# pierluigiferrari/ssd_keras

Measured on AMD Instinct MI355X. Metric: images/sec SSD300 fwd+decode @batch32, higher is better.
Workload: dtype f32 (decode, threshold, TF-style f32 NMS, top-k); bf16 conv backbone; 1 GPU; SSD300 VGG-16 inference (mode='inference': forward + DecodeDetections), 21 classes, batch 32 per GPU, conf 0.01 / NMS 0.45 / top-200, random-init weights, synthetic 300x300x3 uint8-range images; per_gpu_batch=32, global_batch=32, conv_dtype=bf16, parallelism=replicas x1, launch=hip_graph (forward + DecodeDetections captured once, replayed per step), decode_stream=same stream; DecodeDetections reads the head outputs directly (no y_pred in HBM)

## Files before the change

### include/ssdhip.h

```cpp
#ifndef SSDHIP_H
#define SSDHIP_H

#include <stddef.h>

#ifdef __cplusplus
extern "C" {
#endif

#define SSDHIP_ABI_VERSION 1

enum {
    SSDHIP_OK = 0,
    SSDHIP_E_BADARG = -1,
    SSDHIP_E_WORKSPACE = -2,
    SSDHIP_E_LAUNCH = -3
};

enum { SSDHIP_F32 = 0, SSDHIP_F64 = 1 };
enum { SSDHIP_CENTROIDS = 0, SSDHIP_CORNERS = 1, SSDHIP_MINMAX = 2 };
enum { SSDHIP_BORDER_HALF = 0, SSDHIP_BORDER_INCLUDE = 1, SSDHIP_BORDER_EXCLUDE = 2 };
enum {
    SSDHIP_SEM_NUMPY = 0,
    SSDHIP_SEM_KERAS = 1,
    SSDHIP_SEM_DEBUG = 2
// ... 139 lines not shown
int ssdhip_conv1_1_x3_nhwc(const float* x, const float* weight, const float* bias, void* y, int B, int H, int W, int relu, void* stream);
int ssdhip_conv1_1_x3_pre_nhwc(const float* images, const float* weight, const float* bias, void* y, int B, int H, int W, int relu,
                               const float* mean_h, const float* divide_h, const int* swap_h, void* stream);

size_t ssdhip_conv2d_splitk_workspace_bytes(int B, int H, int W, int Cin, int Cout, int kernel, int stride, int pad, int dilation,
                                            int ksplit);
int ssdhip_conv2d_splitk_nhwc_bf16(const void* x, const void* weight, const void* bias, void* y, int B, int H, int W, int Cin, int Cout,
                                   int kernel, int stride, int pad, int dilation, int relu, int ksplit, void* ws, size_t ws_bytes,
                                   void* stream);

int ssdhip_conv2d_same_nhwc_bf16_variant(int variant, const void* x, const void* weight, const void* bias, void* y,
                                         int B, int H, int W, int Cin, int Cout, int kernel, int dilation, int relu, void* stream);

int ssdhip_assemble_predictions_strided_f32(int n_layers, const void* const* conf_h, const void* const* loc_h, const int* n_anchors_h,
                                            const int* n_boxes_h, const int* conf_stride_h, const int* loc_stride_h,
                                            const float* anchors_var, int B, int N, int C, float* y_pred, void* stream);
int ssdhip_decode_from_heads_f32(int n_layers, const void* const* conf_h, const void* const* loc_h, const int* n_anchors_h,
                                 const int* n_boxes_h, const int* conf_stride_h, const int* loc_stride_h, const float* anchors_var,
                                 int B, int N, int C, double conf_thresh, double iou_thresh, int top_k, int nms_cap, int class_agnostic,
                                 int semantics, int coords, int normalize_coords, double img_height, double img_width, int border_pixels,
                                 void* out, int out_dtype, int out_rows, int* out_count, int* out_anchor_idx, void* ws, size_t ws_bytes,
                                 void* stream);

int ssdhip_decode_from_heads(int n_layers, const void* const* conf_h, const void* const* loc_h,
                             const void* const* conf_bias_h, const void* const* loc_bias_h,
                             const int* n_anchors_h, const int* n_boxes_h, const int* conf_stride_h,
                             const int* loc_stride_h, const float* anchors_var, int B, int N, int C,
                             double conf_thresh, double iou_thresh, int top_k, int nms_cap, int class_agnostic,
                             int semantics, int coords, int normalize_coords, double img_height, double img_width,
                             int border_pixels, void* out, int out_dtype, int out_rows, int* out_count,
                             int* out_anchor_idx, void* ws, size_t ws_bytes, void* stream);

int ssdhip_conv2d_same_pool2_nhwc_bf16(const void* x, const void* weight, const void* bias, void* y, int B, int H, int W,
                                       int Cin, int Cout, int kernel, int dilation, int relu, void* stream);

int ssdhip_conv2d_same_group_nhwc_bf16(int n_problems, const void* const* x_h, const void* const* weight_h,
                                       const void* const* bias_h, void* const* y_h, const int* B_h, const int* H_h,
                                       const int* W_h, const int* Cin_h, const int* Cout_h, const int* kernel_h,
                                       const int* dilation_h, int relu, void* stream);

int ssdhip_conv3x3_c64_nhwc_bf16(const void* x, const void* weight, const void* bias, void* y, int B, int H, int W,
                                 int Cin, int Cout, int relu, int pool, int n_workgroups, void* stream);
int ssdhip_conv3x3_c64_pool_keep_nhwc_bf16(const void* x, const void* weight, const void* bias, void* y_full, void* y_pooled, int B, int H,
                                           int W, int Cin, int Cout, int relu, int n_workgroups, void* stream);

int ssdhip_conv3x3_halo_nhwc_bf16(const void* x, const void* weight, const void* bias, void* y, int B, int H, int W,
                                  int Cin, int Cout, int relu, int pool, void* stream);

int ssdhip_conv3x3_halo_plan(int B, int H, int W, int Cout, int pool, int* plan);

int ssdhip_conv3x3_halo_masked_nhwc_bf16(const void* x, const void* weight, const void* mask, void* y, float* bias_partial,
                                         int bias_rows, int B, int H, int W, int Cin, int Cout, void* stream);
int ssdhip_conv3x3_halo_masked_bias_rows(int B, int H, int W, int Cout);

int ssdhip_conv3x3_halo_pool_keep_nhwc_bf16(const void* x, const void* weight, const void* bias, void* y_full, void* y_pooled, int B, int H,
                                            int W, int Cin, int Cout, int relu, void* stream);

size_t ssdhip_conv_chain_packed_bytes(int k, int Cin, int Cout);
int ssdhip_conv_chain_pack_weight(const void* weight, void* packed, int k, int Cin, int Cout, void* stream);
int ssdhip_conv_chain_nhwc_bf16(const void* x, int B, int H, int W, int C0, int n_layers, const void* const* packed_h,
                                const void* const* bias_h, void* const* y_h, const int* k_h, const int* stride_h, const int* pad_h,
                                const int* cout_h, const int* relu_h, void* stream);
size_t ssdhip_conv_chain_x3_packed_bytes(int k, int Cin, int Cout);
int ssdhip_conv_chain_x3_pack_weight(const void* weight_x3, void* packed, int k, int Cin, int Cout, void* stream);
int ssdhip_conv_chain_x3_nhwc_f16(const void* x, int B, int H, int W, int C0, int n_layers, const void* const* packed_h,
                                  const float* const* bias_h, void* const* y_h, const int* k_h, const int* stride_h, const int* pad_h,
                                  const int* cout_h, const int* relu_h, const float* mul_h, void* stream);

size_t ssdhip_conv3x3_wgrad_workspace_bytes(int B, int H, int W, int Cin, int Cout);
int ssdhip_conv3x3_wgrad_bias_nhwc_bf16(const void* x, const void* dy, float* dw, const float* bias_partial, int bias_rows, float* db,
                                        int B, int H, int W, int Cin, int Cout, void* ws, size_t ws_bytes, void* stream);
int ssdhip_conv3x3_wgrad_nhwc_bf16(const void* x, const void* dy, float* dw, int B, int H, int W, int Cin, int Cout, void* ws,
                                   size_t ws_bytes, void* stream);

int ssdhip_conv3x3_halo_strided_nhwc_bf16(const void* x, const void* weight, const void* bias, void* y, int B, int H, int W,
                                          int Cin, int Cout, int stride, int pad, int relu, void* stream);

int ssdhip_conv3x3_halo_group_nhwc_bf16(int n_problems, const void* const* x_h, const void* const* weight_h, const void* const* bias_h,
                                        void* const* y_h, const int* B_h, const int* H_h, const int* W_h, const int* Cin_h,
                                        const int* Cout_h, int relu, int max_workgroups, void* stream);

int ssdhip_conv1_block_nhwc_bf16(const void* x3, const void* w1, const void* b1, const void* weight, const void* bias, void* y,
                                 int B, int H, int W, int Cout, int relu, int pool, int n_workgroups, void* stream);

int ssdhip_conv3x3_cin3_nhwc_bf16(const void* x, const void* weight, const void* bias, void* y, int B, int H, int W,
                                  int Cin, int Cout, int relu, void* stream);

size_t ssdhip_conv_bn_elu_pack_bytes(int Cin, int Cout, int kernel);
int ssdhip_conv_bn_elu_nhwc_bf16(const void* x, const void* w_packed, const float* scale, const float* shift, void* y, int B, int H, int W,
                                 int Cin, int Cout, int kernel, int pool, void* stream);

int ssdhip_bn_elu_train_blocks(long long positions, int C);
int ssdhip_bn_elu_train_fwd_nhwc_bf16(const void* y, const void* gamma, const void* beta, int param_bf16, void* running_mean,
                                      void* running_var, int running_bf16, double momentum, double eps, void* full, void* pooled,
                                      float* mean, float* invstd, float* tables, float* partial, int B, int H, int W, int C,
                                      int n_slots, void* stream);
int ssdhip_bn_elu_train_bwd_nhwc_bf16(const void* y, const float* mean, const float* invstd, const void* gamma, const void* beta,
                                      int param_bf16, const void* g_full, const void* g_pooled, void* dy, float* dgamma,
                                      float* dbeta, float* partial, int B, int H, int W, int C, int n_slots, void* stream);

int ssdhip_conv_same_bias_nhwc_bf16(const void* x, const void* w_packed, const void* bias, void* y, int B, int H, int W, int Cin, int Cout,
                                    int kernel, void* stream);
int ssdhip_ssd7_pack_filters(int n_layers, const void* const* weights, void* const* fwd, void* const* flipped, const int* Cin,
                             const int* Cout, const int* kernel, const long long* strides, void* stream);
int ssdhip_ssd7_conv_wgrad_plan(int B, int H, int W, int Cin, int Cout, int kernel, int* plan);
size_t ssdhip_ssd7_conv_wgrad_workspace_bytes(int B, int H, int W, int Cin, int Cout, int kernel);
int ssdhip_ssd7_conv_wgrad_nhwc_bf16(const void* x, const void* dy, void* dw, void* db, int B, int H, int W, int Cin, int Cout, int kernel,
                                     int out_bf16, const long long* dw_strides, void* workspace, size_t workspace_bytes, void* stream);

int ssdhip_image_program(const void* x, int in_dtype, void* y, int out_dtype, int n_images, long long pixels_per_image,
                         const int* ops_dev, const double* args_dev, void* stream);
int ssdhip_image_resize_cv_u8(const void* x, void* y, int B, int H, int W, int Ho, int Wo, int C, int kind, int area, const int* ix_dev,
                              const double* wx_dev, int nx, const int* iy_dev, const double* wy_dev, int ny, void* stream);
int ssdhip_image_resize_gather_cv_u8(const void* x, void* y, int B, int H, int W, int Ho, int Wo, int C, const int* plan_dev,
                                     const int* ix_dev, const double* wx_dev, int nx, const int* iy_dev, const double* wy_dev, int ny,
                                     const void* background_dev, void* stream);
int ssdhip_image_warp_affine_u8(const void* x, void* y, int B, int H, int W, int Ho, int Wo, int C, const int* geo_dev, const int* xtab_dev,
                                const int* ytab_dev, const void* background_dev, void* stream);
int ssdhip_image_resize_gather_ragged_u8(const void* x, const long long* table_dev, void* y, int B, int Ho, int Wo, const int* plan_dev,
                                         const int* ix_dev, const double* wx_dev, int nx, const int* iy_dev, const double* wy_dev, int ny,
                                         const void* background_dev, void* stream);
int ssdhip_image_program_ragged_u8(const void* x, const long long* table_dev, void* y, int B, long long max_pixels, const int* ops_dev,
                                   const double* args_dev, void* stream);
int ssdhip_image_hist_u8(const void* x, long long n_pixels, int C, int channel, unsigned int* hist_dev, void* stream);
int ssdhip_image_lut_u8(const void* x, void* y, long long n_values, int C, int channel_mask, const void* table_dev, void* stream);

int ssdhip_conv3x3_image_nhwc_bf16(const void* x, const void* weight, const void* bias, void* y, int B, int H, int W, int Cin, int Cout,
                                   int dilation, int relu, void* stream);
int ssdhip_conv2d_image_nhwc_bf16(const void* x, const void* weight, const void* bias, void* y, int B, int H, int W, int Cin, int Cout,
                                  int ksize, int stride, int padding, int dilation, int relu, void* stream);
int ssdhip_conv2d_image_x3_nhwc_f16(const void* x, const void* weight, const float* bias, void* y, int B, int H, int W, int C, int Cout,
                                    int ksize, int stride, int padding, int dilation, int relu, int out_f32, float oscale, void* stream);

typedef struct ssdhip_shadow_desc {
    const void* src;
    void* cl;
    void* tr;
    int O, I, KK, tr_ostride, tr_ooff, tile0;
    int src_channels_last;
    int reserved;
} ssdhip_shadow_desc;
int ssdhip_shadow_refresh(const ssdhip_shadow_desc* table_dev, int n_weights, int n_tiles, int n_vectors, int n_vector_blocks, void* stream);
int ssdhip_sgd_momentum_step(int n_tensors, void* const* params_h, const void* const* grads_h, void* const* bufs_h,
                             const long long* numel_h, double lr, double momentum, double weight_decay, void* stream);

#define SSDHIP_ADAM_MAX_GROUPS 64
typedef struct ssdhip_adam_group {
    double lr, decay, beta_1, beta_2;
    double b1t, b2t;
    float lr_t, one_minus_beta_1, one_minus_beta_2, beta_1_f, beta_2_f, epsilon, weight_decay;
    int reserved;
} ssdhip_adam_group;
typedef struct ssdhip_adam_state {
    long long iterations;
    int n_groups, reserved;
    ssdhip_adam_group groups[];
} ssdhip_adam_state;
size_t ssdhip_adam_state_bytes(int n_groups);
int ssdhip_adam_state_init(void* state, int n_groups, int group, double lr, double beta_1, double beta_2, double epsilon, double decay,
                           double weight_decay, long long iterations, void* stream);
int ssdhip_adam_step(int n_tensors, void* const* params_h, const void* const* grads_h, void* const* m_h, void* const* v_h,
                     void* const* vhat_h, const long long* numel_h, int group, void* state, int tick, void* stream);
int ssdhip_adam_step_bf16(int n_tensors, void* const* params_h, const void* const* grads_h, void* const* master_h, void* const* m_h,
                          void* const* v_h, void* const* vhat_h, const long long* numel_h, int group, void* state, int tick, void* stream);
int ssdhip_optim_set_lr(void* state, int group, double lr, void* stream);

typedef struct ssdhip_sgd_group {
    double lr, decay, momentum;
    float lr_t, momentum_f, weight_decay;
    int reserved;
} ssdhip_sgd_group;
typedef struct ssdhip_sgd_state {
    long long iterations;
    int n_groups, reserved;
    ssdhip_sgd_group groups[];
} ssdhip_sgd_state;
size_t ssdhip_sgd_state_bytes(int n_groups);
int ssdhip_sgd_state_init(void* state, int n_groups, int group, double lr, double momentum, double decay, double weight_decay,
                          long long iterations, void* stream);
int ssdhip_sgd_set_lr(void* state, int group, double lr, void* stream);
int ssdhip_sgd_step(int n_tensors, void* const* params_h, const void* const* grads_h, void* const* bufs_h, const long long* numel_h,
                    int group, void* state, int rule, int nesterov, int tick, void* stream);
int ssdhip_sgd_step_bf16(int n_tensors, void* const* params_h, const void* const* grads_h, void* const* master_h, void* const* bufs_h,
                         const long long* numel_h, int group, void* state, int rule, int nesterov, int tick, void* stream);

typedef struct ssdhip_augment_params {
    int img_height, img_width;
    double expand_prob, expand_min_scale, expand_max_scale;
    double crop_prob, crop_min_scale, crop_max_scale, crop_min_aspect_ratio, crop_max_aspect_ratio;
    int n_trials, n_bounds;
    double bound_cdf[8], bound_lower[8], bound_upper[8];
    double flip_prob;
    int n_modes, interpolation_modes[8], out_height, out_width;
    int max_rounds;
} ssdhip_augment_params;
int ssdhip_augment_plans(const int* geometry_dev, int B, int H, int W, int out_h, int out_w, int n_taps, int* plan_dev, int* ix_dev,
                         double* wx_dev, int* iy_dev, double* wy_dev, void* stream);
int ssdhip_ssd_augment_decide(const ssdhip_augment_params* params, int B, const unsigned int* mt_state, const double* labels,
                              const int* n_labels, int* geometry, double* labels_out, int* n_labels_out, unsigned int* mt_state_out,
                              void* stream);
typedef struct ssdhip_augment_photo {
    double prob[4], lower[4], upper[4];
    double swap_prob;
} ssdhip_augment_photo;
int ssdhip_ssd_augment_decide_stream(const ssdhip_augment_params* params, const ssdhip_augment_photo* photo, int B,
                                     const unsigned int* mt_state, const double* labels, const int* n_labels, int* programs_ops,
                                     double* programs_args, int* geometry, double* labels_out, int* n_labels_out,
                                     unsigned int* mt_state_out, void* stream);
int ssdhip_ssd_augment_decide_stream_ragged(const ssdhip_augment_params* params, const ssdhip_augment_photo* photo, int B,
                                            const long long* table_dev, const unsigned int* mt_state, const double* labels,
                                            const int* n_labels, int* programs_ops, double* programs_args, int* geometry,
                                            double* labels_out, int* n_labels_out, unsigned int* mt_state_out, void* stream);
int ssdhip_augment_plans_ragged(const int* geometry_dev, const long long* table_dev, int B, int out_h, int out_w, int n_taps, int* plan_dev,
// ... 7 lines not shown
```

### ssd_keras_amd/_native.py

```python
from __future__ import annotations

import ctypes
import os
import threading

import numpy as np

_LIB_PATH = os.environ.get("SSDHIP_LIB") or os.path.join(os.path.dirname(os.path.abspath(__file__)), "libssdhip.so")
_lib = None
_lock = threading.Lock()

F32, F64 = 0, 1
COORDS = {"centroids": 0, "corners": 1, "minmax": 2}
BORDER = {"half": 0, "include": 1, "exclude": 2}
SEM_NUMPY, SEM_KERAS, SEM_DEBUG = 0, 1, 2
ABI_VERSION = 1


class SsdHipError(RuntimeError):
    pass


def lib_path():
    return _LIB_PATH
# ... 24 lines not shown
    "ssdhip_decode_workspace_bytes": (_SZ, [_I] * 7),
    "ssdhip_decode_detections": (_I, [_P] + [_I] * 4 + [_D, _D] + [_I] * 6 + [_D, _D, _I, _P, _I, _I] + [_P] * 3 + [_SZ, _P]),
    "ssdhip_decode_stages": (_I, [_I, _P] + [_I] * 4 + [_D, _D] + [_I] * 6 + [_D, _D, _I, _P, _I, _I] + [_P] * 3 + [_SZ, _P]),
    "ssdhip_encode_workspace_bytes": (_SZ, [_I] * 4),
    "ssdhip_encode": (_I, [_P] * 4 + [_I] * 5 + [_D, _D, _I, _D, _D] + [_I] * 4 + [_P] * 4 + [_SZ, _P]),
    "ssdhip_loss_workspace_bytes": (_SZ, [_I] * 3),
    "ssdhip_loss_forward": (_I, [_P, _P] + [_I] * 5 + [_F] + [_P] * 4 + [_SZ, _P]),
    "ssdhip_loss_backward": (_I, [_P] * 5 + [_I] * 3 + [_F, _P, _P]),
    "ssdhip_convert_coordinates": (_I, [_P, _I, _P, _LL] + [_I] * 4 + [_P]),
    "ssdhip_iou_result_dtype": (_I, [_I] * 3),
    "ssdhip_box_overlap": (_I, [_I, _P, _I, _I, _P] + [_I] * 5 + [_P, _P]),
    "ssdhip_match_bipartite_greedy": (_I, [_P, _I, _I, _P, _P]),
    "ssdhip_match_multi_workspace_bytes": (_SZ, [_I, _I]),
    "ssdhip_match_multi": (_I, [_P, _I, _I, _D] + [_P] * 4 + [_SZ, _P]),
    "ssdhip_greedy_nms_workspace_bytes": (_SZ, [_I]),
    "ssdhip_greedy_nms": (_I, [_P] + [_I] * 4 + [_P, _I, _D, _I, _I] + [_P] * 3 + [_SZ, _P]),
    "ssdhip_box_filter": (_I, [_P] * 3 + [_I] * 6 + [_D] * 3 + [_I, _P, _P]),
    "ssdhip_match_predictions_workspace_bytes": (_SZ, [_I, _I]),
    "ssdhip_match_predictions": (_I, [_P, _P, _I] + [_P] * 3 + [_I, _I, _D, _I] + [_P] * 6 + [_SZ, _P]),
    "ssdhip_match_predictions_multi": (_I, [_P] * 3 + [_I] + [_P] * 3 + [_I, _I, _P, _I, _D, _I] + [_P] * 6 + [_SZ, _P]),
    "ssdhip_bias_act_nhwc_bf16": (_I, [_P] * 3 + [_LL, _I, _I, _P]),
    "ssdhip_bias_act_maxpool_nhwc_bf16": (_I, [_P] * 3 + [_I] * 10 + [_P]),
    "ssdhip_l2_normalize_nhwc_bf16": (_I, [_P] * 3 + [_LL, _I, _P]),
    "ssdhip_pool2_l2_normalize_nhwc_bf16": (_I, [_P] * 4 + [_I] * 4 + [_P]),
    "ssdhip_preprocess_nhwc_f32_to_bf16": (_I, [_P, _P, _LL, _I] + [_P] * 4),
    "ssdhip_assemble_predictions_bf16": (_I, [_I] + [_P] * 7 + [_I] * 3 + [_P, _P]),
    "ssdhip_l2_normalize_bwd_waves": (_I, [_LL, _I, _I]),
    "ssdhip_l2_normalize_fwd": (_I, [_P] * 4 + [_LL, _I, _I, _P]),
    "ssdhip_l2_normalize_bwd": (_I, [_P] * 6 + [_I, _LL, _I, _I, _P]),
    "ssdhip_relu_bwd_bias_blocks": (_I, [_LL, _I]),
    "ssdhip_channel_sums_nhwc_bf16": (_I, [_P, _P, _LL, _I, _I, _P]),
    "ssdhip_conv1x1_wgrad_workspace_bytes": (_SZ, [_LL, _I, _I]),
    "ssdhip_conv1x1_wgrad_bias_nhwc_bf16": (_I, [_P] * 4 + [_I, _P, _LL, _I, _I, _P, _SZ, _P]),
    "ssdhip_conv3x3_taps_wgrad_workspace_bytes": (_SZ, [_I] * 10),
    "ssdhip_conv3x3_taps_wgrad_bias_nhwc_bf16": (_I, [_P] * 4 + [_I, _P] + [_I] * 10 + [_P, _SZ, _P]),
    "ssdhip_row_sums_f32": (_I, [_P, _I, _I, _P, _P]),
    "ssdhip_embed_strided_nhwc_bf16": (_I, [_P, _P] + [_I] * 8 + [_P]),
    "ssdhip_assemble_predictions_backward_bf16": (_I, [_I] + [_P] * 6 + [_I] * 3 + [_P]),
    "ssdhip_assemble_backward_lds_bytes": (_SZ, [_I, _P, _P, _I]),
    "ssdhip_conv1_1_bwd_blocks": (_I, [_I] * 3),
    "ssdhip_conv1_1_bwd_nhwc_bf16": (_I, [_P] * 5 + [_I] * 4 + [_P]),
    "ssdhip_relu_bwd_bias_nhwc_bf16": (_I, [_P] * 4 + [_LL, _I, _I, _P]),
    "ssdhip_maxpool2_relu_bwd_bias_nhwc_bf16": (_I, [_P] * 4 + [_I] * 5 + [_P]),
    "ssdhip_maxpool_bwd_nhwc_bf16": (_I, [_P] * 3 + [_I] * 9 + [_P]),
    "ssdhip_assemble_predictions_strided_bf16": (_I, [_I] + [_P] * 9 + [_I] * 3 + [_P, _P]),
    "ssdhip_conv2d_same_nhwc_bf16": (_I, [_P] * 4 + [_I] * 8 + [_P]),
    "ssdhip_conv2d_nhwc_bf16": (_I, [_P] * 4 + [_I] * 10 + [_P]),
    "ssdhip_conv2d_nhwc_bf16_variant": (_I, [_I] + [_P] * 4 + [_I] * 10 + [_P]),
    "ssdhip_conv2d_x3_nhwc_f16": (_I, [_P] * 4 + [_I] * 12 + [_F, _P]),
    "ssdhip_conv3x3_halo_x3_nhwc_f16": (_I, [_P] * 4 + [_I] * 7 + [_F, _P]),
    "ssdhip_x3_split_nhwc": (_I, [_P, _P, _LL, _I, _P]),
    "ssdhip_x3_merge_nhwc": (_I, [_P, _P, _LL, _I, _P]),
    "ssdhip_x3_maxpool_nhwc": (_I, [_P, _P] + [_I] * 9 + [_P]),
    "ssdhip_x3_l2_normalize_nhwc": (_I, [_P] * 3 + [_LL, _I, _F, _P]),
    "ssdhip_conv1_1_x3_nhwc": (_I, [_P] * 4 + [_I] * 4 + [_P]),
    "ssdhip_conv1_1_x3_pre_nhwc": (_I, [_P] * 4 + [_I] * 4 + [_P] * 4),
    "ssdhip_conv2d_splitk_workspace_bytes": (_SZ, [_I] * 10),
    "ssdhip_conv2d_splitk_nhwc_bf16": (_I, [_P] * 4 + [_I] * 11 + [_P, _SZ, _P]),
    "ssdhip_conv2d_same_nhwc_bf16_variant": (_I, [_I] + [_P] * 4 + [_I] * 8 + [_P]),
    "ssdhip_assemble_predictions_strided_f32": (_I, [_I] + [_P] * 7 + [_I] * 3 + [_P, _P]),
    "ssdhip_decode_from_heads_f32": (_I, [_I] + [_P] * 7 + [_I] * 3 + [_D, _D] + [_I] * 6 + [_D, _D, _I, _P, _I, _I] + [_P] * 3 + [_SZ, _P]),
    "ssdhip_decode_from_heads": (_I, [_I] + [_P] * 9 + [_I] * 3 + [_D, _D] + [_I] * 6 + [_D, _D, _I, _P, _I, _I] + [_P] * 3 + [_SZ, _P]),
    "ssdhip_conv2d_same_pool2_nhwc_bf16": (_I, [_P] * 4 + [_I] * 8 + [_P]),
    "ssdhip_conv2d_same_group_nhwc_bf16": (_I, [_I] + [_P] * 11 + [_I, _P]),
    "ssdhip_conv3x3_c64_nhwc_bf16": (_I, [_P] * 4 + [_I] * 8 + [_P]),
    "ssdhip_conv3x3_c64_pool_keep_nhwc_bf16": (_I, [_P] * 5 + [_I] * 7 + [_P]),
    "ssdhip_conv3x3_halo_nhwc_bf16": (_I, [_P] * 4 + [_I] * 7 + [_P]),
    "ssdhip_conv3x3_halo_plan": (_I, [_I] * 5 + [_INTP]),
    "ssdhip_conv3x3_halo_masked_nhwc_bf16": (_I, [_P] * 5 + [_I] * 6 + [_P]),
    "ssdhip_conv3x3_halo_masked_bias_rows": (_I, [_I] * 4),
    "ssdhip_conv3x3_halo_pool_keep_nhwc_bf16": (_I, [_P] * 5 + [_I] * 6 + [_P]),
    "ssdhip_conv_chain_packed_bytes": (_SZ, [_I] * 3),
    "ssdhip_conv_chain_pack_weight": (_I, [_P, _P] + [_I] * 3 + [_P]),
    "ssdhip_conv_chain_nhwc_bf16": (_I, [_P] + [_I] * 5 + [_P] * 9),
    "ssdhip_conv_chain_x3_packed_bytes": (_SZ, [_I] * 3),
    "ssdhip_conv_chain_x3_pack_weight": (_I, [_P, _P] + [_I] * 3 + [_P]),
    "ssdhip_conv_chain_x3_nhwc_f16": (_I, [_P] + [_I] * 5 + [_P] * 10),
    "ssdhip_conv3x3_wgrad_workspace_bytes": (_SZ, [_I] * 5),
    "ssdhip_conv3x3_wgrad_bias_nhwc_bf16": (_I, [_P] * 4 + [_I, _P] + [_I] * 5 + [_P, _SZ, _P]),
    "ssdhip_conv3x3_wgrad_nhwc_bf16": (_I, [_P] * 3 + [_I] * 5 + [_P, _SZ, _P]),
    "ssdhip_conv3x3_halo_strided_nhwc_bf16": (_I, [_P] * 4 + [_I] * 8 + [_P]),
    "ssdhip_conv3x3_halo_group_nhwc_bf16": (_I, [_I] + [_P] * 9 + [_I, _I, _P]),
    "ssdhip_conv1_block_nhwc_bf16": (_I, [_P] * 6 + [_I] * 7 + [_P]),
    "ssdhip_conv3x3_cin3_nhwc_bf16": (_I, [_P] * 4 + [_I] * 6 + [_P]),
    "ssdhip_conv_bn_elu_pack_bytes": (_SZ, [_I] * 3),
    "ssdhip_conv_bn_elu_nhwc_bf16": (_I, [_P] * 5 + [_I] * 7 + [_P]),
    "ssdhip_bn_elu_train_blocks": (_I, [_LL, _I]),
    "ssdhip_bn_elu_train_fwd_nhwc_bf16": (_I, [_P] * 3 + [_I, _P, _P, _I, _D, _D] + [_P] * 6 + [_I] * 5 + [_P]),
    "ssdhip_bn_elu_train_bwd_nhwc_bf16": (_I, [_P] * 5 + [_I] + [_P] * 6 + [_I] * 5 + [_P]),
    "ssdhip_conv_same_bias_nhwc_bf16": (_I, [_P] * 4 + [_I] * 6 + [_P]),
    "ssdhip_ssd7_pack_filters": (_I, [_I] + [_P] * 3 + [_INTP] * 3 + [_LLP, _P]),
    "ssdhip_ssd7_conv_wgrad_plan": (_I, [_I] * 6 + [_INTP]),
    "ssdhip_ssd7_conv_wgrad_workspace_bytes": (_SZ, [_I] * 6),
    "ssdhip_ssd7_conv_wgrad_nhwc_bf16": (_I, [_P] * 4 + [_I] * 7 + [_LLP, _P, _SZ, _P]),
    "ssdhip_image_program": (_I, [_P, _I, _P, _I, _I, _LL] + [_P] * 3),
    "ssdhip_image_resize_cv_u8": (_I, [_P, _P] + [_I] * 8 + [_P, _P, _I, _P, _P, _I, _P]),
    "ssdhip_image_resize_gather_cv_u8": (_I, [_P, _P] + [_I] * 6 + [_P] * 3 + [_I, _P, _P, _I, _P, _P]),
    "ssdhip_image_warp_affine_u8": (_I, [_P, _P] + [_I] * 6 + [_P] * 5),
    "ssdhip_image_resize_gather_ragged_u8": (_I, [_P, _P, _P] + [_I] * 3 + [_P] * 3 + [_I, _P, _P, _I, _P, _P]),
    "ssdhip_image_program_ragged_u8": (_I, [_P, _P, _P, _I, _LL] + [_P] * 3),
    "ssdhip_image_hist_u8": (_I, [_P, _LL, _I, _I, _P, _P]),
    "ssdhip_image_lut_u8": (_I, [_P, _P, _LL, _I, _I, _P, _P]),
    "ssdhip_conv3x3_image_nhwc_bf16": (_I, [_P] * 4 + [_I] * 7 + [_P]),
    "ssdhip_conv2d_image_nhwc_bf16": (_I, [_P] * 4 + [_I] * 10 + [_P]),
    "ssdhip_conv2d_image_x3_nhwc_f16": (_I, [_P] * 4 + [_I] * 11 + [_F, _P]),
    "ssdhip_shadow_refresh": (_I, [_P] + [_I] * 4 + [_P]),
    "ssdhip_sgd_momentum_step": (_I, [_I] + [_P] * 4 + [_D] * 3 + [_P]),
    "ssdhip_adam_state_bytes": (_SZ, [_I]),
    "ssdhip_adam_state_init": (_I, [_P, _I, _I] + [_D] * 6 + [_LL, _P]),
    "ssdhip_adam_step": (_I, [_I] + [_P] * 6 + [_I, _P, _I, _P]),
    "ssdhip_adam_step_bf16": (_I, [_I] + [_P] * 7 + [_I, _P, _I, _P]),
    "ssdhip_optim_set_lr": (_I, [_P, _I, _D, _P]),
    "ssdhip_sgd_state_bytes": (_SZ, [_I]),
    "ssdhip_sgd_state_init": (_I, [_P, _I, _I] + [_D] * 4 + [_LL, _P]),
    "ssdhip_sgd_set_lr": (_I, [_P, _I, _D, _P]),
    "ssdhip_sgd_step": (_I, [_I] + [_P] * 4 + [_I, _P, _I, _I, _I, _P]),
    "ssdhip_sgd_step_bf16": (_I, [_I] + [_P] * 5 + [_I, _P, _I, _I, _I, _P]),
    "ssdhip_augment_plans": (_I, [_P] + [_I] * 6 + [_P] * 6),
    "ssdhip_ssd_augment_decide": (_I, [_PARAMS, _I] + [_P] * 8),
    "ssdhip_ssd_augment_decide_stream": (_I, [_PARAMS, _PHOTO, _I] + [_P] * 10),
    "ssdhip_ssd_augment_decide_stream_ragged": (_I, [_PARAMS, _PHOTO, _I] + [_P] * 11),
    "ssdhip_augment_plans_ragged": (_I, [_P, _P] + [_I] * 4 + [_P] * 6),
}


def load():
    global _lib
    if _lib is not None:
        return _lib
    with _lock:
        if _lib is not None:
            return _lib
        if not os.path.exists(_LIB_PATH):
            raise SsdHipError("libssdhip.so not found at %s: build it with `python -m ssd_keras_amd.build` "
                              "(hipcc, gfx950).  ssd_keras_amd has no CPU fallback." % _LIB_PATH)
        lib = ctypes.CDLL(_LIB_PATH)
        for name, (restype, argtypes) in SIGNATURES.items():
            if not hasattr(lib, name):
                raise SsdHipError("%s lacks %s: rebuild it with `python -m ssd_keras_amd.build`" % (_LIB_PATH, name))
            fn = getattr(lib, name)
            fn.restype, fn.argtypes = restype, argtypes
        if lib.ssdhip_abi_version() != ABI_VERSION:
            raise SsdHipError("libssdhip.so ABI %d != expected %d" % (lib.ssdhip_abi_version(), ABI_VERSION))
        _lib = lib
    return _lib


def check(rc, what):
    if rc != 0:
        raise SsdHipError("%s failed: %s (rc=%d)" % (what, load().ssdhip_strerror(rc).decode(), rc))


def _torch():
    import torch
    return torch


def require_cuda(t, name):
    if not t.is_cuda:
        raise SsdHipError("%s must live on a GPU (got device %s): ssd_keras_amd has no CPU path" % (name, t.device))
    if not t.is_contiguous():
        raise SsdHipError("%s must be contiguous" % name)


def current_stream_ptr(device):
    torch = _torch()
    return ctypes.c_void_p(torch.cuda.current_stream(device).cuda_stream)


def launch(name, device, *args):
    torch = _torch()
    with torch.cuda.device(device):
        rc = getattr(load(), name)(*args, current_stream_ptr(device))
    check(rc, name)


class _Workspaces:

    def __init__(self):
        self._bufs = {}

    def get(self, device, purpose, nbytes, zeroed=False):
        torch = _torch()
        key = (str(device), purpose, int(torch.cuda.current_stream(device).cuda_stream))
        buf = self._bufs.get(key)
        if buf is None or buf.numel() < nbytes:
            buf = (torch.zeros if zeroed else torch.empty)(int(nbytes), dtype=torch.uint8, device=device)
# ... 526 lines not shown
    launch("ssdhip_maxpool_bwd_nhwc_bf16", x.device, _ptr(x), _ptr(gy), _ptr(gx), b, h, w, c, int(kernel), int(stride), int(pad), ho, wo)
    return gx


def conv2d_same(x, weight, bias, dilation=1, relu=True, variant=None):
    torch = _torch()
    x, (b, h, w, cin) = _nhwc_bf16(x, "x")
    cout, cin_w, kh, kw = weight.shape
    if weight.dtype != torch.bfloat16 or cin_w != cin or kh != kw:
        raise SsdHipError("weight must be bfloat16 (Cout, %d, k, k)" % cin)
    wt = weight if weight.permute(0, 2, 3, 1).is_contiguous() else weight.permute(0, 2, 3, 1).contiguous().permute(0, 3, 1, 2)
    y = torch.empty((b, h, w, cout), dtype=torch.bfloat16, device=x.device).permute(0, 3, 1, 2)
    args = (_ptr(x), _ptr(wt), _ptr(bias), _ptr(y), b, h, w, cin, cout, int(kh), int(dilation), int(bool(relu)))
    if variant is None:
        launch("ssdhip_conv2d_same_nhwc_bf16", x.device, *args)
    else:
        launch("ssdhip_conv2d_same_nhwc_bf16_variant", x.device, int(variant), *args)
    return y


def conv3x3_halo_plan(b, h, w, pool, cout=128):
    plan = (ctypes.c_int * 4)()
    check(load().ssdhip_conv3x3_halo_plan(int(b), int(h), int(w), int(cout), int(bool(pool)), plan), "ssdhip_conv3x3_halo_plan")
    return tuple(plan)


def conv3x3_halo(x, weight, bias, relu=True, pool=False):
    torch = _torch()
    x, (b, h, w, cin) = _nhwc_bf16(x, "x")
    cout, cin_w, kh, kw = weight.shape
    if weight.dtype != torch.bfloat16 or cin_w != cin or kh != 3 or kw != 3:
        raise SsdHipError("weight must be bfloat16 (Cout, %d, 3, 3)" % cin)
    wt = weight if weight.permute(0, 2, 3, 1).is_contiguous() else weight.permute(0, 2, 3, 1).contiguous().permute(0, 3, 1, 2)
    ho, wo = ((h + 1) // 2, (w + 1) // 2) if pool else (h, w)
    y = torch.empty((b, ho, wo, cout), dtype=torch.bfloat16, device=x.device).permute(0, 3, 1, 2)
    launch("ssdhip_conv3x3_halo_nhwc_bf16", x.device, _ptr(x), _ptr(wt), _ptr(bias), _ptr(y), b, h, w, cin, cout, int(bool(relu)),
           int(bool(pool)))
    return y


def conv3x3_halo_masked(x, weight, mask, sums=False):
    torch = _torch()
    lib = load()
    cout, cin_w, kh, kw = weight.shape
    if (not x.is_cuda or x.dtype != torch.bfloat16 or weight.dtype != torch.bfloat16 or mask.dtype != torch.bfloat16 or kh != 3 or kw != 3
            or cin_w % 128 or cout % 128 or x.shape[1] != cin_w):
        return None
    x, (b, h, w, cin) = _nhwc_bf16(x, "x")
    mask, mshape = _nhwc_bf16(mask, "mask")
    if mshape != (b, h, w, cout):
        raise SsdHipError("mask must have the output's shape %s, got %s" % ((b, h, w, cout), mshape))
    wt = weight if weight.permute(0, 2, 3, 1).is_contiguous() else weight.permute(0, 2, 3, 1).contiguous().permute(0, 3, 1, 2)
    y = torch.empty((b, h, w, cout), dtype=torch.bfloat16, device=x.device).permute(0, 3, 1, 2)
    partial, rows = None, 0
    with torch.cuda.device(x.device):
        if sums:
            rows = lib.ssdhip_conv3x3_halo_masked_bias_rows(b, h, w, cout)
            if rows <= 0:
                return None
            partial = torch.empty((rows, cout), dtype=torch.float32, device=x.device)
        rc = lib.ssdhip_conv3x3_halo_masked_nhwc_bf16(_ptr(x), _ptr(wt), _ptr(mask), _ptr(y), _ptr(partial), rows, b, h, w, cin, cout,
                                                      current_stream_ptr(x.device))
    if rc == -1:
        return None
    check(rc, "ssdhip_conv3x3_halo_masked_nhwc_bf16")
    return (y, partial) if sums else y


def conv3x3_image_supported(x, weight, dilation=1):
    b, cin, h, w = x.shape
    cout, cin_w, kh, kw = weight.shape
    return kh == 3 and kw == 3 and cin_w == cin and h * w <= 384 and cin % 64 == 0 and cout % 64 == 0 and 1 <= int(dilation) <= 16


def conv3x3_image(x, weight, bias, dilation=1, relu=True):
    torch = _torch()
    x, (b, h, w, cin) = _nhwc_bf16(x, "x")
    cout, cin_w, kh, kw = weight.shape
    if weight.dtype != torch.bfloat16 or cin_w != cin or kh != 3 or kw != 3:
        raise SsdHipError("weight must be bfloat16 (Cout, %d, 3, 3)" % cin)
    wt = weight if weight.permute(0, 2, 3, 1).is_contiguous() else weight.permute(0, 2, 3, 1).contiguous().permute(0, 3, 1, 2)
    y = torch.empty((b, h, w, cout), dtype=torch.bfloat16, device=x.device).permute(0, 3, 1, 2)
    launch("ssdhip_conv3x3_image_nhwc_bf16", x.device, _ptr(x), _ptr(wt), _ptr(bias), _ptr(y), b, h, w, cin, cout, int(dilation),
           int(bool(relu)))
    return y


def conv2d_image_supported(x, weight, stride=1, padding=0, dilation=1):
    b, cin, h, w = x.shape
    cout, cin_w, kh, kw = weight.shape
    k, s, p, d = int(kh), int(stride), int(padding), int(dilation)
    if kh != kw or k not in (1, 3) or cin_w != cin or cin % 64 or cout % 64 or h * w > 384:
        return False
    if not (1 <= s <= 4 and 1 <= d <= 16 and 0 <= p <= d * (k // 2)) or h + 2 * p < d * (k - 1) + 1 or w + 2 * p < d * (k - 1) + 1:
        return False
    ho, wo = (h + 2 * p - d * (k - 1) - 1) // s + 1, (w + 2 * p - d * (k - 1) - 1) // s + 1
    return 1 <= ho * wo <= 384


def conv2d_image(x, weight, bias, stride=1, padding=0, dilation=1, relu=True):
    torch = _torch()
    x, (b, h, w, cin) = _nhwc_bf16(x, "x")
    cout, cin_w, kh, kw = weight.shape
    if weight.dtype != torch.bfloat16 or cin_w != cin or kh != kw or kh not in (1, 3):
        raise SsdHipError("weight must be bfloat16 (Cout, %d, k, k) with k in (1, 3)" % cin)
    k, s, p, d = int(kh), int(stride), int(padding), int(dilation)
    wt = weight if weight.permute(0, 2, 3, 1).is_contiguous() else weight.permute(0, 2, 3, 1).contiguous().permute(0, 3, 1, 2)
    ho, wo = (h + 2 * p - d * (k - 1) - 1) // s + 1, (w + 2 * p - d * (k - 1) - 1) // s + 1
    if ho < 1 or wo < 1:
        raise SsdHipError("the filter does not fit the padded map")
    y = torch.empty((b, ho, wo, cout), dtype=torch.bfloat16, device=x.device).permute(0, 3, 1, 2)
    launch("ssdhip_conv2d_image_nhwc_bf16", x.device, _ptr(x), _ptr(wt), _ptr(bias), _ptr(y), b, h, w, cin, cout, k, s, p, d,
           int(bool(relu)))
    return y


def conv_chain_pack(weight, out=None):
    torch = _torch()
    lib = load()
    cout, cin, kh, kw = weight.shape
    if weight.dtype != torch.bfloat16 or kh != kw:
        raise SsdHipError("weight must be bfloat16 (Cout, Cin, k, k)")
    n = int(lib.ssdhip_conv_chain_packed_bytes(kh, cin, cout))
    if n == 0:
        return None
    wt = weight if weight.permute(0, 2, 3, 1).is_contiguous() else weight.permute(0, 2, 3, 1).contiguous().permute(0, 3, 1, 2)
    if out is not None and (out.numel() != n or out.dtype != torch.uint8 or out.device != weight.device):
        raise SsdHipError("conv_chain_pack: `out` does not match this filter's packed size")
    packed = out if out is not None else torch.empty((n,), dtype=torch.uint8, device=weight.device)
    launch("ssdhip_conv_chain_pack_weight", weight.device, _ptr(wt), _ptr(packed), kh, cin, cout)
    return packed


def conv_chain(x, layers):
    torch = _torch()
    lib = load()
    x, (b, h, w, c0) = _nhwc_bf16(x, "x")
    n = len(layers)
    outs, ys = [], []
    hh, ww = h, w
    for l in layers:
        hh = (hh + 2 * l["pad"] - l["k"]) // l["stride"] + 1
        ww = (ww + 2 * l["pad"] - l["k"]) // l["stride"] + 1
        if hh < 1 or ww < 1:
            return None
        if l.get("keep", False):
            y = torch.empty((b, hh, ww, l["cout"]), dtype=torch.bfloat16, device=x.device).permute(0, 3, 1, 2)
            outs.append(y)
            ys.append(y)
        else:
            ys.append(None)
    parr = lambda ts: (ctypes.c_void_p * n)(*[(t.data_ptr() if t is not None else None) for t in ts])
    iarr = lambda key: (ctypes.c_int * n)(*[int(l[key]) for l in layers])
    with torch.cuda.device(x.device):
        rc = lib.ssdhip_conv_chain_nhwc_bf16(_ptr(x), b, h, w, c0, n, parr([l["packed"] for l in layers]), parr([l.get("bias") for l in layers]),
                                             parr(ys), iarr("k"), iarr("stride"), iarr("pad"), iarr("cout"), iarr("relu"),
                                             current_stream_ptr(x.device))
    if rc == -1:
        return None
    check(rc, "ssdhip_conv_chain_nhwc_bf16")
    return outs


def conv_chain_x3_pack(packed_weight, out=None):
    torch = _torch()
    lib = load()
# ... 621 lines not shown
                or t.dtype not in (torch.float32, torch.bfloat16)):
            raise SsdHipError("bn_elu_train: %s must be a contiguous (%d,) float32 or bfloat16 tensor on %s" % (name, c, device))
        dtypes.add(t.dtype)
    if len(dtypes) > 1:
        raise SsdHipError("bn_elu_train: %s must share one dtype" % " and ".join(named))
    return int(dtypes.pop() == torch.bfloat16)


def bn_elu_train_blocks(positions, c):
    return int(load().ssdhip_bn_elu_train_blocks(int(positions), int(c)))


def bn_elu_train_forward(y, gamma, beta, running_mean, running_var, momentum, eps, pool, keep_full):
    torch = _torch()
    b, h, w, c = _bn_train_map(y, "y")
    nb = bn_elu_train_blocks(b * h * w, c)
    if nb == 0:
        raise SsdHipError("bn_elu_train: no kernel for C = %d with B H W = %d (C in 32, 48, 64; at least two positions)" % (c, b * h * w))
    if pool and (h < 2 or w < 2):
        raise SsdHipError("bn_elu_train: a %d x %d map has no 2 x 2 window to pool" % (h, w))
    param_bf16 = _bn_train_vectors(c, y.device, gamma=gamma, beta=beta)
    if (running_mean is None) != (running_var is None):
        raise SsdHipError("bn_elu_train: running_mean and running_var come together")
    running_bf16 = 0 if running_mean is None else _bn_train_vectors(c, y.device, running_mean=running_mean, running_var=running_var)
    dev = y.device
    full = torch.empty((b, h, w, c), dtype=torch.bfloat16, device=dev).permute(0, 3, 1, 2) if (keep_full or not pool) else None
    pooled = torch.empty((b, h // 2, w // 2, c), dtype=torch.bfloat16, device=dev).permute(0, 3, 1, 2) if pool else None
    stats = torch.empty((4, c), dtype=torch.float32, device=dev)
    partial = torch.empty((nb, 3, c), dtype=torch.float32, device=dev)
    launch("ssdhip_bn_elu_train_fwd_nhwc_bf16", dev, _ptr(y), _ptr(gamma), _ptr(beta), param_bf16, _ptr(running_mean), _ptr(running_var),
           running_bf16, float(momentum), float(eps), _ptr(full), _ptr(pooled), _ptr(stats[0]), _ptr(stats[1]), _ptr(stats[2]),
           _ptr(partial), b, h, w, c, nb)
    return full, pooled, stats[0], stats[1]


def bn_elu_train_backward(y, mean, invstd, gamma, beta, g_full, g_pooled):
    torch = _torch()
    b, h, w, c = _bn_train_map(y, "y")
    nb = bn_elu_train_blocks(b * h * w, c)
    if nb == 0:
        raise SsdHipError("bn_elu_train: no kernel for C = %d with B H W = %d (C in 32, 48, 64; at least two positions)" % (c, b * h * w))
    if g_full is None and g_pooled is None:
        raise SsdHipError("bn_elu_train: the backward needs the gradient of the full map, of the pooled map or both")
    if g_full is not None and _bn_train_map(g_full, "g_full") != (b, h, w, c):
        raise SsdHipError("bn_elu_train: g_full must have y's shape")
    if g_pooled is not None and (h < 2 or w < 2 or _bn_train_map(g_pooled, "g_pooled") != (b, h // 2, w // 2, c)):
        raise SsdHipError("bn_elu_train: g_pooled must be the gradient of y's 2 x 2 'valid' pooled map")
    param_bf16 = _bn_train_vectors(c, y.device, gamma=gamma, beta=beta)
    if _bn_train_vectors(c, y.device, mean=mean, invstd=invstd) != 0:
        raise SsdHipError("bn_elu_train: mean and invstd are float32")
    dev = y.device
    dy = torch.empty((b, h, w, c), dtype=torch.bfloat16, device=dev).permute(0, 3, 1, 2)
    grads = torch.empty((2, c), dtype=torch.float32, device=dev)
    partial = torch.empty((nb, 2, c), dtype=torch.float32, device=dev)
    launch("ssdhip_bn_elu_train_bwd_nhwc_bf16", dev, _ptr(y), _ptr(mean), _ptr(invstd), _ptr(gamma), _ptr(beta), param_bf16, _ptr(g_full),
           _ptr(g_pooled), _ptr(dy), _ptr(grads[0]), _ptr(grads[1]), _ptr(partial), b, h, w, c, nb)
    return dy, grads[0], grads[1]


def conv1_block(x, w1, b1, weight, bias, relu=True, pool=False):
    torch = _torch()
    if not x.is_cuda or x.dtype != torch.bfloat16 or x.dim() != 4 or x.shape[1] != 3:
        raise SsdHipError("x must be a (B, 3, H, W) bfloat16 CUDA tensor")
    if not x.permute(0, 2, 3, 1).is_contiguous():
        x = x.permute(0, 2, 3, 1).contiguous().permute(0, 3, 1, 2)
    b, _, h, w = x.shape
    if tuple(w1.shape) != (64, 3, 3, 3) or weight.shape[1:] != (64, 3, 3) or w1.dtype != torch.bfloat16 or weight.dtype != torch.bfloat16:
        raise SsdHipError("conv1_block needs bfloat16 (64, 3, 3, 3) and (Cout, 64, 3, 3) weights")
    cl = lambda t: t if t.permute(0, 2, 3, 1).is_contiguous() else t.permute(0, 2, 3, 1).contiguous().permute(0, 3, 1, 2)
    w1c, w2c = cl(w1), cl(weight)
    cout = weight.shape[0]
    ho, wo = ((h + 1) // 2, (w + 1) // 2) if pool else (h, w)
    y = torch.empty((b, ho, wo, cout), dtype=torch.bfloat16, device=x.device).permute(0, 3, 1, 2)
    dev = x.device
    n_cu = _CU_COUNT.get(dev.index)
    if n_cu is None:
        n_cu = torch.cuda.get_device_properties(dev).multi_processor_count
        _CU_COUNT[dev.index] = n_cu
    launch("ssdhip_conv1_block_nhwc_bf16", dev, _ptr(x), _ptr(w1c), _ptr(b1), _ptr(w2c), _ptr(bias), _ptr(y), b, h, w, cout,
           int(bool(relu)), int(bool(pool)), int(n_cu))
    return y


CONVERSIONS = {"minmax2centroids": 0, "centroids2minmax": 1, "corners2centroids": 2, "centroids2corners": 3,
               "minmax2corners": 4, "corners2minmax": 4}


def _float_device(a, name):
    torch = _torch()
    if isinstance(a, np.ndarray):
        if a.dtype not in (np.float32, np.float64):
            a = a.astype(np.float64)
        return to_device(a)
    if not torch.is_tensor(a):
        return to_device(np.asarray(a, dtype=np.float64))
    if a.dtype not in (torch.float32, torch.float64):
        a = a.to(torch.float64)
    return to_device(a)


def _dt(t):
    torch = _torch()
    return F32 if t.dtype == torch.float32 else F64


def convert_coordinates(t, start_index, conversion, border_pixels):
    torch = _torch()
    require_cuda(t, "tensor")
    L = int(t.shape[-1])
    rows = t.numel() // L if L else 0
    out = torch.empty(t.shape, dtype=torch.float64, device=t.device)
    if t.numel() == 0:
        return out
    launch("ssdhip_convert_coordinates", t.device, _ptr(t), _dt(t), _ptr(out), rows, L, int(start_index), CONVERSIONS[conversion],
           BORDER[border_pixels])
    return out


def box_overlap(op, b1, b2, coords, mode, border_pixels):
    torch = _torch()
    lib = load()
    require_cuda(b1, "boxes1")
    require_cuda(b2, "boxes2")
    m, n = int(b1.shape[0]), int(b2.shape[0])
    rdt = torch.float32 if lib.ssdhip_iou_result_dtype(_dt(b1), _dt(b2), COORDS[coords]) == F32 else torch.float64
    outer = mode == "outer_product"
    out = torch.empty((m, n) if outer else (max(m, n) if min(m, n) > 0 else 0,), dtype=rdt, device=b1.device)
    if out.numel() == 0:
        return out
    launch("ssdhip_box_overlap", b1.device, int(op), _ptr(b1), _dt(b1), m, _ptr(b2), _dt(b2), n, COORDS[coords], 0 if outer else 1,
           BORDER[border_pixels], _ptr(out))
    return out


def match_bipartite_greedy(w):
    torch = _torch()
    require_cuda(w, "weight_matrix")
    m, n = int(w.shape[0]), int(w.shape[1])
    out = torch.zeros((m,), dtype=torch.int32, device=w.device)
    if m == 0:
        return out
    launch("ssdhip_match_bipartite_greedy", w.device, _ptr(w), m, n, _ptr(out))
    return out


def match_multi(w, threshold):
    torch = _torch()
    lib = load()
    require_cuda(w, "weight_matrix")
    m, n = int(w.shape[0]), int(w.shape[1])
    gt = torch.empty((max(n, 1),), dtype=torch.int32, device=w.device)
    col = torch.empty((max(n, 1),), dtype=torch.int32, device=w.device)
    cnt = torch.zeros((1,), dtype=torch.int32, device=w.device)
    ws = workspaces.get(w.device, "match_multi", lib.ssdhip_match_multi_workspace_bytes(m, n))
    launch("ssdhip_match_multi", w.device, _ptr(w), m, n, float(threshold), _ptr(gt), _ptr(col), _ptr(cnt), _ptr(ws), ws.numel())
    k = int(cnt.item())
    return gt[:k], col[:k]


def greedy_nms_rows(rows, seg_offsets, score_col, box_col, iou_threshold, coords, border_pixels):
    torch = _torch()
    lib = load()
    require_cuda(rows, "rows")
    n_total, L = int(rows.shape[0]), int(rows.shape[1])
    S = len(seg_offsets) - 1
    dev = rows.device
# ... 349 lines not shown
```

### ssd_keras_amd/csrc/ssdhip_bf16.h

```cpp
#pragma once
#include <hip/hip_runtime.h>
#include <stdint.h>

namespace ssdhip {

typedef unsigned int u32;

typedef unsigned short bf16_t;
typedef __bf16 bf16x2 __attribute__((ext_vector_type(2)));
typedef __bf16 bf16x8 __attribute__((ext_vector_type(8)));
typedef _Float16 f16x8 __attribute__((ext_vector_type(8)));
typedef float f32x2 __attribute__((ext_vector_type(2)));
typedef float f32x16 __attribute__((ext_vector_type(16)));
typedef short s16x2 __attribute__((ext_vector_type(2)));
typedef int i32x4 __attribute__((ext_vector_type(4)));
typedef unsigned int u32x2 __attribute__((ext_vector_type(2)));
typedef unsigned int u32x4 __attribute__((ext_vector_type(4)));

__device__ __forceinline__ float bf16_float(u32 h) { return __uint_as_float(h << 16); }
template <typename T = u32>
__device__ __forceinline__ T bf16_bits(float f) {
    const u32 u = __float_as_uint(f);
    if ((u & 0x7fffffffu) > 0x7f800000u) return (T)((u >> 16) | 0x40u);
    return (T)((u + 0x7fffu + ((u >> 16) & 1u)) >> 16);
}

__device__ __forceinline__ u32 pack2_bf16(float a, float b) {
    const f32x2 v = {a, b};
    return __builtin_bit_cast(u32, __builtin_convertvector(v, bf16x2));
}

__device__ __forceinline__ float relu_nan(float v) { return v <= 0.f ? 0.f : v; }

__device__ __forceinline__ u32 pkmax_i16(u32 a, u32 b) {
    return __builtin_bit_cast(u32, __builtin_elementwise_max(__builtin_bit_cast(s16x2, a), __builtin_bit_cast(s16x2, b)));
}

__device__ __forceinline__ u32 split2_f16(float a, float b, u32& lo_out) {
    const _Float16 ha = (_Float16)a, hb = (_Float16)b;
    const _Float16 la = (_Float16)(a - (float)ha), lb = (_Float16)(b - (float)hb);
    lo_out = (u32)__builtin_bit_cast(unsigned short, la) | ((u32)__builtin_bit_cast(unsigned short, lb) << 16);
    return (u32)__builtin_bit_cast(unsigned short, ha) | ((u32)__builtin_bit_cast(unsigned short, hb) << 16);
}

}
```

### ssd_keras_amd/csrc/ssdhip_conv64.hip

```cpp
#include <hip/hip_runtime.h>
#include <stdint.h>
#include <stdlib.h>

#include <type_traits>

#include "ssdhip.h"
#include "ssdhip_math.h"
#include "ssdhip_bf16.h"
#include "ssdhip_tile.h"

#ifndef SSDHIP_C64_ABLATE
#define SSDHIP_C64_ABLATE 0
#endif

namespace ssdhip {

#ifdef SSDHIP_PROFILE
__device__ unsigned long long g_prof64[32];
#define C64_PROF_DECL long long _pt = clock64(); long long _pa[8] = {0, 0, 0, 0, 0, 0, 0, 0}; int _pn = 0;
#define C64_PROF_MARK(i) { const long long _t = clock64(); _pa[i] += _t - _pt; _pt = _t; }
#define C64_PROF_TILE ++_pn;
#define C64_PROF_FLUSH(base) if (lane == 0) { for (int _i = 0; _i < 8; ++_i) atomicAdd(&g_prof64[(base) + _i], (unsigned long long)_pa[_i]); atomicAdd(&g_prof64[(base) + 8], (unsigned long long)_pn); }
#else
#define C64_PROF_DECL
#define C64_PROF_MARK(i)
#define C64_PROF_TILE
#define C64_PROF_FLUSH(base)
#endif

#ifndef SSDHIP_C64_NLOAD
#define SSDHIP_C64_NLOAD 1
#endif
constexpr int C64_NLOAD = SSDHIP_C64_NLOAD;
constexpr int C64_THREADS = (4 + C64_NLOAD) * 64;
constexpr int C64_NPROD = 3;
constexpr int C64_FRONT_THREADS = (4 + C64_NPROD) * 64;
constexpr int C64_WBYTES = 9 * 64 * 128;
constexpr int C64_STAGE = 0;
constexpr int c64_halo_bytes(int cs) { return ((9 * (2 * (64 >> cs) + 2) * ((1 << cs) + 2) + 63) / 64) * 1024; }
constexpr int C64_PATCH1 = 1600;
constexpr int C64_PATCH = ((C64_NPROD * C64_PATCH1 + 1023) / 1024) * 1024;
constexpr int C64_WREG_BYTES = 1024;
constexpr int c64_lds_bytes(int cs, int nb, bool front = false, bool wreg = false) {
    return (wreg ? C64_WREG_BYTES : C64_WBYTES) + nb * c64_halo_bytes(cs) + C64_STAGE + (front ? C64_PATCH : 0);
}

struct C64Params {
    const bf16_t* x;
    const bf16_t* w;
    const bf16_t* bias;
    bf16_t* y;
    int B, H, W, Cout, relu;
    int HT, WT, n_slices, tiles;
    int Ho, Wo;
    int x_bytes, w_bytes;
    const bf16_t* x3;
    const bf16_t* w1;
    const bf16_t* b1;
    int prio;
    int xcd_pairs;
    bf16_t* y2;
};

#if defined(__HIP_DEVICE_COMPILE__)
__device__ __forceinline__ float c64_max_with_lane_xor1(float v) {
    float r;
    asm("s_nop 1\n\tv_max_f32_dpp %0, %1, %1 quad_perm:[1,0,3,2] row_mask:0xf bank_mask:0xf" : "=v"(r) : "v"(v));
    return r;
}
__device__ __forceinline__ void c64_store_runs(const u32 (&lo)[4], const u32 (&hi)[4], __amdgpu_buffer_rsrc_t ry, u32 voff, u32 soff) {
#pragma unroll
    for (int pr = 0; pr < 2; ++pr) {
        const auto sl = __builtin_amdgcn_permlane32_swap(lo[2 * pr], lo[2 * pr + 1], false, false);
        const auto sh = __builtin_amdgcn_permlane32_swap(hi[2 * pr], hi[2 * pr + 1], false, false);
        if (!(SSDHIP_C64_ABLATE & 1)) __builtin_amdgcn_raw_buffer_store_b128(u32x4{sl[0], sh[0], sl[1], sh[1]}, ry, voff + pr * 32, soff, 0);
    }
}
__device__ __forceinline__ u32 c64_load_u16(u32 voff, i32x4 rsrc, u32 soff) {
    u32 v;
    asm volatile("buffer_load_ushort %0, %1, %2, %3 offen" : "=v"(v) : "v"(voff), "s"(rsrc), "s"(soff) : "memory");
    return v;
}

__device__ __forceinline__ u32 c64_load_u32(u32 voff, i32x4 rsrc, u32 soff) {
    u32 v;
    asm volatile("buffer_load_dword %0, %1, %2, %3 offen" : "=v"(v) : "v"(voff), "s"(rsrc), "s"(soff) : "memory");
    return v;
}

template <int CS, bool POOL, int NB, bool FRONT, bool WREG, bool KEEP = false>
__device__ __forceinline__ void conv64_body(const C64Params& p, unsigned char* lds) {
    static_assert(!KEEP || (POOL && !FRONT), "KEEP is a variant of the pooled, un-fused kernel");
    constexpr int CC = 1 << CS, RP = 64 >> CS;
    constexpr int HC = CC + 2, HR = 2 * RP + 2;
    constexpr int HPX = HR * HC;
    constexpr int SLOTS = 9 * HPX;
    constexpr int NP = (SLOTS + 63) / 64;
    constexpr int HB = NP * 1024;
    static_assert(HB == c64_halo_bytes(CS) && c64_lds_bytes(CS, NB, FRONT, WREG) <= 160 * 1024, "LDS budget");
    constexpr int WB = WREG ? C64_WREG_BYTES : C64_WBYTES;
    constexpr int W_OFF = 0, H_OFF = WB, STAGE_OFF = WB + NB * HB, PATCH_OFF = STAGE_OFF + C64_STAGE;
    constexpr unsigned OOB = 0x80000000u;

    const int G = (int)gridDim.x;
    int slice = (int)blockIdx.x % p.n_slices, first = (int)blockIdx.x / p.n_slices;
    const int stride = G / p.n_slices;
    if (p.xcd_pairs) {
        const int xcd = (int)blockIdx.x & 7, j = (int)blockIdx.x >> 3;
        slice = j % p.n_slices;
        first = xcd + 8 * (j / p.n_slices);
    }
    if (first >= p.tiles) return;
    const int co0 = slice * 64;

    const int tid = threadIdx.x, lane = tid & 63;
    const int wave = __builtin_amdgcn_readfirstlane(tid >> 6);
    const int wc = wave >> 1, wp = wave & 1;
    const int r31 = lane & 31, khalf = lane >> 5;
    const u32 lds0 = (u32)(uintptr_t)(__attribute__((address_space(3))) unsigned char*)lds;
    const int xneg = (p.W + 1) * 128;
    const i32x4 rx = tile_rsrc(reinterpret_cast<const unsigned char*>(p.x) - xneg, p.x_bytes + 2 * xneg);
    const i32x4 rw = tile_rsrc(p.w, p.w_bytes);

    if (!WREG && wave < 4) {
        const int pos = lane & 7;
#pragma unroll
        for (int t = 0; t < 9; ++t)
#pragma unroll
            for (int i = 0; i < 2; ++i) {
                const int piece = i * 4 + wave;
                const int row = piece * 8 + (lane >> 3);
                const int j = pos ^ ((row >> 1) & 7);
                tile_dma16_soff((u32)((co0 + row) * 1152 + t * 128 + j * 16), rw, lds0 + W_OFF + t * 8192 + piece * 1024, 0u);
            }
    }

    auto tile_origin = [&](int tile, int& b, int& h0, int& w0) {
        const int wt = tile % p.WT, r = tile / p.WT;
        b = r / p.HT;
        h0 = (r - b * p.HT) * (2 * RP);
        w0 = wt * CC;
    };

    if constexpr (FRONT) {
      if (wave >= 4) {
        const int prod = wave - 4;
        constexpr int PR = HR + 2, PC = HC + 2, PROW = PC * 3, PATCH = PR * PROW;
        constexpr int NRAW = (PATCH + 63) / 64, NBLK = (HPX + 31) / 32, MYB = NBLK / C64_NPROD;
        static_assert(NB == 2 && (PR + 1) * PROW * 2 <= C64_PATCH1 && NRAW * 64 * 2 <= C64_PATCH1 && NBLK % C64_NPROD == 0,
                      "two halo buffers; a patch copy holds the patch, a spare row and every raw slot");
        unsigned char* patch = lds + PATCH_OFF + prod * C64_PATCH1;
        for (int i = lane; i < C64_PATCH1 / 4; i += 64) reinterpret_cast<u32*>(patch)[i] = 0u;
        bf16x8 aw[2][2];
#pragma unroll
        for (int cb = 0; cb < 2; ++cb)
#pragma unroll
            for (int st = 0; st < 2; ++st) {
                union { bf16x8 v; unsigned short u[8]; } t;
#pragma unroll
                for (int j = 0; j < 8; ++j) {
                    const int k = (2 * st + khalf) * 8 + j;
                    t.u[j] = k < 27 ? p.w1[(cb * 32 + r31) * 27 + k] : (unsigned short)0;
                }
                aw[cb][st] = t.v;
            }
        float b1v[2][16];
#pragma unroll
        for (int cb = 0; cb < 2; ++cb)
#pragma unroll
            for (int g = 0; g < 4; ++g)
#pragma unroll
                for (int e = 0; e < 4; ++e)
                    b1v[cb][4 * g + e] = p.b1 ? __uint_as_float((u32)p.b1[cb * 32 + 8 * g + 4 * khalf + e] << 16) : 0.f;
        u32 pbase[MYB], hdst[MYB], hcoord[MYB];
#pragma unroll
        for (int blk = 0; blk < MYB; ++blk) {
            const int hp = (C64_NPROD * blk + prod) * 32 + r31, hpc = hp < HPX ? hp : HPX - 1;
            const int hr = hpc / HC, hc = hpc - hr * HC;
            pbase[blk] = (u32)((hr * PROW + hc * 3) * 2);
            hdst[blk] = (u32)(hpc * 144 + 8 * khalf);
            hcoord[blk] = (u32)((hr << 8) | hc | (hp < HPX ? 0 : 0x10000));
        }
        const i32x4 r3 = tile_rsrc(p.x3, p.B * p.H * p.W * 6);
        auto run = [&](auto widec) {
        constexpr bool WIDE = decltype(widec)::value;
        constexpr int ROWB = PROW * 2, NDW = PATCH / 2, DPR = PROW / 2, NRAWW = (NDW + 63) / 64;
        constexpr int NR = WIDE ? NRAWW : NRAW;
        static_assert(PROW % 2 == 0 && NRAWW * 64 * 4 <= C64_PATCH1 && (HR + 1) * ROWB + (HC - 1) * 6 + 32 <= C64_PATCH1,
                      "dword patch rows; every raw slot and every fragment read stay inside the producer's patch copy");
        [[maybe_unused]] u32 kofs[2][8];
        [[maybe_unused]] u32 fadr[MYB][4], fsel[MYB][5];
        if constexpr (WIDE) {
#pragma unroll
            for (int blk = 0; blk < MYB; ++blk) {
                const u32 sb = pbase[blk] & 2u, a0 = pbase[blk] - sb;
                const u32 fun0 = 0x03020100u + sb * 0x01010101u, fun2 = fun0 + 0x02020202u;
                const u32 one = sb | ((sb + 1u) << 8);
                if (khalf == 0) {
                    fadr[blk][0] = a0; fadr[blk][1] = a0 + 4; fadr[blk][2] = a0 + ROWB + 12; fadr[blk][3] = a0 + 2 * ROWB;
                    fsel[blk][0] = fun0; fsel[blk][1] = fun0; fsel[blk][2] = fun2; fsel[blk][3] = fun0; fsel[blk][4] = fun0;
                } else {
                    fadr[blk][0] = a0 + 16; fadr[blk][1] = a0 + ROWB; fadr[blk][2] = a0 + 2 * ROWB + 12; fadr[blk][3] = a0 + 2 * ROWB + 16;
                    fsel[blk][0] = one | ((one + 0x0404u) << 16);
                    fsel[blk][1] = fun2;
                    fsel[blk][2] = fun0;
                    fsel[blk][3] = one | 0x0c0c0000u;
                    fsel[blk][4] = 0x0c0c0c0cu;
                }
            }
        } else {
#pragma unroll
            for (int st = 0; st < 2; ++st)
#pragma unroll
                for (int j = 0; j < 8; ++j) {
                    const int k = (2 * st + khalf) * 8 + j;
                    kofs[st][j] = (u32)(((k / 9) * PROW + (k % 9)) * 2);
                }
        }
        u32 rrel[NR], rco[NR];
#pragma unroll
        for (int i = 0; i < NR; ++i) {
            const int n = 64 * i + lane;
            if constexpr (WIDE) {
                const int nn = n < NDW ? n : 0;
                const int pr = nn / DPR, c4 = nn - pr * DPR;
                rrel[i] = n < NDW ? (u32)((pr * p.W) * 6 + c4 * 4) : OOB;
                rco[i] = (u32)((pr << 16) | (((2 * c4) / 3) << 8) | ((2 * c4 + 1) / 3));
            } else {
                const int nn = n < PATCH ? n : 0;
                const int pr = nn / PROW, rem = nn - pr * PROW, pc = rem / 3;
                rrel[i] = n < PATCH ? (u32)(((pr * p.W) * 3 + rem) * 2) : OOB;
                rco[i] = (u32)((pr << 16) | (pc << 8) | pc);
            }
        }
        auto load = [&](u32 voff, u32 soff) { return WIDE ? c64_load_u32(voff, r3, soff) : c64_load_u16(voff, r3, soff); };
        auto request = [&](int tile, u32 (&raw)[NR]) {
            int b, h0, w0;
            tile_origin(tile, b, h0, w0);
            const int ph = h0 - 2, pw = w0 - 2;
            const bool inside = ph >= 0 && pw >= 0 && ph + PR <= p.H && pw + PC <= p.W;
            if (inside) {
                const u32 soff = (u32)((((b * p.H + ph) * p.W + pw) * 3) * 2);
#pragma unroll
                for (int i = 0; i < NR; ++i) raw[i] = load(rrel[i], soff);
            } else {
                const int base = ((b * p.H + ph) * p.W + pw) * 6;
#pragma unroll
                for (int i = 0; i < NR; ++i) {
                    const int pr = (int)(rco[i] >> 16), pcs = (int)(rco[i] >> 8) & 0xff, pce = (int)rco[i] & 0xff;
                    const bool ok = rrel[i] != OOB && (unsigned)(ph + pr) < (unsigned)p.H && (unsigned)(pw + pcs) < (unsigned)p.W &&
                                    (unsigned)(pw + pce) < (unsigned)p.W;
                    raw[i] = load(ok ? (u32)(base + (int)rrel[i]) : OOB, 0u);
                }
            }
        };
        C64_PROF_DECL
        auto landed = [&](u32 (&raw)[NR], bool newer) {
            if (newer) asm volatile("s_waitcnt vmcnt(%0)" :: "n"(NR) : "memory");
            else asm volatile("s_waitcnt vmcnt(0)" ::: "memory");
#pragma unroll
            for (int i = 0; i < NR; ++i) asm volatile("" : "+v"(raw[i]));
        };
        auto produce = [&](int tile, const u32 (&raw)[NR], int buf) {
            int b, h0, w0;
            tile_origin(tile, b, h0, w0);
            unsigned char* hb = lds + H_OFF + buf * HB;
            bf16x8 bfr[MYB][2];
            if constexpr (WIDE) {
#pragma unroll
                for (int i = 0; i < NR; ++i) reinterpret_cast<u32*>(patch)[64 * i + lane] = raw[i];
#pragma unroll
                for (int blk = 0; blk < MYB; ++blk) {
                    const u32* q0 = reinterpret_cast<const u32*>(patch + fadr[blk][0]);
                    const u32* q1 = reinterpret_cast<const u32*>(patch + fadr[blk][1]);
                    const u32* q2 = reinterpret_cast<const u32*>(patch + fadr[blk][2]);
                    const u32* q3 = reinterpret_cast<const u32*>(patch + fadr[blk][3]);
                    const u32 s0 = q0[0], s1 = q1[0], s2 = q1[1], s3 = q1[2], s4 = q1[3];
                    const u32 t0 = q2[0], t1 = q2[1], t2 = q3[0], t3 = q3[1], t4 = q3[2], t5 = q3[3];
                    const u32x4 f0 = {__builtin_amdgcn_perm(s1, s0, fsel[blk][0]), __builtin_amdgcn_perm(s2, s1, fsel[blk][1]),
                                          __builtin_amdgcn_perm(s3, s2, fsel[blk][1]), __builtin_amdgcn_perm(s4, s3, fsel[blk][1])};
                    const u32x4 f1 = {__builtin_amdgcn_perm(t1, t0, fsel[blk][2]), __builtin_amdgcn_perm(t3, t2, fsel[blk][3]),
                                          __builtin_amdgcn_perm(t4, t3, fsel[blk][4]), __builtin_amdgcn_perm(t5, t4, fsel[blk][4])};
                    bfr[blk][0] = __builtin_bit_cast(bf16x8, f0);
                    bfr[blk][1] = __builtin_bit_cast(bf16x8, f1);
                }
            } else {
#pragma unroll
                for (int i = 0; i < NR; ++i) reinterpret_cast<unsigned short*>(patch)[64 * i + lane] = (unsigned short)raw[i];
#pragma unroll
                for (int blk = 0; blk < MYB; ++blk)
#pragma unroll
                    for (int st = 0; st < 2; ++st) {
                        union { bf16x8 v; unsigned short u[8]; } t;
#pragma unroll
                        for (int j = 0; j < 8; ++j) t.u[j] = *reinterpret_cast<const unsigned short*>(patch + pbase[blk] + kofs[st][j]);
                        bfr[blk][st] = t.v;
                    }
            }
            if (p.prio & 2) __builtin_amdgcn_s_setprio(3);
            f32x16 a1[MYB][2];
#pragma unroll
            for (int blk = 0; blk < MYB; ++blk)
#pragma unroll
                for (int cb = 0; cb < 2; ++cb) {
#pragma unroll
                    for (int v = 0; v < 16; ++v) a1[blk][cb][v] = 0.f;
                    a1[blk][cb] = __builtin_amdgcn_mfma_f32_32x32x16_bf16(aw[cb][0], bfr[blk][0], a1[blk][cb], 0, 0, 0);
                }
#pragma unroll
            for (int blk = 0; blk < MYB; ++blk)
#pragma unroll
                for (int cb = 0; cb < 2; ++cb) a1[blk][cb] = __builtin_amdgcn_mfma_f32_32x32x16_bf16(aw[cb][1], bfr[blk][1], a1[blk][cb], 0, 0, 0);
            if (p.prio & 2) __builtin_amdgcn_s_setprio(0);
            C64_PROF_MARK(2)
            auto finish = [&](auto edge) {
                constexpr bool EDGE = decltype(edge)::value;
#pragma unroll
                for (int blk = 0; blk < MYB; ++blk) {
                    const int hr = (int)(hcoord[blk] >> 8) & 0xff, hc = (int)hcoord[blk] & 0xff;
                    const bool live = (blk + 1 < MYB) || !(hcoord[blk] & 0x10000);
                    const bool in_img = !EDGE || ((unsigned)(h0 - 1 + hr) < (unsigned)p.H && (unsigned)(w0 - 1 + hc) < (unsigned)p.W);
                    const u32 keep = in_img ? 0xffffffffu : 0u;
#pragma unroll
                    for (int cb = 0; cb < 2; ++cb)
#pragma unroll
                        for (int g = 0; g < 4; ++g) {
                            float o[4];
#pragma unroll
                            for (int e = 0; e < 4; ++e) o[e] = a1[blk][cb][4 * g + e] + b1v[cb][4 * g + e];
                            u32 lo = pkmax_i16(pack2_bf16(o[0], o[1]), 0u), hi = pkmax_i16(pack2_bf16(o[2], o[3]), 0u);
                            if constexpr (EDGE) { lo &= keep; hi &= keep; }
                            if (live) *reinterpret_cast<uint2*>(hb + hdst[blk] + (cb * 32 + 8 * g) * 2) = make_uint2(lo, hi);
                        }
                }
            };
            if (h0 >= 1 && w0 >= 1 && h0 - 1 + HR <= p.H && w0 - 1 + HC <= p.W) finish(std::false_type{});
            else finish(std::true_type{});
            C64_PROF_MARK(3)
        };
        u32 raw_a[NR], raw_b[NR];
        request(first, raw_a);
        landed(raw_a, false);
        produce(first, raw_a, 0);
        if (first + stride < p.tiles) request(first + stride, raw_a);
        asm volatile("s_waitcnt lgkmcnt(0)" ::: "memory");
        __builtin_amdgcn_s_barrier();
        int buf = 0;
        auto step = [&](int tile, u32 (&cur)[NR], u32 (&nxt)[NR]) {
            const bool req = !(SSDHIP_C64_ABLATE & 8) && tile + 2 * stride < p.tiles;
            if (req) request(tile + 2 * stride, nxt);
            C64_PROF_MARK(0)
            if (!(SSDHIP_C64_ABLATE & 8) && tile + stride < p.tiles) {
                landed(cur, req);
                C64_PROF_MARK(1)
                produce(tile + stride, cur, buf ^ 1);
            }
            asm volatile("s_waitcnt lgkmcnt(0)" ::: "memory");
            C64_PROF_MARK(4)
            __builtin_amdgcn_s_barrier();
            C64_PROF_MARK(5)
            C64_PROF_TILE
            buf ^= 1;
        };
        for (int tile = first; tile < p.tiles; tile += 2 * stride) {
            step(tile, raw_a, raw_b);
            if (tile + stride >= p.tiles) break;
            step(tile + stride, raw_b, raw_a);
        }
        if (wave == 4) { C64_PROF_FLUSH(16) }
        };
        if (!(p.W & 1) && !((uintptr_t)p.x3 & 3)) run(std::true_type{});
        else run(std::false_type{});
        return;
      }
    }

    if (!FRONT && wave >= 4) {
        const int lw = wave - 4;
        constexpr int NPW = NP / C64_NLOAD;
        static_assert(NP % C64_NLOAD == 0, "every loader wave issues the same number of pieces (compile-time wait counts)");
        int hrc[NPW];
        u32 rel[NPW];
#pragma unroll
        for (int k = 0; k < NPW; ++k) {
            const int n = 64 * (k * C64_NLOAD + lw) + lane;
            const int px = n / 9, c = n - 9 * px;
            const int hr = px / HC, hc = px - hr * HC;
            const bool data = c < 8 && px < HPX;
            hrc[k] = data ? ((hr << 16) | (hc << 4) | c) : -1;
            rel[k] = data ? (u32)((hr * p.W + hc) * 128 + c * 16) : OOB;
        }
        auto issue_halo = [&](int tile, int buf) {
            int b, h0, w0;
            tile_origin(tile, b, h0, w0);
            const u32 dst = lds0 + H_OFF + buf * HB + lw * 1024;
            if (h0 >= 1 && w0 >= 1 && h0 + 2 * RP + 1 <= p.H && w0 + CC + 1 <= p.W) {
                const u32 soff = (u32)(((b * p.H + h0 - 1) * p.W + (w0 - 1)) * 128 + xneg);
#pragma unroll
                for (int k = 0; k < NPW; ++k) tile_dma16_soff(rel[k], rx, dst + k * C64_NLOAD * 1024, soff);
            } else {
#pragma unroll
                for (int k = 0; k < NPW; ++k) {
                    const int h = h0 - 1 + (hrc[k] >> 16), w = w0 - 1 + ((hrc[k] >> 4) & 0xfff);
                    const bool ok = hrc[k] >= 0 && (unsigned)h < (unsigned)p.H && (unsigned)w < (unsigned)p.W;
                    const u32 voff = ok ? (u32)(((b * p.H + h) * p.W + w) * 128 + (hrc[k] & 15) * 16 + xneg) : OOB;
                    tile_dma16_soff(voff, rx, dst + k * C64_NLOAD * 1024, 0u);
                }
            }
        };
        static_assert(FRONT || (NB == 3 && 2 * NPW <= 63), "wait accounting: two halos of NPW loads in flight must fit vmcnt");
        issue_halo(first, 0);
        if (first + stride < p.tiles) issue_halo(first + stride, 1);
        if (first + 2 * stride < p.tiles) issue_halo(first + 2 * stride, 2);
        if (first + 2 * stride < p.tiles) asm volatile("s_waitcnt vmcnt(%0)" :: "n"(2 * NPW) : "memory");
        else if (first + stride < p.tiles) asm volatile("s_waitcnt vmcnt(%0)" :: "n"(NPW) : "memory");
        else asm volatile("s_waitcnt vmcnt(0)" ::: "memory");
        __builtin_amdgcn_s_barrier();
        int buf = 0;
        C64_PROF_DECL
        for (int tile = first; tile < p.tiles; tile += stride) {
            if (tile + 2 * stride < p.tiles) asm volatile("s_waitcnt vmcnt(%0)" :: "n"(NPW) : "memory");
            else asm volatile("s_waitcnt vmcnt(0)" ::: "memory");
            C64_PROF_MARK(0)
            __builtin_amdgcn_s_barrier();
            C64_PROF_MARK(1)
            if (tile + 3 * stride < p.tiles) issue_halo(tile + 3 * stride, buf);
            C64_PROF_MARK(2)
            C64_PROF_TILE
            buf = buf + 1 == NB ? 0 : buf + 1;
        }
        if (wave == 4) { C64_PROF_FLUSH(16) }
        return;
    }

    if (p.prio & 1) __builtin_amdgcn_s_setprio(2);
    const int q = wp * 32 + r31;
    const int rp = q >> CS, col = q & (CC - 1);
    u32 bbase[2];
#pragma unroll
    for (int pi = 0; pi < 2; ++pi) bbase[pi] = (u32)(H_OFF + ((2 * rp + pi) * HC + col) * 144 + khalf * 16);
    u32 ylane[2];
    [[maybe_unused]] u32 yfull[2] = {0u, 0u};
    if constexpr (KEEP) {
#pragma unroll
        for (int pi = 0; pi < 2; ++pi) yfull[pi] = (u32)((((2 * rp + pi) * p.W + col) * p.Cout) * 2 + khalf * 16);
    }
    if constexpr (POOL) {
        ylane[0] = ylane[1] = (u32)(((rp * p.Wo + (col >> 1)) * p.Cout) * 2 + khalf * 16);
    } else {
#pragma unroll
        for (int pi = 0; pi < 2; ++pi) ylane[pi] = (u32)((((2 * rp + pi) * p.W + col) * p.Cout) * 2 + khalf * 16);
    }
    u32 abase[4];
    {
// ... 73 lines not shown
        int b, h0, w0;
        tile_origin(tile, b, h0, w0);
        const u32 floor16 = p.relu ? 0u : 0x80008000u;
        if constexpr ((SSDHIP_C64_ABLATE & 2) != 0) {
            asm volatile("" :: "v"(acc[0]), "v"(acc[1]));
        } else
        if constexpr (POOL) {
            if constexpr (KEEP) {
                const size_t img2 = (size_t)p.H * p.W * p.Cout * 2;
                const __amdgpu_buffer_rsrc_t ry2 = __builtin_amdgcn_make_buffer_rsrc(reinterpret_cast<unsigned char*>(p.y2) + (size_t)b * img2, 0, (int)img2, 0x00020000);
                const u32 sbase2 = (u32)(((h0 * p.W + w0) * p.Cout + co0 + wc * 32) * 2);
#pragma unroll
                for (int pi = 0; pi < 2; ++pi) {
                    const bool ok = ((h0 + 2 * rp + pi) < p.H) & ((w0 + col) < p.W);
                    const u32 voff2 = yfull[pi] | (ok ? 0u : OOB);
                    u32 lo[4], hi[4];
#pragma unroll
                    for (int g = 0; g < 4; ++g) {
                        lo[g] = pkmax_i16(pack2_bf16(acc[pi][4 * g] + bv[4 * g], acc[pi][4 * g + 1] + bv[4 * g + 1]), floor16);
                        hi[g] = pkmax_i16(pack2_bf16(acc[pi][4 * g + 2] + bv[4 * g + 2], acc[pi][4 * g + 3] + bv[4 * g + 3]), floor16);
                    }
                    c64_store_runs(lo, hi, ry2, voff2, sbase2);
                }
            }
            const size_t img = (size_t)p.Ho * p.Wo * p.Cout * 2;
            const __amdgpu_buffer_rsrc_t ry = __builtin_amdgcn_make_buffer_rsrc(reinterpret_cast<unsigned char*>(p.y) + (size_t)b * img, 0, (int)img, 0x00020000);
            const u32 sbase = (u32)((((h0 >> 1) * p.Wo + (w0 >> 1)) * p.Cout + co0 + wc * 32) * 2);
            const int hq = h0 + 2 * rp, wq = w0 + col;
            const bool okp = (!(r31 & 1)) & (((h0 >> 1) + rp) < p.Ho) & ((wq >> 1) < p.Wo);
            const u32 voff = ylane[0] | (okp ? 0u : OOB);
            auto pooled = [&](auto edge) {
                constexpr bool EDGE = decltype(edge)::value;
                const bool has_below = !EDGE || hq + 1 < p.H, has_right = !EDGE || wq + 1 < p.W;
                u32 lo[4], hi[4];
#pragma unroll
                for (int g = 0; g < 4; ++g) {
                    float o[4];
#pragma unroll
                    for (int e = 0; e < 4; ++e) {
                        float v = acc[0][4 * g + e];
                        if constexpr (EDGE) {
                            const float below = acc[1][4 * g + e];
                            if (has_below) v = below > v ? below : v;
                            const float right = __int_as_float(__builtin_amdgcn_update_dpp(0, __float_as_int(v), 0xB1, 0xf, 0xf, false));
                            if (has_right) v = right > v ? right : v;
                        } else {
                            const float below = acc[1][4 * g + e];
                            v = below > v ? below : v;
                            v = c64_max_with_lane_xor1(v);
                        }
                        o[e] = v + bv[4 * g + e];
                    }
                    lo[g] = pkmax_i16(pack2_bf16(o[0], o[1]), floor16);
                    hi[g] = pkmax_i16(pack2_bf16(o[2], o[3]), floor16);
                }
                c64_store_runs(lo, hi, ry, voff, sbase);
            };
            if (h0 + 2 * RP <= p.H && w0 + CC <= p.W) pooled(std::false_type{});
            else pooled(std::true_type{});
        } else {
            const size_t img = (size_t)p.H * p.W * p.Cout * 2;
            const __amdgpu_buffer_rsrc_t ry = __builtin_amdgcn_make_buffer_rsrc(reinterpret_cast<unsigned char*>(p.y) + (size_t)b * img, 0, (int)img, 0x00020000);
            const u32 sbase = (u32)(((h0 * p.W + w0) * p.Cout + co0 + wc * 32) * 2);
#pragma unroll
            for (int pi = 0; pi < 2; ++pi) {
                const bool ok = ((h0 + 2 * rp + pi) < p.H) & ((w0 + col) < p.W);
                const u32 voff = ylane[pi] | (ok ? 0u : OOB);
                u32 lo[4], hi[4];
#pragma unroll
                for (int g = 0; g < 4; ++g) {
                    lo[g] = pkmax_i16(pack2_bf16(acc[pi][4 * g] + bv[4 * g], acc[pi][4 * g + 1] + bv[4 * g + 1]), floor16);
                    hi[g] = pkmax_i16(pack2_bf16(acc[pi][4 * g + 2] + bv[4 * g + 2], acc[pi][4 * g + 3] + bv[4 * g + 3]), floor16);
                }
                c64_store_runs(lo, hi, ry, voff, sbase);
            }
        }
        C64_PROF_MARK(2)
        C64_PROF_TILE
    }
    if (wave == 0) { C64_PROF_FLUSH(0) }
}
#endif

template <int CS, bool POOL, int NB, bool FRONT = false, bool WREG = false, bool KEEP = false>
__global__ __launch_bounds__(FRONT ? C64_FRONT_THREADS : C64_THREADS, 1) void conv64_kernel(C64Params p) {
#if defined(__HIP_DEVICE_COMPILE__)
    __shared__ __attribute__((aligned(1024))) unsigned char lds[c64_lds_bytes(CS, NB, FRONT, WREG)];
    conv64_body<CS, POOL, NB, FRONT, WREG, KEEP>(p, lds);
#endif
}

}

using namespace ssdhip;

static int c64_launch(const void* x, const void* weight, const void* bias, void* y, void* y2, int B, int H, int W, int Cin, int Cout, int relu,
                      int pool, int n_workgroups, void* stream_) {
    hipStream_t stream = static_cast<hipStream_t>(stream_);
    if (!x || !weight || !y || B <= 0 || H <= 0 || W <= 0 || Cin != 64 || Cout <= 0 || (Cout % 64)) return SSDHIP_E_BADARG;
    if (((uintptr_t)x | (uintptr_t)weight | (uintptr_t)y | (uintptr_t)y2) & 15 || ((uintptr_t)bias & 1)) return SSDHIP_E_BADARG;
    if (y2 && !pool) return SSDHIP_E_BADARG;
    const long long xb = (long long)B * H * W * 128, wb = (long long)Cout * 1152;
    if (xb >= 0x7ffff000LL || wb >= 0x7ffff000LL || (long long)B * H * W * Cout > 0x7fffffff0LL) return SSDHIP_E_BADARG;
    C64Params p;
    p.x = static_cast<const bf16_t*>(x); p.w = static_cast<const bf16_t*>(weight); p.bias = static_cast<const bf16_t*>(bias);
    p.y = static_cast<bf16_t*>(y);
    p.B = B; p.H = H; p.W = W; p.Cout = Cout; p.relu = relu ? 1 : 0;
    p.Ho = (H + 1) / 2; p.Wo = (W + 1) / 2;
    p.x_bytes = (int)xb; p.w_bytes = (int)wb;
    p.x3 = nullptr; p.w1 = nullptr; p.b1 = nullptr;
    p.y2 = static_cast<bf16_t*>(y2);
    { const char* e = getenv("SSDHIP_C64_PRIO"); p.prio = e ? atoi(e) : 1; }
    p.n_slices = Cout / 64;
    int cs_best = 4;
    long long best = -1;
    for (int cs = 4; cs >= 3; --cs) {
        const long long wt = (W + (1 << cs) - 1) >> cs, ht = (p.Ho + (64 >> cs) - 1) / (64 >> cs);
        if (best < 0 || wt * ht < best) { best = wt * ht; cs_best = cs; p.WT = (int)wt; p.HT = (int)ht; }
    }
    const long long tiles = (long long)B * p.HT * p.WT;
    if (tiles > 0x3fffffffLL) return SSDHIP_E_BADARG;
    p.tiles = (int)tiles;
    int G = n_workgroups > 0 ? n_workgroups : 256;
    if (G > 4096) G = 4096;
    G = (G / p.n_slices) * p.n_slices;
    if (G < p.n_slices) G = p.n_slices;
    { const char* e = getenv("SSDHIP_C64_XCD"); p.xcd_pairs = (p.n_slices > 1 && G % (8 * p.n_slices) == 0 && !(e && atoi(e) == 0)) ? 1 : 0; }
    static const bool wreg = []() { const char* e = getenv("SSDHIP_C64_WREG"); return e ? atoi(e) != 0 : true; }();
#define C64_LAUNCH(CS_, POOL_) do { if (wreg) hipLaunchKernelGGL((conv64_kernel<CS_, POOL_, 3, false, true>), dim3(G), dim3(C64_THREADS), 0, stream, p); \
                                    else hipLaunchKernelGGL((conv64_kernel<CS_, POOL_, 3>), dim3(G), dim3(C64_THREADS), 0, stream, p); } while (0)
    if (pool && y2) {
        if (cs_best == 3) hipLaunchKernelGGL((conv64_kernel<3, true, 3, false, true, true>), dim3(G), dim3(C64_THREADS), 0, stream, p);
        else hipLaunchKernelGGL((conv64_kernel<4, true, 3, false, true, true>), dim3(G), dim3(C64_THREADS), 0, stream, p);
    } else if (pool) {
        if (cs_best == 3) C64_LAUNCH(3, true); else C64_LAUNCH(4, true);
    } else {
        if (cs_best == 3) C64_LAUNCH(3, false); else C64_LAUNCH(4, false);
    }
#undef C64_LAUNCH
    return hipGetLastError() == hipSuccess ? SSDHIP_OK : SSDHIP_E_LAUNCH;
}

extern "C" int ssdhip_conv3x3_c64_nhwc_bf16(const void* x, const void* weight, const void* bias, void* y, int B, int H, int W,
                                            int Cin, int Cout, int relu, int pool, int n_workgroups, void* stream) {
    return c64_launch(x, weight, bias, y, nullptr, B, H, W, Cin, Cout, relu, pool, n_workgroups, stream);
}

extern "C" int ssdhip_conv3x3_c64_pool_keep_nhwc_bf16(const void* x, const void* weight, const void* bias, void* y_full, void* y_pooled, int B,
                                                      int H, int W, int Cin, int Cout, int relu, int n_workgroups, void* stream) {
    if (!y_full) return SSDHIP_E_BADARG;
    return c64_launch(x, weight, bias, y_pooled, y_full, B, H, W, Cin, Cout, relu, 1, n_workgroups, stream);
}

extern "C" int ssdhip_conv1_block_nhwc_bf16(const void* x3, const void* w1, const void* b1, const void* weight, const void* bias, void* y,
                                            int B, int H, int W, int Cout, int relu, int pool, int n_workgroups, void* stream_) {
    hipStream_t stream = static_cast<hipStream_t>(stream_);
    if (!x3 || !w1 || !weight || !y || B <= 0 || H <= 0 || W <= 0 || Cout <= 0 || (Cout % 64)) return SSDHIP_E_BADARG;
    if (((uintptr_t)weight | (uintptr_t)y) & 15 || (((uintptr_t)x3 | (uintptr_t)w1 | (uintptr_t)b1 | (uintptr_t)bias) & 1)) return SSDHIP_E_BADARG;
    const long long wb = (long long)Cout * 1152;
    if ((long long)B * H * W * 6 >= 0x7ffff000LL || wb >= 0x7ffff000LL || (long long)B * H * W * Cout > 0x7fffffff0LL) return SSDHIP_E_BADARG;
    C64Params p;
    p.x = nullptr; p.w = static_cast<const bf16_t*>(weight); p.bias = static_cast<const bf16_t*>(bias);
    p.y = static_cast<bf16_t*>(y);
    p.x3 = static_cast<const bf16_t*>(x3); p.w1 = static_cast<const bf16_t*>(w1); p.b1 = static_cast<const bf16_t*>(b1);
    p.y2 = nullptr;
    { const char* e = getenv("SSDHIP_C64_PRIO"); p.prio = e ? atoi(e) : 3; }
    p.B = B; p.H = H; p.W = W; p.Cout = Cout; p.relu = relu ? 1 : 0;
    p.Ho = (H + 1) / 2; p.Wo = (W + 1) / 2;
    p.x_bytes = 0; p.w_bytes = (int)wb;
    p.n_slices = Cout / 64;
    int cs_best = 4;
    long long best = -1;
    for (int cs = 4; cs >= 3; --cs) {
        const long long wt = (W + (1 << cs) - 1) >> cs, ht = (p.Ho + (64 >> cs) - 1) / (64 >> cs);
        if (best < 0 || wt * ht < best) { best = wt * ht; cs_best = cs; p.WT = (int)wt; p.HT = (int)ht; }
    }
    const long long tiles = (long long)B * p.HT * p.WT;
    if (tiles > 0x3fffffffLL) return SSDHIP_E_BADARG;
    p.tiles = (int)tiles;
    int G = n_workgroups > 0 ? n_workgroups : 256;
    if (G > 4096) G = 4096;
    G = (G / p.n_slices) * p.n_slices;
    if (G < p.n_slices) G = p.n_slices;
    { const char* e = getenv("SSDHIP_C64_XCD"); p.xcd_pairs = (p.n_slices > 1 && G % (8 * p.n_slices) == 0 && !(e && atoi(e) == 0)) ? 1 : 0; }
    static const bool wreg = []() { const char* e = getenv("SSDHIP_C64_WREG"); return e ? atoi(e) != 0 : true; }();
#define C64F_LAUNCH(CS_, POOL_) do { if (wreg) hipLaunchKernelGGL((conv64_kernel<CS_, POOL_, 2, true, true>), dim3(G), dim3(C64_FRONT_THREADS), 0, stream, p); \
                                     else hipLaunchKernelGGL((conv64_kernel<CS_, POOL_, 2, true>), dim3(G), dim3(C64_FRONT_THREADS), 0, stream, p); } while (0)
    if (pool) {
        if (cs_best == 3) C64F_LAUNCH(3, true); else C64F_LAUNCH(4, true);
    } else {
        if (cs_best == 3) C64F_LAUNCH(3, false); else C64F_LAUNCH(4, false);
    }
#undef C64F_LAUNCH
    return hipGetLastError() == hipSuccess ? SSDHIP_OK : SSDHIP_E_LAUNCH;
}

#ifdef SSDHIP_PROFILE
extern "C" int ssdhip_profile_read_c64(unsigned long long* host_out, int reset) {
    if (hipMemcpyFromSymbol(host_out, HIP_SYMBOL(g_prof64), sizeof(g_prof64)) != hipSuccess) return -1;
    if (reset) { unsigned long long z[32] = {0}; if (hipMemcpyToSymbol(HIP_SYMBOL(g_prof64), z, sizeof(z)) != hipSuccess) return -1; }
    return 0;
}
#endif
```

### ssd_keras_amd/csrc/ssdhip_convimg.hip

```cpp
#include <hip/hip_runtime.h>
#include <stdint.h>
#include <stdlib.h>

#include "ssdhip.h"
#include "ssdhip_math.h"
#include "ssdhip_bf16.h"
#include "ssdhip_tile.h"

namespace ssdhip {

constexpr int CI_THREADS = 512;
constexpr int CI_PX = 384;
constexpr int CI_ROW = 144;
constexpr int CI_SLAB = (CI_PX + 1) * CI_ROW;
[[maybe_unused]] constexpr int CI_ZERO = CI_PX * CI_ROW;
constexpr int CI_WST = 128 * 128;
constexpr int CI_NW = 3;
constexpr int CI_W0 = 2 * CI_SLAB;
constexpr int CI_DUMP = CI_W0 + CI_NW * CI_WST;
constexpr int CI_BIAS = CI_DUMP + 1024;
constexpr int CI_LDS = CI_BIAS + 512;
static_assert(CI_LDS <= 160 * 1024, "LDS budget");
static_assert(CI_SLAB % 16 == 0, "slab buffers are 16-byte aligned");

#ifdef SSDHIP_PROFILE
__device__ unsigned long long g_profi[8];
#define CI_PROF_DECL long long _pt = clock64(); long long _pa[4] = {0, 0, 0, 0};
#define CI_PROF_MARK(i) { const long long _t = clock64(); _pa[i] += _t - _pt; _pt = _t; }
#define CI_PROF_FLUSH if (tid == 0) { for (int _i = 0; _i < 4; ++_i) atomicAdd(&g_profi[_i], (unsigned long long)_pa[_i]); atomicAdd(&g_profi[4], 1ull); }
#else
#define CI_PROF_DECL
#define CI_PROF_MARK(i)
#define CI_PROF_FLUSH
#endif

struct ConvImgParams {
    const bf16_t* x;
    const bf16_t* w;
    const bf16_t* bias;
    bf16_t* y;
    int B, H, W, Cin, Cout, dil, relu;
    int n_cot;
    int xcd_map;
    int n_pxt;
    int Ho, Wo, stride, pad;
    int xC, xslices, out_f32;
    const float* bias32;
    float oscale;
};


template <int BM, int KS, int NPB, bool X3 = false>
__global__ __launch_bounds__(CI_THREADS, 1) void conv_image_kernel(ConvImgParams p) {
#if defined(__HIP_DEVICE_COMPILE__)
    __shared__ __attribute__((aligned(1024))) unsigned char lds[CI_LDS];
    constexpr unsigned OOB = 0x80000000u;
    const int tid = threadIdx.x, lane = tid & 63;
    const int wave = __builtin_amdgcn_readfirstlane(tid >> 6);
    constexpr int NCB = BM / 64;
    constexpr int WCH = BM / 2;
    constexpr int NFP = BM / 64;
    constexpr int NT = KS * KS;

    const int wm = wave & 1, wn = wave >> 1;
    const int r31 = lane & 31, khalf = lane >> 5;
    const u32 lds0 = (u32)(uintptr_t)(__attribute__((address_space(3))) unsigned char*)lds;
    const int HW = p.H * p.W, HWo = p.Ho * p.Wo;

    int b, ct;
    const int tpi = p.n_cot * p.n_pxt;
    if (p.xcd_map) {
        const int xcd = (int)blockIdx.x & 7, j = (int)blockIdx.x >> 3;
        ct = j % tpi;
        b = xcd + 8 * (j / tpi);
    } else {
        b = (int)blockIdx.x / tpi;
        ct = (int)blockIdx.x - b * tpi;
    }
    if (b >= p.B) return;
    const int pt = ct / p.n_cot;
    ct -= pt * p.n_cot;
    const int px0 = pt * (128 * NPB);
    const int npx = (KS == 1 && p.n_pxt > 1) ? min(HW - px0, 128 * NPB) : HW;
    const int co0 = ct * BM;
    const int n_slices = p.Cin >> 6, n_steps = n_slices * NT;
    constexpr int SR = (KS == 1 && NPB == 1) ? 3 : 7;

    CI_PROF_DECL
    if (tid < 2 * (CI_ROW / 4)) reinterpret_cast<u32*>(lds + (tid / (CI_ROW / 4)) * CI_SLAB + CI_ZERO)[tid % (CI_ROW / 4)] = 0u;
    if (tid >= 128 && tid < 128 + BM) {
        if constexpr (X3) reinterpret_cast<float*>(lds + CI_BIAS)[tid - 128] = p.bias32 ? p.bias32[co0 + tid - 128] : 0.f;
        else reinterpret_cast<float*>(lds + CI_BIAS)[tid - 128] = p.bias ? __uint_as_float((u32)p.bias[co0 + tid - 128] << 16) : 0.f;
    }
    const int XC = X3 ? p.xC : p.Cin;
    const i32x4 rx = tile_rsrc(p.x + ((size_t)b * HW + px0) * XC, (u32)((size_t)npx * XC * 2));
    const i32x4 rw = tile_rsrc(p.w + (size_t)co0 * NT * p.Cin, (u32)((size_t)BM * NT * p.Cin * 2));

    u32 wrel[NFP];
#pragma unroll
    for (int i = 0; i < NFP; ++i) {
        const int row = (NFP * wave + i) * 8 + (lane >> 3);
        const int j = (lane & 7) ^ ((row >> 1) & 7);
        wrel[i] = (u32)((row * NT * p.Cin) * 2 + j * 16);
    }
    auto issue_slab = [&](const int slice, const int t, const int buf) {
        const int piece = t * 8 + wave, n = piece * 64 + lane;
        const int px = n / 9, c = n - 9 * px;
        const bool ok = (slice < n_slices) & (px < npx) & (c < 8);
        const bool any = (slice < n_slices) & (piece * 64 < 9 * npx);
        const int xs = (X3 && slice >= p.xslices) ? slice - p.xslices : slice;
        tile_dma16(ok ? (u32)((px * XC + xs * 64) * 2 + c * 16) : OOB, rx,
                   wave_uniform(any ? lds0 + buf * CI_SLAB + piece * 1024 : lds0 + CI_DUMP));
    };
    auto issue_filter_piece = [&](const int i, const int wstep, const int stage) {
        const bool wok = wstep < n_steps;
        const int ws = wstep / NT, wt = wstep - NT * ws;
        const u32 wo = (u32)((wt * p.Cin + ws * 64) * 2);
        tile_dma16(wok ? wrel[i] + wo : OOB, rw,
                   wave_uniform(wok ? lds0 + CI_W0 + stage * CI_WST + (NFP * wave + i) * 1024 : lds0 + CI_DUMP));
    };
    auto issue_filters = [&](const int wstep, const int stage) {
#pragma unroll
        for (int i = 0; i < NFP; ++i) issue_filter_piece(i, wstep, stage);
    };

    u32 abase[4];
    {
        const int row = wm * WCH + r31;
#pragma unroll
        for (int kk = 0; kk < 4; ++kk) abase[kk] = (u32)(CI_W0 + row * 128 + (((2 * kk + khalf) ^ ((row >> 1) & 7)) << 4));
    }
    u32 baddr[NT][NPB];
#pragma unroll
    for (int pi = 0; pi < NPB; ++pi) {
        const int q = px0 + wn * (32 * NPB) + pi * 32 + r31;
// ... 48 lines not shown
                __builtin_amdgcn_sched_barrier(0);
                if (kk < 3) { read_a(stage_off, kk + 1, (kk + 1) & 1); read_b(t, kk + 1, (kk + 1) & 1); }
                else if (t < NT - 1) read_b(t + 1, 0, 0);
                __builtin_amdgcn_sched_barrier(0);
#pragma unroll
                for (int pi = 0; pi < NPB; ++pi) {
                    if constexpr (X3) acc[0][pi] = __builtin_amdgcn_mfma_f32_32x32x16_f16(__builtin_bit_cast(f16x8, fa[kk & 1][0]), __builtin_bit_cast(f16x8, fb[kk & 1][pi]), acc[0][pi], 0, 0, 0);
                    else acc[0][pi] = __builtin_amdgcn_mfma_f32_32x32x16_bf16(fa[kk & 1][0], fb[kk & 1][pi], acc[0][pi], 0, 0, 0);
                }
                __builtin_amdgcn_sched_barrier(0);
                if constexpr (KS == 3) {
                    if (kk < NFP) issue_filter_piece(kk, s * NT + t + 2, stage_p2);
                    if (kk == NFP) issue_slab(s + 1, t, (s + 1) & 1);
                } else if constexpr (SR == 7) {
                    if (kk < 3) { issue_slab(s + 1, 2 * kk, (s + 1) & 1); issue_slab(s + 1, 2 * kk + 1, (s + 1) & 1); }
                    else {
                        issue_slab(s + 1, 6, (s + 1) & 1);
#pragma unroll
                        for (int i = 0; i < NFP; ++i) issue_filter_piece(i, s + 2, stage_p2);
                    }
                } else {
                    if (kk < 3) issue_slab(s + 1, kk, (s + 1) & 1);
                    else {
#pragma unroll
                        for (int i = 0; i < NFP; ++i) issue_filter_piece(i, s + 2, stage_p2);
                    }
                }
                __builtin_amdgcn_sched_barrier(0);
                if constexpr (NCB == 2) {
#pragma unroll
                    for (int pi = 0; pi < NPB; ++pi) {
                        if constexpr (X3) acc[1][pi] = __builtin_amdgcn_mfma_f32_32x32x16_f16(__builtin_bit_cast(f16x8, fa[kk & 1][1]), __builtin_bit_cast(f16x8, fb[kk & 1][pi]), acc[1][pi], 0, 0, 0);
                        else acc[1][pi] = __builtin_amdgcn_mfma_f32_32x32x16_bf16(fa[kk & 1][1], fb[kk & 1][pi], acc[1][pi], 0, 0, 0);
                    }
                }
            }
            if constexpr (KS == 1) stg = stg == CI_NW - 1 ? 0 : stg + 1;
        }
        const u32 flip = (s & 1) ? (u32)(-CI_SLAB) : (u32)CI_SLAB;
#pragma unroll
        for (int t = 0; t < NT; ++t)
#pragma unroll
            for (int pi = 0; pi < NPB; ++pi) baddr[t][pi] += flip;
    }

    CI_PROF_MARK(2)
    asm volatile("s_waitcnt vmcnt(0)" ::: "memory");
    if constexpr (X3) {
#pragma unroll
        for (int ci = 0; ci < NCB; ++ci)
#pragma unroll
            for (int pi = 0; pi < NPB; ++pi) {
                const int q = px0 + wn * (32 * NPB) + pi * 32 + r31;
#pragma unroll
                for (int g = 0; g < 4; ++g) {
                    const int chl = wm * WCH + ci * 32 + 8 * g + 4 * khalf;
                    const float4 b4 = *reinterpret_cast<const float4*>(lds + CI_BIAS + chl * 4);
                    const float bv[4] = {b4.x, b4.y, b4.z, b4.w};
                    float v[4];
#pragma unroll
                    for (int e = 0; e < 4; ++e) {
                        float t = acc[ci][pi][4 * g + e] * p.oscale + bv[e];
                        if (p.relu) t = t > 0.f ? t : (t != t ? t : 0.f);
                        v[e] = t;
                    }
                    if (q >= HWo) continue;
                    const size_t pix = (size_t)b * HWo + q;
                    if (p.out_f32) {
                        *reinterpret_cast<float4*>(reinterpret_cast<float*>(p.y) + pix * p.Cout + co0 + chl) = make_float4(v[0], v[1], v[2], v[3]);
                    } else {
                        u32 l0, l1;
                        const u32 h0 = split2_f16(v[0], v[1], l0), h1 = split2_f16(v[2], v[3], l1);
                        bf16_t* row = p.y + pix * (2 * p.Cout) + co0 + chl;
                        *reinterpret_cast<uint2*>(row) = make_uint2(h0, h1);
                        *reinterpret_cast<uint2*>(row + p.Cout) = make_uint2(l0, l1);
                    }
                }
            }
        CI_PROF_MARK(3)
        CI_PROF_FLUSH
        return;
    }
    const u32 floor16 = p.relu ? 0u : 0x80008000u;
    const size_t img = (size_t)HWo * p.Cout * 2;
    const __amdgpu_buffer_rsrc_t ry = __builtin_amdgcn_make_buffer_rsrc(reinterpret_cast<unsigned char*>(p.y) + (size_t)b * img, 0, (int)img, 0x00020000);
#pragma unroll
    for (int ci = 0; ci < NCB; ++ci) {
        float bv[16];
#pragma unroll
        for (int g = 0; g < 4; ++g) {
            const float4 t4 = *reinterpret_cast<const float4*>(lds + CI_BIAS + (wm * WCH + ci * 32 + 8 * g + 4 * khalf) * 4);
            bv[4 * g] = t4.x; bv[4 * g + 1] = t4.y; bv[4 * g + 2] = t4.z; bv[4 * g + 3] = t4.w;
        }
#pragma unroll
        for (int pi = 0; pi < NPB; ++pi) {
            const int q = px0 + wn * (32 * NPB) + pi * 32 + r31;
            const u32 voff = (u32)((q * p.Cout + co0 + wm * WCH + ci * 32) * 2 + khalf * 16) | (q < HWo ? 0u : OOB);
            u32 lo[4], hi[4];
#pragma unroll
            for (int g = 0; g < 4; ++g) {
                lo[g] = pkmax_i16(pack2_bf16(acc[ci][pi][4 * g] + bv[4 * g], acc[ci][pi][4 * g + 1] + bv[4 * g + 1]), floor16);
                hi[g] = pkmax_i16(pack2_bf16(acc[ci][pi][4 * g + 2] + bv[4 * g + 2], acc[ci][pi][4 * g + 3] + bv[4 * g + 3]), floor16);
            }
#pragma unroll
            for (int pr = 0; pr < 2; ++pr) {
                const auto sl = __builtin_amdgcn_permlane32_swap(lo[2 * pr], lo[2 * pr + 1], false, false);
                const auto sh = __builtin_amdgcn_permlane32_swap(hi[2 * pr], hi[2 * pr + 1], false, false);
                __builtin_amdgcn_raw_buffer_store_b128(u32x4{sl[0], sh[0], sl[1], sh[1]}, ry, voff + pr * 32, 0, 0);
            }
        }
    }
    CI_PROF_MARK(3)
    CI_PROF_FLUSH
#endif
}

}

using namespace ssdhip;

static void ci_pick_tiles(int B, int HW, int Kc, int Cout, int ksize, int stride, int padding, int HWo, int& bm, int& n_pxt) {
    bm = ((Cout % 128) == 0 && (long long)B * (Cout / 128) >= 192) ? 128 : 64;
    if (const char* e = getenv("SSDHIP_CONVIMG_BM")) { const int v = atoi(e); if (v == 64 || (v == 128 && (Cout % 128) == 0)) bm = v; }
    n_pxt = 1;
    const char* e = getenv("SSDHIP_CONVIMG_PXT");
    if (ksize != 1 || stride != 1 || padding != 0 || HWo <= 128 || (e && atoi(e) == 0) || getenv("SSDHIP_CONVIMG_BM")) return;
    int n_cu = 256;
    { int dev = 0, n = 0; if (hipGetDevice(&dev) == hipSuccess && hipDeviceGetAttribute(&n, hipDeviceAttributeMultiprocessorCount, dev) == hipSuccess && n > 0) n_cu = n; }
    auto cost = [&](long long tiles, long long px, long long co) { return ((tiles + n_cu - 1) / n_cu) * (px + co) * Kc * 2; };
    long long best = cost((long long)B * (Cout / bm), HW, bm);
    const int npt = (HWo + 127) / 128;
    for (int co = 128; co >= 64; co -= 64) {
        if (Cout % co) continue;
        const long long c = cost((long long)B * (Cout / co) * npt, 128, co);
        if (c < best) { best = c; bm = co; n_pxt = npt; }
    }
}

extern "C" int ssdhip_conv2d_image_nhwc_bf16(const void* x, const void* weight, const void* bias, void* y, int B, int H, int W, int Cin,
                                             int Cout, int ksize, int stride, int padding, int dilation, int relu, void* stream_) {
    hipStream_t stream = static_cast<hipStream_t>(stream_);
    if (!x || !weight || !y || B <= 0 || H <= 0 || W <= 0 || Cin <= 0 || Cout <= 0) return SSDHIP_E_BADARG;
    if ((ksize != 1 && ksize != 3) || stride < 1 || stride > 4 || dilation < 1 || dilation > 16 || padding < 0 ||
        padding > dilation * (ksize / 2))
        return SSDHIP_E_BADARG;
    if ((Cin % 64) || (Cout % 64) || (long long)H * W > CI_PX) return SSDHIP_E_BADARG;
    const int Ho = (H + 2 * padding - dilation * (ksize - 1) - 1) / stride + 1, Wo = (W + 2 * padding - dilation * (ksize - 1) - 1) / stride + 1;
    if (H + 2 * padding < dilation * (ksize - 1) + 1 || W + 2 * padding < dilation * (ksize - 1) + 1 || Ho < 1 || Wo < 1 ||
        (long long)Ho * Wo > CI_PX)
        return SSDHIP_E_BADARG;
    if (((uintptr_t)x | (uintptr_t)weight | (uintptr_t)y) & 15 || ((uintptr_t)bias & 1)) return SSDHIP_E_BADARG;
    if ((long long)H * W * (Cin > Cout ? Cin : Cout) * 2 >= 0x7ffff000LL || 128LL * 9 * Cin * 2 >= 0x7ffff000LL) return SSDHIP_E_BADARG;
    ConvImgParams p;
    p.x = static_cast<const bf16_t*>(x); p.w = static_cast<const bf16_t*>(weight); p.bias = static_cast<const bf16_t*>(bias);
    p.y = static_cast<bf16_t*>(y);
    p.B = B; p.H = H; p.W = W; p.Cin = Cin; p.Cout = Cout; p.dil = dilation; p.relu = relu ? 1 : 0;
    p.Ho = Ho; p.Wo = Wo; p.stride = stride; p.pad = padding;
    p.xC = Cin; p.xslices = Cin / 64; p.out_f32 = 0; p.bias32 = nullptr; p.oscale = 1.f;
    int bm;
    ci_pick_tiles(B, H * W, Cin, Cout, ksize, stride, padding, Ho * Wo, bm, p.n_pxt);
    p.n_cot = Cout / bm;
    const dim3 grid((unsigned)(B * p.n_cot * p.n_pxt)), block(CI_THREADS);
    p.xcd_map = (B % 8 == 0) ? 1 : 0;
    const bool small = (Ho * Wo <= 128 && (ksize == 3 || H * W <= 128)) || p.n_pxt > 1;
#define CI_LAUNCH(BM_, KS_, NPB_) hipLaunchKernelGGL((conv_image_kernel<BM_, KS_, NPB_>), grid, block, 0, stream, p)
    if (ksize == 3) {
        if (bm == 128) { if (small) CI_LAUNCH(128, 3, 1); else CI_LAUNCH(128, 3, 3); }
        else { if (small) CI_LAUNCH(64, 3, 1); else CI_LAUNCH(64, 3, 3); }
    } else {
        if (bm == 128) { if (small) CI_LAUNCH(128, 1, 1); else CI_LAUNCH(128, 1, 3); }
        else { if (small) CI_LAUNCH(64, 1, 1); else CI_LAUNCH(64, 1, 3); }
    }
#undef CI_LAUNCH
    return hipGetLastError() == hipSuccess ? SSDHIP_OK : SSDHIP_E_LAUNCH;
}

extern "C" int ssdhip_conv2d_image_x3_nhwc_f16(const void* x, const void* weight, const float* bias, void* y, int B, int H, int W, int C,
                                               int Cout, int ksize, int stride, int padding, int dilation, int relu, int out_f32,
                                               float oscale, void* stream_) {
    hipStream_t stream = static_cast<hipStream_t>(stream_);
    if (!x || !weight || !y || B <= 0 || H <= 0 || W <= 0 || C <= 0 || Cout <= 0) return SSDHIP_E_BADARG;
    if ((ksize != 1 && ksize != 3) || stride < 1 || stride > 4 || dilation < 1 || dilation > 16 || padding < 0 ||
        padding > dilation * (ksize / 2))
        return SSDHIP_E_BADARG;
    if ((C % 64) || (Cout % 64) || (long long)H * W > CI_PX) return SSDHIP_E_BADARG;
    const int Ho = (H + 2 * padding - dilation * (ksize - 1) - 1) / stride + 1, Wo = (W + 2 * padding - dilation * (ksize - 1) - 1) / stride + 1;
    if (H + 2 * padding < dilation * (ksize - 1) + 1 || W + 2 * padding < dilation * (ksize - 1) + 1 || Ho < 1 || Wo < 1 ||
        (long long)Ho * Wo > CI_PX)
        return SSDHIP_E_BADARG;
    if (((uintptr_t)x | (uintptr_t)weight | (uintptr_t)y) & 15 || ((uintptr_t)bias & 3)) return SSDHIP_E_BADARG;
    if ((long long)H * W * 3 * (C > Cout ? C : Cout) * 4 >= 0x7ffff000LL || 128LL * 9 * 3 * C * 2 >= 0x7ffff000LL) return SSDHIP_E_BADARG;
    ConvImgParams p;
    p.x = static_cast<const bf16_t*>(x); p.w = static_cast<const bf16_t*>(weight); p.bias = nullptr;
    p.y = static_cast<bf16_t*>(y);
    p.B = B; p.H = H; p.W = W; p.Cin = 3 * C; p.Cout = Cout; p.dil = dilation; p.relu = relu ? 1 : 0;
    p.Ho = Ho; p.Wo = Wo; p.stride = stride; p.pad = padding;
    p.xC = 2 * C; p.xslices = C / 64; p.out_f32 = out_f32 ? 1 : 0; p.bias32 = bias; p.oscale = oscale;
    int bm;
    ci_pick_tiles(B, H * W, 3 * C, Cout, ksize, stride, padding, Ho * Wo, bm, p.n_pxt);
    p.n_cot = Cout / bm;
    const dim3 grid((unsigned)(B * p.n_cot * p.n_pxt)), block(CI_THREADS);
    p.xcd_map = (B % 8 == 0) ? 1 : 0;
    const bool small = (Ho * Wo <= 128 && (ksize == 3 || H * W <= 128)) || p.n_pxt > 1;
#define CI_LAUNCH3(BM_, KS_, NPB_) hipLaunchKernelGGL((conv_image_kernel<BM_, KS_, NPB_, true>), grid, block, 0, stream, p)
    if (ksize == 3) {
        if (bm == 128) { if (small) CI_LAUNCH3(128, 3, 1); else CI_LAUNCH3(128, 3, 3); }
        else { if (small) CI_LAUNCH3(64, 3, 1); else CI_LAUNCH3(64, 3, 3); }
    } else {
        if (bm == 128) { if (small) CI_LAUNCH3(128, 1, 1); else CI_LAUNCH3(128, 1, 3); }
        else { if (small) CI_LAUNCH3(64, 1, 1); else CI_LAUNCH3(64, 1, 3); }
    }
#undef CI_LAUNCH3
    return hipGetLastError() == hipSuccess ? SSDHIP_OK : SSDHIP_E_LAUNCH;
}

extern "C" int ssdhip_conv3x3_image_nhwc_bf16(const void* x, const void* weight, const void* bias, void* y, int B, int H, int W, int Cin,
                                              int Cout, int dilation, int relu, void* stream_) {
    return ssdhip_conv2d_image_nhwc_bf16(x, weight, bias, y, B, H, W, Cin, Cout, 3, 1, dilation, dilation, relu, stream_);
}

#ifdef SSDHIP_PROFILE
extern "C" int ssdhip_profile_read_convimg(unsigned long long* host_out, int reset) {
    if (hipMemcpyFromSymbol(host_out, HIP_SYMBOL(g_profi), sizeof(g_profi)) != hipSuccess) return -1;
    if (reset) { unsigned long long z[8] = {0}; if (hipMemcpyToSymbol(HIP_SYMBOL(g_profi), z, sizeof(z)) != hipSuccess) return -1; }
    return 0;
}
#endif
```

### ssd_keras_amd/csrc/ssdhip_layers.hip

```cpp
#include <hip/hip_runtime.h>
#include <stdint.h>

#include "ssdhip.h"
#include "ssdhip_math.h"
#include "ssdhip_bf16.h"
#include "ssdhip_heads.h"

namespace ssdhip {

__device__ __forceinline__ u32 bias_act2(u32 x, u32 b, bool relu) {
    u32 lo = bf16_bits(bf16_float(x & 0xffffu) + bf16_float(b & 0xffffu));
    u32 hi = bf16_bits(bf16_float(x >> 16) + bf16_float(b >> 16));
    if (relu) {
        if ((lo & 0x8000u) && (lo & 0x7fffu) <= 0x7f80u) lo = 0;
        if ((hi & 0x8000u) && (hi & 0x7fffu) <= 0x7f80u) hi = 0;
    }
    return lo | (hi << 16);
}
__device__ __forceinline__ uint4 bias_act8(uint4 x, uint4 b, bool relu) {
    return make_uint4(bias_act2(x.x, b.x, relu), bias_act2(x.y, b.y, relu), bias_act2(x.z, b.z, relu), bias_act2(x.w, b.w, relu));
}
__device__ __forceinline__ u32 bfmax1(u32 a, u32 b) {
    const float fa = bf16_float(a), fb = bf16_float(b);
    return (fa > fb || fa != fa) ? a : b;
}
__device__ __forceinline__ u32 bfmax2(u32 a, u32 b) { return bfmax1(a & 0xffffu, b & 0xffffu) | (bfmax1(a >> 16, b >> 16) << 16); }
__device__ __forceinline__ uint4 bfmax8(uint4 a, uint4 b) { return make_uint4(bfmax2(a.x, b.x), bfmax2(a.y, b.y), bfmax2(a.z, b.z), bfmax2(a.w, b.w)); }

__global__ __launch_bounds__(256) void bias_act_kernel(const uint4* __restrict__ x, const uint4* __restrict__ bias,
                                                       uint4* __restrict__ y, u32 nvec, u32 cvec, int relu) {
    const u32 stride = gridDim.x * 256u;
    for (u32 i0 = blockIdx.x * 256u + threadIdx.x; i0 < nvec; i0 += 4u * stride) {
        uint4 v[4];
#pragma unroll
        for (int u = 0; u < 4; ++u) { const u32 i = i0 + u * stride; if (i < nvec) v[u] = x[i]; }
#pragma unroll
        for (int u = 0; u < 4; ++u) {
            const u32 i = i0 + u * stride;
            if (i < nvec) y[i] = bias_act8(v[u], bias ? bias[i % cvec] : make_uint4(0, 0, 0, 0), relu != 0);
        }
    }
}

__global__ __launch_bounds__(256) void bias_act_maxpool_kernel(const uint4* __restrict__ x, const uint4* __restrict__ bias,
                                                               uint4* __restrict__ y, int B, int H, int W, u32 cvec, int k, int s,
                                                               int p, int Ho, int Wo, int relu) {
    const u32 total = (u32)B * Ho * Wo * cvec;
    for (u32 i = blockIdx.x * 256u + threadIdx.x; i < total; i += gridDim.x * 256u) {
        const u32 cg = i % cvec;
        u32 t = i / cvec;
        const int wo = t % Wo; t /= Wo;
        const int ho = t % Ho;
        const int b = t / Ho;
        const int h0 = max(ho * s - p, 0), h1 = min(ho * s - p + k, H);
        const int w0 = max(wo * s - p, 0), w1 = min(wo * s - p + k, W);
        const uint4 bv = bias ? bias[cg] : make_uint4(0, 0, 0, 0);
        uint4 best = make_uint4(0xff80ff80u, 0xff80ff80u, 0xff80ff80u, 0xff80ff80u);
        if (k == 3 && s == 1) {
            uint4 v[9];
            bool in[9];
#pragma unroll
            for (int dh = 0; dh < 3; ++dh)
#pragma unroll
                for (int dw = 0; dw < 3; ++dw) {
                    const int hi = ho - p + dh, wi = wo - p + dw;
                    in[dh * 3 + dw] = hi >= 0 && hi < H && wi >= 0 && wi < W;
                    const int hc = min(max(hi, 0), H - 1), wc = min(max(wi, 0), W - 1);
                    v[dh * 3 + dw] = x[((size_t)(b * H + hc) * W + wc) * cvec + cg];
                }
#pragma unroll
            for (int q = 0; q < 9; ++q)
                if (in[q]) best = bfmax8(bias_act8(v[q], bv, relu != 0), best);
            y[i] = best;
            continue;
        }
        for (int hi = h0; hi < h1; ++hi)
            for (int wi = w0; wi < w1; ++wi)
                best = bfmax8(bias_act8(x[((size_t)(b * H + hi) * W + wi) * cvec + cg], bv, relu != 0), best);
        y[i] = best;
    }
}

constexpr int POOL3_THREADS = 1024;
typedef unsigned short l_u16x2 __attribute__((ext_vector_type(2)));
__device__ __forceinline__ u32 l_ordered2(u32 v) {
    const u32 mag = v & 0x7fff7fffu;
    const l_u16x2 over = __builtin_elementwise_sub_sat(__builtin_bit_cast(l_u16x2, mag), __builtin_bit_cast(l_u16x2, 0x7f807f80u));
    const l_u16x2 one = __builtin_elementwise_min(over, __builtin_bit_cast(l_u16x2, 0x00010001u));
    v &= ~(__builtin_bit_cast(u32, one) << 15);
    const u32 neg = __builtin_bit_cast(u32, __builtin_bit_cast(s16x2, v) >> 15);
    return v ^ (neg & 0x7fff7fffu);
}
__device__ __forceinline__ u32 l_unordered2(u32 t) {
    const u32 neg = __builtin_bit_cast(u32, __builtin_bit_cast(s16x2, t) >> 15);
    return t ^ (neg & 0x7fff7fffu);
}
__global__ __launch_bounds__(POOL3_THREADS) void pool3x3s1_slab_kernel(const uint4* __restrict__ x, uint4* __restrict__ y, int H, int W,
                                                                       u32 cvec, u32 slabs) {
    extern __shared__ uint4 pool3_tile[];
    const u32 b = blockIdx.x / slabs, slab = blockIdx.x - b * slabs;
    const u32 n = (u32)(H * W) * 8u;
    const size_t base = (size_t)b * (size_t)(H * W) * cvec + slab * 8u;
    for (u32 i = threadIdx.x; i < n; i += POOL3_THREADS) {
        const uint4 v = x[base + (size_t)(i >> 3) * cvec + (i & 7u)];
        pool3_tile[i] = make_uint4(l_ordered2(v.x), l_ordered2(v.y), l_ordered2(v.z), l_ordered2(v.w));
    }
    __syncthreads();
    for (u32 i = threadIdx.x; i < n; i += POOL3_THREADS) {
        const int px = (int)(i >> 3), c = (int)(i & 7u);
        const int h = px / W, w = px - h * W;
        uint4 best = make_uint4(0x80008000u, 0x80008000u, 0x80008000u, 0x80008000u);
#pragma unroll
        for (int dh = -1; dh <= 1; ++dh)
#pragma unroll
            for (int dw = -1; dw <= 1; ++dw) {
                const int hi = h + dh, wi = w + dw;
                const bool in = (hi >= 0) & (hi < H) & (wi >= 0) & (wi < W);
                const uint4 v = pool3_tile[(in ? hi * W + wi : px) * 8 + c];
                best = make_uint4(pkmax_i16(v.x, best.x), pkmax_i16(v.y, best.y), pkmax_i16(v.z, best.z), pkmax_i16(v.w, best.w));
            }
        y[base + (size_t)px * cvec + (u32)c] = make_uint4(l_unordered2(best.x), l_unordered2(best.y), l_unordered2(best.z), l_unordered2(best.w));
    }
}

__global__ __launch_bounds__(256) void l2norm_kernel(const uint4* __restrict__ x, const float* __restrict__ gamma,
                                                     uint4* __restrict__ y, u32 n_pixels, u32 cvec) {
    const u32 lane = threadIdx.x & 63u;
    const u32 wave = (blockIdx.x * 256u + threadIdx.x) >> 6;
    const u32 nwaves = (gridDim.x * 256u) >> 6;
    for (u32 px = wave; px < n_pixels; px += nwaves) {
        const uint4* row = x + (size_t)px * cvec;
        float ss = 0.f;
        for (u32 j = lane; j < cvec; j += 64u) {
            const uint4 v = row[j];
            const u32 w[4] = {v.x, v.y, v.z, v.w};
#pragma unroll
            for (int q = 0; q < 4; ++q) { const float a = bf16_float(w[q] & 0xffffu), c = bf16_float(w[q] >> 16); ss += a * a; ss += c * c; }
        }
        for (int off = 32; off > 0; off >>= 1) ss += __shfl_xor(ss, off);
        const float inv = rsqrtf(fmaxf(ss, 1e-12f));
        for (u32 j = lane; j < cvec; j += 64u) {
            const uint4 v = row[j];
            const u32 w[4] = {v.x, v.y, v.z, v.w};
            u32 o[4];
#pragma unroll
            for (int q = 0; q < 4; ++q) {
                const float g0 = gamma[j * 8 + q * 2], g1 = gamma[j * 8 + q * 2 + 1];
                o[q] = bf16_bits((bf16_float(w[q] & 0xffffu) * inv) * g0) | (bf16_bits((bf16_float(w[q] >> 16) * inv) * g1) << 16);
            }
            y[(size_t)px * cvec + j] = make_uint4(o[0], o[1], o[2], o[3]);
        }
    }
}

__global__ __launch_bounds__(256) void pool2_l2norm_kernel(const uint4* __restrict__ x, const float* __restrict__ gamma, uint4* __restrict__ y_pool,
                                                           uint4* __restrict__ y_norm, int B, int H, int W, int Ho, int Wo) {
    const u32 lane = threadIdx.x & 63u;
    const u32 wave = (blockIdx.x * 256u + threadIdx.x) >> 6;
    const u32 nwaves = (gridDim.x * 256u) >> 6;
    float g[8];
#pragma unroll
    for (int e = 0; e < 8; ++e) g[e] = gamma[lane * 8 + e];
    const u32 total = (u32)B * Ho * Wo;
    for (u32 o = wave; o < total; o += nwaves) {
        const int wo = o % Wo;
        const int ho = (o / Wo) % Ho;
        const int b = o / (Wo * Ho);
        uint4 v[4];
        bool in[4];
#pragma unroll
        for (int q = 0; q < 4; ++q) {
            const int h = 2 * ho + (q >> 1), w = 2 * wo + (q & 1);
            in[q] = h < H && w < W;
            v[q] = in[q] ? x[((size_t)(b * H + h) * W + w) * 64 + lane] : make_uint4(0, 0, 0, 0);
        }
        uint4 best = make_uint4(0xff80ff80u, 0xff80ff80u, 0xff80ff80u, 0xff80ff80u);
#pragma unroll
        for (int q = 0; q < 4; ++q)
            if (in[q]) best = bfmax8(v[q], best);
        y_pool[(size_t)o * 64 + lane] = best;
        float ss[4];
#pragma unroll
        for (int q = 0; q < 4; ++q) {
            const u32 w4[4] = {v[q].x, v[q].y, v[q].z, v[q].w};
            float acc = 0.f;
#pragma unroll
            for (int t = 0; t < 4; ++t) { const float a = bf16_float(w4[t] & 0xffffu), c = bf16_float(w4[t] >> 16); acc += a * a; acc += c * c; }
            ss[q] = acc;
        }
        for (int off = 32; off > 0; off >>= 1) {
#pragma unroll
            for (int q = 0; q < 4; ++q) ss[q] += __shfl_xor(ss[q], off);
        }
#pragma unroll
        for (int q = 0; q < 4; ++q) {
            if (!in[q]) continue;
            const float inv = rsqrtf(fmaxf(ss[q], 1e-12f));
            const u32 w4[4] = {v[q].x, v[q].y, v[q].z, v[q].w};
            u32 r[4];
#pragma unroll
            for (int t = 0; t < 4; ++t)
                r[t] = bf16_bits((bf16_float(w4[t] & 0xffffu) * inv) * g[2 * t]) | (bf16_bits((bf16_float(w4[t] >> 16) * inv) * g[2 * t + 1]) << 16);
            const int h = 2 * ho + (q >> 1), w = 2 * wo + (q & 1);
            y_norm[((size_t)(b * H + h) * W + w) * 64 + lane] = make_uint4(r[0], r[1], r[2], r[3]);
// ... 580 lines not shown
```

### ssd_keras_amd/models/_common.py

```python
from __future__ import annotations

import numpy as np
import torch
from torch import nn
import torch.nn.functional as F

from .. import _native as nat
from ..anchor_math import n_boxes_for
from ..keras_layers.keras_layer_AnchorBoxes import AnchorBoxes
from ..keras_layers.keras_layer_DecodeDetections import DecodeDetections
from ..keras_layers.keras_layer_DecodeDetectionsFast import DecodeDetectionsFast
from ..keras_layers.keras_layer_L2Normalization import L2Normalization
from . import _conv_select as sel
from . import _shadow
from ._graphed import GraphedInference
from ._heads import PredictorHeads
from ._train_fns import (_AssembleTrainFn, _ConvBiasActFn, _ConvBiasActPoolFn, _MaxPoolFn, _PackedHeadFn, _ReluLink,
                         _conv_input_weight_grads)



def conv_out(n, k, s=1, p=0, d=1):
    return (n + 2 * p - d * (k - 1) - 1) // s + 1


def pool_out(n, k, s, p=0, ceil_mode=False):
    if ceil_mode:
        o = -(-(n + 2 * p - k) // s) + 1
        if (o - 1) * s >= n + p:
            o -= 1
        return o
    return (n + 2 * p - k) // s + 1


def he_normal_(module):
    for m in module.modules():
        if isinstance(m, nn.Conv2d):
            nn.init.kaiming_normal_(m.weight, mode='fan_in', nonlinearity='relu')
            if m.bias is not None:
                nn.init.zeros_(m.bias)


def resolve_anchor_config(n_predictor_layers, min_scale, max_scale, scales, aspect_ratios_global,
                          aspect_ratios_per_layer, two_boxes_for_ar1, steps, offsets, variances):
    if aspect_ratios_global is None and aspect_ratios_per_layer is None:
        raise ValueError("`aspect_ratios_global` and `aspect_ratios_per_layer` cannot both be None. At least one needs to be specified.")
    if aspect_ratios_per_layer:
        if len(aspect_ratios_per_layer) != n_predictor_layers:
            raise ValueError("It must be either aspect_ratios_per_layer is None or len(aspect_ratios_per_layer) == {}, but "
                             "len(aspect_ratios_per_layer) == {}.".format(n_predictor_layers, len(aspect_ratios_per_layer)))
    if (min_scale is None or max_scale is None) and scales is None:
        raise ValueError("Either `min_scale` and `max_scale` or `scales` need to be specified.")
    if scales:
        if len(scales) != n_predictor_layers + 1:
            raise ValueError("It must be either scales is None or len(scales) == {}, but len(scales) == {}.".format(
                n_predictor_layers + 1, len(scales)))
    else:
        scales = np.linspace(min_scale, max_scale, n_predictor_layers + 1)
    if len(variances) != 4:
        raise ValueError("4 variance values must be pased, but {} values were received.".format(len(variances)))
    if np.any(np.array(variances) <= 0):
        raise ValueError("All variances must be >0, but the variances given are {}".format(variances))
    if (steps is not None) and (len(steps) != n_predictor_layers):
        raise ValueError("You must provide at least one step value per predictor layer.")
    if (offsets is not None) and (len(offsets) != n_predictor_layers):
        raise ValueError("You must provide at least one offset value per predictor layer.")
    ars = aspect_ratios_per_layer if aspect_ratios_per_layer else [aspect_ratios_global] * n_predictor_layers
    n_boxes = [n_boxes_for(ar, two_boxes_for_ar1) for ar in ars]
    steps = steps if steps is not None else [None] * n_predictor_layers
    offsets = offsets if offsets is not None else [None] * n_predictor_layers
    return list(scales), ars, n_boxes, steps, offsets


class SSDModel(PredictorHeads, nn.Module):

    def __init__(self, image_size, n_classes, mode, l2_regularization, subtract_mean, divide_by_stddev, swap_channels,
                 confidence_thresh, iou_threshold, top_k, nms_max_output_size, coords, normalize_coords):
        super().__init__()
        if mode not in ('training', 'inference', 'inference_fast'):
            raise ValueError("`mode` must be one of 'training', 'inference' or 'inference_fast', but received '{}'.".format(mode))
        self.img_height, self.img_width, self.img_channels = image_size
        self.n_classes = n_classes + 1
        self.mode = mode
        self.l2_regularization = l2_regularization
        self.subtract_mean = subtract_mean
        self.divide_by_stddev = divide_by_stddev
        self.swap_channels = swap_channels
        self.fused_inference = True
        self.fused_training = True
        self.decoder = None
        if mode != 'training':
            layer = DecodeDetections if mode == 'inference' else DecodeDetectionsFast
            self.decoder = layer(confidence_thresh=confidence_thresh, iou_threshold=iou_threshold, top_k=top_k,
                                 nms_max_output_size=nms_max_output_size, coords=coords,
                                 normalize_coords=normalize_coords, img_height=self.img_height,
                                 img_width=self.img_width, name='decoded_predictions')
        self._anchor_cache = {}
        self._packed_heads = {}

    def _fused(self, x, conv=None):
        return (self.fused_inference and x.is_cuda and x.dtype == torch.bfloat16 and not torch.is_grad_enabled()
                and (conv is None or (conv.weight.dtype == torch.bfloat16 and conv.out_channels % 8 == 0)))

    @staticmethod
    def _conv_nobias(conv, x):
        return F.conv2d(x, conv.weight, None, conv.stride, conv.padding, conv.dilation, conv.groups)

    _conv_choice = {}

    def _pick(self, key, candidates):
        mode = sel.switch("CONV")
        if mode in candidates:
            return mode
        prefer = sel.switch("PREFER")
        if prefer and prefer in candidates:
            return prefer
        if mode == "igemm" and "igemm" not in candidates:
            return "miopen"
        hit = SSDModel._conv_choice.get(key)
        if hit is None:
            if mode != "auto_miopen" and len(candidates) > 1 and "miopen" in candidates:
                candidates = {k: v for k, v in candidates.items() if k != "miopen"}
                if len(candidates) == 1:
                    hit = next(iter(candidates))
                    SSDModel._conv_choice[key] = hit
                    return hit
            best, hit, times = None, None, {}
            for name in sorted(candidates, key=lambda n: n == "miopen"):
                fn = candidates[name]
                fn()
                torch.cuda.synchronize()
                a, b = torch.cuda.Event(enable_timing=True), torch.cuda.Event(enable_timing=True)
                if best is not None:
                    a.record()
                    fn()
                    b.record()
                    b.synchronize()
                    if a.elapsed_time(b) > 3.0 * best / 4.0:
                        continue
                t = None
                for _ in range(3):
                    a.record()
                    for _ in range(6):
                        fn()
                    b.record()
                    b.synchronize()
                    t = a.elapsed_time(b) if t is None else min(t, a.elapsed_time(b))
                times[name] = t
                if best is None or t < best:
                    best, hit = t, name
            if key and key[0] == "act" and hit in ("igemm", "miopen"):
                near = [(times[name], name) for name in ("halo", "image", "igemm6", "igemm5")
                        if name in times and times[name] <= 1.08 * best]
                if near:
# ... 22 lines not shown
            if len(cands) == 1:
                return cands["miopen"]()
            name = sel.untimed_choice(g, relu) or self._pick(sel.act_key(g, relu), cands)
            return cands[name]()
        if self._fused_train(x, conv):
            run, _name = self._train_thunk(conv, x, relu)
            if run is not None:
                wb, bb, wt = self._bf16_shadow(conv, with_transposed=True)
                return _ConvBiasActFn.apply(x, conv.weight, conv.bias, run, conv.stride, conv.padding, conv.dilation, relu, wb, bb, wt,
                                            link_in, link_out)
        y = conv(x)
        return F.relu(y) if relu else y

    def _fused_train(self, x, conv):
        return (self.fused_training and x.is_cuda and torch.is_grad_enabled() and conv.bias is not None and conv.groups == 1
                and (x.dtype == torch.bfloat16 or (torch.is_autocast_enabled() and torch.get_autocast_dtype("cuda") == torch.bfloat16)))


    def _bf16_shadow(self, conv, with_transposed=False):
        if conv.weight.dtype == torch.bfloat16:
            return (conv.weight.detach(), conv.bias.detach(), None) if with_transposed else (conv.weight.detach(), conv.bias.detach())
        st = _shadow.fresh(self, conv.weight.device)
        i = st.index.get(id(conv))
        if i is None:
            return (None, None, None) if with_transposed else (None, None)
        if with_transposed:
            packed = st.tr_arg[i][0] != conv.out_channels
            return st.cl[i], st.bias[i], (None if packed else st.tr[i])
        return st.cl[i], st.bias[i]

    def _packed_head_shadow(self, l):
        ch = self.conf_heads[l]
        if ch.weight.dtype == torch.bfloat16:
            return None
        return _shadow.fresh(self, ch.weight.device).packs.get(l)

    def _train_thunk(self, conv, x, relu):
        g = sel.geometry_of(conv, x)
        if sel.first_layer(g):
            return (lambda xb, wb, bb: nat.conv3x3_cin3(xb, wb, bb, relu=relu)), "cin3"
        cands = sel.candidates(g, relu, sel.TRAINING)
        if not cands:
            return None, None
        key = sel.act_key(g, relu)
        forced = sel.switch("CONV")
        if len(cands) == 1:
            name = "igemm"
        elif forced in cands:
            name = forced
        elif SSDModel._conv_choice.get(key) in cands:
            name = SSDModel._conv_choice[key]
        else:
            with torch.no_grad():
                xb = x.detach().to(torch.bfloat16).contiguous(memory_format=torch.channels_last)
                wb = conv.weight.detach().to(torch.bfloat16).contiguous(memory_format=torch.channels_last)
                bb = conv.bias.detach().to(torch.bfloat16)
                name = self._pick(key, {n: (lambda fn=fn: fn(xb, wb, bb)) for n, fn in cands.items()})
            if name not in cands:
                name = "igemm"
        return cands[name], name

    @staticmethod
    def relu_link():
        return _ReluLink() if torch.is_grad_enabled() else None


    def conv_act_pool(self, conv, x, kernel, stride, pad=0, ceil_mode=False, link_in=None):
        if self._fused(x, conv):
            cands = {"miopen": lambda: nat.bias_act_maxpool(self._conv_nobias(conv, x), conv.bias, kernel, stride, pad, ceil_mode,
                                                            relu=True)}
            for name, fn in sel.pooled_candidates(sel.geometry_of(conv, x), kernel, stride, pad, ceil_mode).items():
                cands[name] = lambda fn=fn: fn(x, conv.weight, conv.bias)
            name = (self._pick(("pool", tuple(x.shape), conv.out_channels, conv.kernel_size[0], conv.dilation[0], kernel, stride, pad),
                               cands) if len(cands) > 1 else "miopen")
            return cands[name]()
        if (kernel == 2 and stride == 2 and pad == 0 and ceil_mode and self._fused_train(x, conv) and conv.out_channels % 8 == 0
                and 256 % (conv.out_channels // 8) == 0 and not sel.on("NO_FUSED_POOL_BWD")):
            run, _name = self._train_thunk(conv, x, True)
            if run is not None:
                wb, bb, wt = self._bf16_shadow(conv, with_transposed=True)
                return _ConvBiasActPoolFn.apply(x, conv.weight, conv.bias, run, conv.stride, conv.padding, conv.dilation, wb, bb, wt, link_in)
        return self.max_pool(self.conv_act(conv, x, relu=True, link_in=link_in), kernel, stride, pad, ceil_mode=ceil_mode)

    def conv1_block_pool(self, c1, c2, x):
        same3 = lambda c: (c.kernel_size == (3, 3) and c.stride == (1, 1) and c.padding == (1, 1) and c.dilation == (1, 1)
                           and c.groups == 1 and c.bias is not None)
        if (not sel.on("NO_CONV1_BLOCK") and sel.switch("CONV") in ("auto", "auto_miopen")
                and self._fused(x, c1) and self._fused(x, c2) and same3(c1) and same3(c2)
                and c1.in_channels == 3 and c1.out_channels == 64
                and c2.in_channels == 64 and c2.out_channels % 64 == 0):
            cands = {"separate": lambda: self.conv_act_pool(c2, self.conv_act(c1, x), 2, 2, ceil_mode=True),
                     "conv1_block": lambda: nat.conv1_block(x, c1.weight, c1.bias, c2.weight, c2.bias, relu=True, pool=True)}
            key = ("conv1_block", tuple(x.shape), c2.out_channels)
            if SSDModel._conv_choice.get(key) is None:
                cands["separate"]()
            name = self._pick(key, cands)
            return cands[name if name in cands else "separate"]()
        return self.conv_act_pool(c2, self.conv_act(c1, x), 2, 2, ceil_mode=True)

    def max_pool(self, x, kernel, stride, pad=0, ceil_mode=False):
        if self._fused(x) and x.shape[1] % 8 == 0:
            return nat.bias_act_maxpool(x, None, kernel, stride, pad, ceil_mode, relu=False)
        if (self.fused_training and x.is_cuda and x.dtype == torch.bfloat16 and torch.is_grad_enabled() and x.shape[1] % 8 == 0
                and x.requires_grad and not sel.on("NO_OWN_POOL")):
            return _MaxPoolFn.apply(x, kernel, stride, pad, ceil_mode)
        return F.max_pool2d(x, kernel, stride, pad, ceil_mode=ceil_mode)

    def preprocess(self, images):
        x = images
        if x.dim() != 4:
            raise ValueError("expected images of shape (batch, height, width, channels)")
        nhwc = x.shape[-1] == self.img_channels and x.shape[1] != self.img_channels
        if (nhwc and self.fused_inference and x.is_cuda and x.dtype == torch.float32 and x.is_contiguous()
                and not torch.is_grad_enabled() and self.img_channels <= 4
                and next(self.parameters()).dtype == torch.bfloat16):
            return nat.preprocess(x, self.subtract_mean, self.divide_by_stddev,
                                  list(self.swap_channels) if self.swap_channels else None)
        if (nhwc and self.fused_training and x.is_cuda and x.dtype == torch.float32 and x.is_contiguous() and torch.is_grad_enabled()
                and not x.requires_grad and self.img_channels <= 4 and torch.is_autocast_enabled()
                and torch.get_autocast_dtype("cuda") == torch.bfloat16 and not sel.on("NO_TRAIN_PREPROCESS")):
            return nat.preprocess(x, self.subtract_mean, self.divide_by_stddev,
                                  list(self.swap_channels) if self.swap_channels else None)
        if nhwc:
            x = x.permute(0, 3, 1, 2)
        x = x.float()
        if self.subtract_mean is not None:
            x = x - self._device_const("mean", x.device, lambda: torch.as_tensor(self.subtract_mean, dtype=torch.float32).view(1, -1, 1, 1))
        if self.divide_by_stddev is not None:
            x = x / self._device_const("std", x.device, lambda: torch.as_tensor(self.divide_by_stddev, dtype=torch.float32).view(1, -1, 1, 1))
        if self.swap_channels:
            x = x.index_select(1, self._device_const("swap", x.device, lambda: torch.as_tensor(list(self.swap_channels), dtype=torch.long)))
        return x.contiguous(memory_format=torch.channels_last)

    def _device_const(self, name, device, build):
        key = ("const", name, str(device))
        t = self._anchor_cache.get(key)
        if t is None:
            t = build().to(device)
            self._anchor_cache[key] = t
        return t

    def anchors_and_variances(self, feature_sizes, device):
        key = (tuple(feature_sizes), str(device))
        t = self._anchor_cache.get(key)
        if t is None:
            t = torch.cat([pb.constant(h, w, device).reshape(-1, 8) for pb, (h, w) in zip(self.priorboxes, feature_sizes)], dim=0)
            self._anchor_cache[key] = t
        return t

    def predictor_sizes(self):
        raise NotImplementedError

    def precise(self, enable=True, check_finite=True):
        if not enable:
            self.__dict__["_precise"] = None
            return self
        from .precise import PreciseForward
        self.__dict__["_precise"] = PreciseForward(self, check_finite=check_finite)
        return self

    def raw_predictions(self, images, decode=False):
        pf = self.__dict__.get("_precise")
        if (pf is not None and images.is_cuda and not torch.is_grad_enabled() and next(self.parameters()).dtype == torch.float32):
            return pf(images, decode=bool(decode and self.decoder is not None))
        self.__dict__["_shadow_fresh"] = False
        self.__dict__["_in_forward"] = True
        try:
            return self._raw_predictions(images, decode)
        finally:
            self.__dict__["_in_forward"] = False

    def _raw_predictions(self, images, decode):
        x = self.preprocess(images)
        dtype = next(self.parameters()).dtype
        xin = x.to(dtype) if not torch.is_autocast_enabled() else x
        split = self._split_heads(xin)
        if split is not None:
            feats, confs = split
            sizes = [(f.shape[2], f.shape[3]) for f in feats]
            anchors = self.anchors_and_variances(sizes, x.device)
            head_args = (confs, [None] * len(confs), [ch.bias for ch in self.conf_heads], [lh.bias for lh in self.loc_heads],
                         [pb.n_boxes for pb in self.priorboxes], anchors, self.n_classes)
            if decode and self.decoder is not None and self.n_classes <= 81:
                return self.decoder.forward_from_heads(*head_args)
            pred = nat.assemble_predictions(*head_args)
            return self.decoder(pred) if (decode and self.decoder is not None) else pred
        feats = self.features(xin)
        b = x.shape[0]
        sizes = [(f.shape[2], f.shape[3]) for f in feats]
        if all(self._fused_head_ok(f, ch) for f, ch in zip(feats, self.conf_heads)):
            packable = all(self._packed_head_ok(ch, lh, f) for f, ch, lh in zip(feats, self.conf_heads, self.loc_heads))
            how = "per_layer"
            if packable and len(feats) <= 8:
                hc = {"per_layer": lambda: self._heads_per_layer(feats), "grouped": lambda: self._heads_grouped(feats)}
                if self._halo_heads_ok(feats):
                    hc["halo_grouped"] = lambda: self._heads_halo_grouped(feats)
                elif self._halo_heads_mixed_ok(feats):
                    hc["halo_mixed"] = lambda: self._heads_halo_mixed(feats)
                how = self._pick(("heads", tuple(tuple(f.shape) for f in feats), self.n_classes), hc)
            confs, locs = (self._heads_halo_grouped(feats) if how == "halo_grouped" else
                           self._heads_halo_mixed(feats) if how == "halo_mixed" else
                           self._heads_grouped(feats) if how == "grouped" else self._heads_per_layer(feats))
            anchors = self.anchors_and_variances(sizes, x.device)
            head_args = (confs, locs, [ch.bias for ch in self.conf_heads], [lh.bias for lh in self.loc_heads],
                         [pb.n_boxes for pb in self.priorboxes], anchors, self.n_classes)
            if decode and self.decoder is not None and self.n_classes <= 81:
                return self.decoder.forward_from_heads(*head_args)
            pred = nat.assemble_predictions(*head_args)
            return self.decoder(pred) if (decode and self.decoder is not None) else pred
        if (torch.is_grad_enabled() and not decode and not sel.on("NO_TRAIN_ASSEMBLY") and len(feats) <= 8
                and all(self._packed_train_head_ok(f, ch, lh) for f, ch, lh in zip(feats, self.conf_heads, self.loc_heads))
                and self._train_assembly_fits(len(feats))):
            ys = []
            for l, (f, ch, lh) in enumerate(zip(feats, self.conf_heads, self.loc_heads)):
                pw, pb, pwt, _nc, _nl = self._packed_head_shadow(l)
                ys.append(_PackedHeadFn.apply(f, ch.weight, ch.bias, lh.weight, lh.bias, pw, pb, pwt))
            anchors = self.anchors_and_variances(sizes, x.device)
            return _AssembleTrainFn.apply(anchors, self.n_classes, [pb_.n_boxes for pb_ in self.priorboxes], *ys)
        confs, locs = [], []
        for f, ch, lh in zip(feats, self.conf_heads, self.loc_heads):
            if self._packed_train_head_ok(f, ch, lh):
                pw, pb, pwt, _nc, _nl = self._packed_head_shadow(len(confs))
                y = _PackedHeadFn.apply(f, ch.weight, ch.bias, lh.weight, lh.bias, pw, pb, pwt).permute(0, 2, 3, 1)
                confs.append(y[..., :ch.out_channels].reshape(b, -1, self.n_classes))
                locs.append(y[..., ch.out_channels:ch.out_channels + lh.out_channels].reshape(b, -1, 4))
                continue
            confs.append(ch(f).permute(0, 2, 3, 1).reshape(b, -1, self.n_classes))
            locs.append(lh(f).permute(0, 2, 3, 1).reshape(b, -1, 4))
        conf = torch.softmax(torch.cat(confs, dim=1).float(), dim=-1)
        loc = torch.cat(locs, dim=1).float()
        anchors = self.anchors_and_variances(sizes, conf.device)
        pred = torch.cat([conf, loc, anchors.unsqueeze(0).expand(b, -1, -1)], dim=2)
        return self.decoder(pred) if (decode and self.decoder is not None) else pred

    def _derived_weights_key(self):
        gammas = tuple((m.gamma.data_ptr(), m.gamma._version) for m in self.modules()
                       if isinstance(m, L2Normalization) and m.gamma is not None)
        return self._head_weights_key() + gammas

    def _refresh_derived_weights(self):
        self._refresh_packed_heads()
        for m in self.modules():
            if isinstance(m, L2Normalization):
                m.refresh_cached_gamma()

    def _fused_head_ok(self, f, conv):
        return (self.fused_inference and f.is_cuda and f.dtype == torch.bfloat16 and not torch.is_grad_enabled()
                and conv.weight.dtype == torch.bfloat16)

    def forward(self, images):
        return self.raw_predictions(images, decode=self.decoder is not None)

    def head_outputs(self, images):
        if torch.is_grad_enabled():
            raise RuntimeError("head_outputs is an inference-path probe: call it under torch.no_grad()")
        self.__dict__["_shadow_fresh"] = False
        self.__dict__["_in_forward"] = True
        had = self.__dict__.get("_head_overlap")
        if not had:
            self.__dict__["_head_overlap"] = "4"
        try:
            x = self.preprocess(images)
            split = self._split_heads(x.to(next(self.parameters()).dtype))
            if split is None:
                raise RuntimeError("head_outputs: this model / input does not take the fused inference path")
            return list(split[1])
        finally:
            self.__dict__["_head_overlap"] = had
            self.__dict__["_in_forward"] = False

    def graphed(self, images, warmup=3, heads_only=False):
        return GraphedInference(self, images, warmup, fn=self.head_outputs if heads_only else None)

    predict = forward

    def l2_regularization_loss(self):
        if not self.l2_regularization:
            return torch.zeros((), device=next(self.parameters()).device)
        return self.l2_regularization * sum((m.weight.float() ** 2).sum() for m in self.modules() if isinstance(m, nn.Conv2d))


def make_priorboxes(img_height, img_width, scales, aspect_ratios, two_boxes_for_ar1, steps, offsets, clip_boxes,
                    variances, coords, normalize_coords, names):
    return nn.ModuleList([
        AnchorBoxes(img_height, img_width, this_scale=scales[i], next_scale=scales[i + 1], aspect_ratios=aspect_ratios[i],
                    two_boxes_for_ar1=two_boxes_for_ar1, this_steps=steps[i], this_offsets=offsets[i],
                    clip_boxes=clip_boxes, variances=variances, coords=coords, normalize_coords=normalize_coords,
                    name=names[i])
        for i in range(len(names))])
```

### ssd_keras_amd/models/_conv_select.py

```python
import os
from collections import namedtuple

from .. import _native as nat

SWITCHES = {
    "CONV": "auto", "PREFER": None, "GEMM_1X1": "0", "IMAGE2": "1",
    "NO_HALO": "0", "NO_IMAGE": "0", "NO_SPLITK": "0", "NO_CONV1_BLOCK": "0", "NO_CHAIN": "0", "NO_POOL_NORM": "0",
    "NO_HALO_MIXED": "0", "HEAD_OVERLAP": None, "GRAPH_HEAD_OVERLAP": "4", "HEAD_SPLIT": "3", "HEAD_WGS": None, "SIDE_PRIORITY": "0",
    "NO_OWN_DGRAD": "0", "NO_OWN_WGRAD": "0", "NO_TAPS_BWD": "0", "NO_MASKED_DGRAD": "0", "NO_MASKED_SUMS": "0", "NO_C64_DGRAD": "0",
    "NO_CONV1_1_BWD": "0", "NO_POOL_KEEP": "0", "NO_HALO_POOL_KEEP": "0", "NO_FUSED_POOL_BWD": "0", "NO_OWN_POOL": "0",
    "NO_TRAIN_PREPROCESS": "0", "NO_TRAIN_ASSEMBLY": "0", "NO_OWN_HEADS": "0",
}


def switch(name):
    return os.environ.get("SSDHIP_" + name, SWITCHES[name])


def on(name):
    return switch(name) == "1"


def autotuned():
    return switch("CONV") in ("auto", "auto_miopen") and not switch("PREFER")


Geometry = namedtuple("Geometry", "batch h w cin cout k stride padding dilation groups bias")
_Shape = namedtuple("_Shape", "shape")


def _square(kh, kw, stride, padding, dilation):
    return (kh == kw and isinstance(padding, tuple) and stride[0] == stride[1] and padding[0] == padding[1] and dilation[0] == dilation[1])


def geometry_of(conv, x=None):
    if not _square(*conv.kernel_size, conv.stride, conv.padding, conv.dilation) or conv.padding_mode != 'zeros':
        return None
    b, _, h, w = x.shape if x is not None else (0, 0, 0, 0)
    return Geometry(b, h, w, conv.in_channels, conv.out_channels, conv.kernel_size[0], conv.stride[0],
                    conv.padding[0], conv.dilation[0], conv.groups, int(conv.bias is not None))


def geometry_of_grads(wb, xb, stride, padding, dilation):
    if not _square(wb.shape[2], wb.shape[3], stride, tuple(padding), dilation):
        return None
    return Geometry(xb.shape[0], xb.shape[2], xb.shape[3], wb.shape[1], wb.shape[0], wb.shape[2], stride[0], padding[0], dilation[0], 1, 1)


def out_side(n, g):
    return (n + 2 * g.padding - g.dilation * (g.k - 1) - 1) // g.stride + 1


def first_layer(g):
    return g is not None and g[3:] == (3, 64, 3, 1, 1, 1, 1, 1)


def igemm(g):
    return (g is not None and g.k in (1, 3) and g.stride == 1 and g.groups == 1 and g.padding == g.dilation * (g.k // 2)
            and g.cin % 64 == 0 and g.cout % 64 == 0 and bool(g.bias))


def igemm_general(g):
    return (g is not None and g.k in (1, 3) and 1 <= g.stride <= 4 and g.groups == 1 and 0 <= g.padding <= g.dilation * (g.k // 2)
            and g.cin % 64 == 0 and g.cout % 64 == 0 and bool(g.bias))


def few_tiles(m_pixels, cout):
    return -(-m_pixels // 128) * -(-cout // 128) <= 100


def splitk_measured_regime(g):
    return g.batch >= 16 and g.h * g.w <= 32 * 32


def halo(g):
    return g.k == 3 and g.dilation == 1 and g.cin % 128 == 0 and g.cout % 128 == 0 and not on("NO_HALO")


def halo_strided(g):
    return (halo(g) and g.stride in (1, 2) and g.padding in (0, 1) and g.w <= 94 and g.h + 2 * g.padding >= 3 and g.w + 2 * g.padding >= 3)


def c64(g):
    return g.cin == 64 and g.k == 3 and g.dilation == 1


def _half_a_chip(g):
    return g.batch * (g.cout // 64) >= 128


def image(g):
    return (g.k == 3 and g.h * g.w <= 384 and g.cin % 64 == 0 and g.cout % 64 == 0 and 1 <= g.dilation <= 16 and _half_a_chip(g)
            and not on("NO_IMAGE"))


def image2(g):
    if switch("IMAGE2") == "0" or on("NO_IMAGE") or g.groups != 1:
        return False
    return _half_a_chip(g) and nat.conv2d_image_supported(_Shape((g.batch, g.cin, g.h, g.w)), _Shape((g.cout, g.cin, g.k, g.k)), g.stride,
                                                          g.padding, g.dilation)


def own_dgrad(g):
    return g is not None and g.groups == 1 and (dgrad_same(g) or dgrad_embedded(g))


def dgrad_same(g):
    return g.stride == 1 and g.k in (1, 3) and g.padding == g.dilation * (g.k // 2) and g.cin % 64 == 0 and g.cout % 64 == 0


def dgrad_embedded(g):
    return (not dgrad_same(g) and g.k == 3 and g.dilation == 1 and g.padding in (0, 1) and g.cin % 64 == 0 and g.cout % 64 == 0)


def dgrad_geometry(g):
    return g._replace(cin=g.cout, cout=g.cin, stride=1, padding=g.dilation * (g.k // 2))


INFERENCE, POOLED, TRAINING, DGRAD = "inference", "pooled", "training", "dgrad"
_EVERYWHERE = (INFERENCE, POOLED, TRAINING, DGRAD)
_UNPOOLED = (INFERENCE, TRAINING, DGRAD)
DGRAD_PRIORITY = ("image", "halo", "c64", "igemm")
UNTIMED_PRIORITY = ("image", "splitk")


def _forms(g, relu, context):
    if igemm(g):
        d, p = g.dilation, g.padding
        pixels = g.batch * g.h * g.w
        return (
            ("igemm", _EVERYWHERE, True, False, lambda x, w, b: nat.conv2d_same(x, w, b, dilation=d, relu=relu)),
            ("igemm6", (INFERENCE, POOLED, TRAINING), True, False, lambda x, w, b: nat.conv2d_same(x, w, b, dilation=d, relu=relu, variant=6)),
            ("igemm5", (INFERENCE,), pixels <= 128 * 128, False, lambda x, w, b: nat.conv2d_same(x, w, b, dilation=d, relu=relu, variant=5)),
            ("splitk", (INFERENCE,), few_tiles(pixels, g.cout), splitk_measured_regime(g) and not on("NO_SPLITK"),
             lambda x, w, b: nat.conv2d(x, w, b, stride=1, padding=p, dilation=d, relu=relu, variant=8)),
            ("c64", _UNPOOLED, c64(g) and not (context == DGRAD and on("NO_C64_DGRAD")), False,
             lambda x, w, b: nat.conv3x3_c64(x, w, b, relu=relu, pool=False)),
            ("halo", _EVERYWHERE, halo(g), False, lambda x, w, b: nat.conv2d_same(x, w, b, dilation=1, relu=relu, variant=7)),
            ("image", _EVERYWHERE, image(g), False, lambda x, w, b: nat.conv3x3_image(x, w, b, dilation=d, relu=relu)),
            ("image", _UNPOOLED, g.k == 1 and image2(g), True, lambda x, w, b: nat.conv2d_image(x, w, b, relu=relu)),
        )
    if igemm_general(g):
        d, s, p = g.dilation, g.stride, g.padding
        general = lambda v: (lambda x, w, b: nat.conv2d(x, w, b, stride=s, padding=p, dilation=d, relu=relu, variant=v))
        return (
            ("igemm", (INFERENCE, TRAINING), True, False, general(None)),
            ("igemm5", (INFERENCE, TRAINING), True, False, general(5)),
            ("igemm6", (INFERENCE, TRAINING), True, False, general(6)),
            ("splitk", (INFERENCE,), few_tiles(g.batch * out_side(g.h, g) * out_side(g.w, g), g.cout),
             splitk_measured_regime(g) and not on("NO_SPLITK"), general(8)),
            ("halo", (INFERENCE,), halo_strided(g), False,
             lambda x, w, b: nat.conv2d(x, w, b, stride=s, padding=p, dilation=1, relu=relu, variant=7)),
            ("image", (INFERENCE, TRAINING), image2(g), True,
             lambda x, w, b: nat.conv2d_image(x, w, b, stride=s, padding=p, dilation=d, relu=relu)),
        )
    return ()


def candidates(g, relu, context):
    return {name: fn for name, contexts, ok, _untimed, fn in _forms(g, relu, context) if ok and context in contexts}


def untimed_choice(g, relu):
    if not (autotuned() and g.batch >= 16):
        return None
    untimed = {name for name, contexts, ok, untimed, _fn in _forms(g, relu, INFERENCE) if ok and untimed and INFERENCE in contexts}
    return next((name for name in UNTIMED_PRIORITY if name in untimed), None)


def pooled_candidates(g, kernel, stride, pad, ceil_mode):
    pool = lambda fn: (lambda x, w, b: nat.bias_act_maxpool(fn(x, w, b), None, kernel, stride, pad, ceil_mode, relu=False))
    cands = {name: pool(fn) for name, fn in candidates(g, True, POOLED).items()}
    if cands and kernel == 2 and stride == 2 and pad == 0 and (ceil_mode or (g.h % 2 == 0 and g.w % 2 == 0)):
        cands["igemm_pool"] = lambda x, w, b: nat.conv2d_same_pool2(x, w, b, dilation=g.dilation, relu=True)
        if halo(g):
            cands["halo_pool"] = lambda x, w, b: nat.conv3x3_halo(x, w, b, relu=True, pool=True)
        if c64(g):
            cands["c64_pool"] = lambda x, w, b: nat.conv3x3_c64(x, w, b, relu=True, pool=True)
    return cands


def act_key(g, relu):
    return ("act", (g.batch, g.cin, g.h, g.w), g.cout, g.k, g.dilation, relu, g.stride, g.padding)
```

### ssd_keras_amd/models/keras_ssd300.py

```python
from __future__ import annotations

import numpy as np
import torch
from torch import nn

from .. import _native as nat

from ..keras_layers.keras_layer_L2Normalization import L2Normalization
from ._conv_select import on
from ._common import SSDModel, conv_out, he_normal_, make_priorboxes, pool_out, resolve_anchor_config


class _VGGBase(SSDModel):

    def _build_vgg(self, in_ch):
        def c(i, o, k=3, **kw):
            return nn.Conv2d(i, o, k, padding=kw.pop('padding', k // 2), **kw)
        self.conv1_1, self.conv1_2 = c(in_ch, 64), c(64, 64)
        self.conv2_1, self.conv2_2 = c(64, 128), c(128, 128)
        self.conv3_1, self.conv3_2, self.conv3_3 = c(128, 256), c(256, 256), c(256, 256)
        self.conv4_1, self.conv4_2, self.conv4_3 = c(256, 512), c(512, 512), c(512, 512)
        self.conv5_1, self.conv5_2, self.conv5_3 = c(512, 512), c(512, 512), c(512, 512)
        self.fc6 = nn.Conv2d(512, 1024, 3, padding=6, dilation=6)
        self.fc7 = nn.Conv2d(1024, 1024, 1)
        self.conv4_3_norm = L2Normalization(gamma_init=20, n_channels=512, name='conv4_3_norm')

    def _vgg_to_conv4_3(self, x):
        ca, cap = self.conv_act, self.conv_act_pool
        x = self.conv1_block_pool(self.conv1_1, self.conv1_2, x)
        l2, l31, l32, l41, l42 = (self.relu_link() for _ in range(5))
        x = cap(self.conv2_2, ca(self.conv2_1, x, link_out=l2), 2, 2, ceil_mode=True, link_in=l2)
        x = cap(self.conv3_3, ca(self.conv3_2, ca(self.conv3_1, x, link_out=l31), link_in=l31, link_out=l32), 2, 2, ceil_mode=True, link_in=l32)
        return ca(self.conv4_3, ca(self.conv4_2, ca(self.conv4_1, x, link_out=l41), link_in=l41, link_out=l42), link_in=l42)

    def _vgg_from_pool4(self, x):
        ca, cap = self.conv_act, self.conv_act_pool
        x = cap(self.conv5_3, ca(self.conv5_2, ca(self.conv5_1, x)), 3, 1, pad=1)
        return ca(self.fc7, ca(self.fc6, x))

    def _vgg_from_conv4_3(self, conv4_3):
        return self._vgg_from_pool4(self.max_pool(conv4_3, 2, 2, ceil_mode=True))

    def _vgg(self, x):
        conv4_3 = self._vgg_to_conv4_3(x)
        return conv4_3, self._vgg_from_conv4_3(conv4_3)

    def _trunk(self, x):
        conv4_3 = self._vgg_to_conv4_3(x)
        norm = self.conv4_3_norm
        if (self._fused(conv4_3) and conv4_3.shape[1] == 512 and norm.fused_inference and norm.gamma is not None
                and not torch.is_grad_enabled() and not on("NO_POOL_NORM")):
            pooled, normed = nat.pool2_l2_normalize(conv4_3, norm.gamma_float32())
            return [normed, self._vgg_from_pool4(pooled)]
        return [norm(conv4_3), self._vgg_from_conv4_3(conv4_3)]

    @staticmethod
    def _vgg_sizes(n):
        for _ in range(3):
            n = pool_out(n, 2, 2, ceil_mode=True)
        c43 = n
        n = pool_out(n, 2, 2, ceil_mode=True)
        return c43, n


class SSD300(_VGGBase):
    SOURCE_CHANNELS = (512, 1024, 512, 256, 256, 256)
    NAMES = ('conv4_3_norm', 'fc7', 'conv6_2', 'conv7_2', 'conv8_2', 'conv9_2')

    def __init__(self, image_size, n_classes, mode, l2_regularization, scales, aspect_ratios, n_boxes, steps, offsets,
                 two_boxes_for_ar1, clip_boxes, variances, coords, normalize_coords, subtract_mean, divide_by_stddev,
                 swap_channels, confidence_thresh, iou_threshold, top_k, nms_max_output_size):
        super().__init__(image_size, n_classes, mode, l2_regularization, subtract_mean, divide_by_stddev, swap_channels,
                         confidence_thresh, iou_threshold, top_k, nms_max_output_size, coords, normalize_coords)
        self._build_vgg(self.img_channels)
        self.conv6_1, self.conv6_2 = nn.Conv2d(1024, 256, 1), nn.Conv2d(256, 512, 3, stride=2, padding=1)
        self.conv7_1, self.conv7_2 = nn.Conv2d(512, 128, 1), nn.Conv2d(128, 256, 3, stride=2, padding=1)
        self.conv8_1, self.conv8_2 = nn.Conv2d(256, 128, 1), nn.Conv2d(128, 256, 3)
        self.conv9_1, self.conv9_2 = nn.Conv2d(256, 128, 1), nn.Conv2d(128, 256, 3)
        self.conf_heads = nn.ModuleList([nn.Conv2d(ch, nb * self.n_classes, 3, padding=1)
                                         for ch, nb in zip(self.SOURCE_CHANNELS, n_boxes)])
        self.loc_heads = nn.ModuleList([nn.Conv2d(ch, nb * 4, 3, padding=1) for ch, nb in zip(self.SOURCE_CHANNELS, n_boxes)])
        self.priorboxes = make_priorboxes(self.img_height, self.img_width, scales, aspect_ratios, two_boxes_for_ar1, steps,
                                          offsets, clip_boxes, variances, coords, normalize_coords,
                                          [n + '_mbox_priorbox' for n in self.NAMES])
        he_normal_(self)

    def trunk_features(self, x):
        return self._trunk(x)

    def extra_features(self, fc7):
        return self.extra_features_tail(self.extra_features_front(fc7))

    def extra_features_front(self, fc7):
        return self.conv_act(self.conv6_2, self.conv_act(self.conv6_1, fc7))

    def extra_features_tail(self, conv6_2):
        ca = self.conv_act
        tail = self._extras_tail_chain(conv6_2)
        if tail is not None:
            return [conv6_2] + tail
        conv7_2 = ca(self.conv7_2, ca(self.conv7_1, conv6_2))
        conv8_2 = ca(self.conv8_2, ca(self.conv8_1, conv7_2))
        conv9_2 = ca(self.conv9_2, ca(self.conv9_1, conv8_2))
        return [conv6_2, conv7_2, conv8_2, conv9_2]

    def _extras_tail_chain(self, conv6_2, _refresh_only=False):
        if not _refresh_only and (not self._fused(conv6_2) or on("NO_CHAIN")):
            return None
        convs = self._tail_convs()
        key = self._tail_chain_key() + (str(conv6_2.device),)
        st = self.__dict__.get("_tail_chain")
        if st is None or st["key"] != key:
            old = st["layers"] if (st is not None and st["layers"] is not None and st["key"][-1] == key[-1]) else None
            layers = []
            with torch.no_grad():
                for i, c in enumerate(convs):
                    wb = c.weight.detach().to(torch.bfloat16).contiguous(memory_format=torch.channels_last)
                    if old is not None:
                        packed = nat.conv_chain_pack(wb, out=old[i]["packed"])
                        bias = old[i]["bias"]
# ... 65 lines not shown
```

Before: 16710 images/sec.

## Fuse f32 preprocessing into conv1 block and fuse conv5_3 with 3x3 pool

Adds a conv1 block variant that reads raw f32 NHWC images directly and applies the mean subtraction, channel swap and bf16 conversion while staging patches into LDS. This removes the separate preprocess kernel and its bf16 intermediate write and read. It also adds an image-conv kernel with a fused 3x3/stride-1 max pool for conv5_3, chosen by autotuning against the separate path. The cost is more complex load paths with doubled input bytes per pixel, and a placeholder tensor that carries the deferred raw images.

```diff
diff --git a/include/ssdhip.h b/include/ssdhip.h
--- a/include/ssdhip.h
+++ b/include/ssdhip.h
@@ -245,6 +245,9 @@
 
 int ssdhip_conv1_block_nhwc_bf16(const void* x3, const void* w1, const void* b1, const void* weight, const void* bias, void* y,
                                  int B, int H, int W, int Cout, int relu, int pool, int n_workgroups, void* stream);
+int ssdhip_conv1_block_f32_nhwc_bf16(const float* images, int channels, const float* mean_h, const float* divide_h, const int* swap_h,
+                                     const void* w1, const void* b1, const void* weight, const void* bias, void* y, int B, int H, int W,
+                                     int Cout, int relu, int pool, int n_workgroups, void* stream);
 
 int ssdhip_conv3x3_cin3_nhwc_bf16(const void* x, const void* weight, const void* bias, void* y, int B, int H, int W,
                                   int Cin, int Cout, int relu, void* stream);
@@ -292,6 +295,8 @@
                                    int dilation, int relu, void* stream);
 int ssdhip_conv2d_image_nhwc_bf16(const void* x, const void* weight, const void* bias, void* y, int B, int H, int W, int Cin, int Cout,
                                   int ksize, int stride, int padding, int dilation, int relu, void* stream);
+int ssdhip_conv3x3_image_pool3_nhwc_bf16(const void* x, const void* weight, const void* bias, void* y, int B, int H, int W, int Cin,
+                                         int Cout, int dilation, int relu, void* stream);
 int ssdhip_conv2d_image_x3_nhwc_f16(const void* x, const void* weight, const float* bias, void* y, int B, int H, int W, int C, int Cout,
                                     int ksize, int stride, int padding, int dilation, int relu, int out_f32, float oscale, void* stream);
 
diff --git a/ssd_keras_amd/_native.py b/ssd_keras_amd/_native.py
--- a/ssd_keras_amd/_native.py
+++ b/ssd_keras_amd/_native.py
@@ -130,6 +130,7 @@
     "ssdhip_conv3x3_halo_strided_nhwc_bf16": (_I, [_P] * 4 + [_I] * 8 + [_P]),
     "ssdhip_conv3x3_halo_group_nhwc_bf16": (_I, [_I] + [_P] * 9 + [_I, _I, _P]),
     "ssdhip_conv1_block_nhwc_bf16": (_I, [_P] * 6 + [_I] * 7 + [_P]),
+    "ssdhip_conv1_block_f32_nhwc_bf16": (_I, [_P, _I] + [_P] * 8 + [_I] * 7 + [_P]),
     "ssdhip_conv3x3_cin3_nhwc_bf16": (_I, [_P] * 4 + [_I] * 6 + [_P]),
     "ssdhip_conv_bn_elu_pack_bytes": (_SZ, [_I] * 3),
     "ssdhip_conv_bn_elu_nhwc_bf16": (_I, [_P] * 5 + [_I] * 7 + [_P]),
@@ -151,6 +152,7 @@
     "ssdhip_image_lut_u8": (_I, [_P, _P, _LL, _I, _I, _P, _P]),
     "ssdhip_conv3x3_image_nhwc_bf16": (_I, [_P] * 4 + [_I] * 7 + [_P]),
     "ssdhip_conv2d_image_nhwc_bf16": (_I, [_P] * 4 + [_I] * 10 + [_P]),
+    "ssdhip_conv3x3_image_pool3_nhwc_bf16": (_I, [_P] * 4 + [_I] * 7 + [_P]),
     "ssdhip_conv2d_image_x3_nhwc_f16": (_I, [_P] * 4 + [_I] * 11 + [_F, _P]),
     "ssdhip_shadow_refresh": (_I, [_P] + [_I] * 4 + [_P]),
     "ssdhip_sgd_momentum_step": (_I, [_I] + [_P] * 4 + [_D] * 3 + [_P]),
@@ -843,6 +845,19 @@
     wt = weight if weight.permute(0, 2, 3, 1).is_contiguous() else weight.permute(0, 2, 3, 1).contiguous().permute(0, 3, 1, 2)
     y = torch.empty((b, h, w, cout), dtype=torch.bfloat16, device=x.device).permute(0, 3, 1, 2)
     launch("ssdhip_conv3x3_image_nhwc_bf16", x.device, _ptr(x), _ptr(wt), _ptr(bias), _ptr(y), b, h, w, cin, cout, int(dilation),
+           int(bool(relu)))
+    return y
+
+
+def conv3x3_image_pool3(x, weight, bias, dilation=1, relu=True):
+    torch = _torch()
+    x, (b, h, w, cin) = _nhwc_bf16(x, "x")
+    cout, cin_w, kh, kw = weight.shape
+    if weight.dtype != torch.bfloat16 or cin_w != cin or kh != 3 or kw != 3:
+        raise SsdHipError("weight must be bfloat16 (Cout, %d, 3, 3)" % cin)
+    wt = weight if weight.permute(0, 2, 3, 1).is_contiguous() else weight.permute(0, 2, 3, 1).contiguous().permute(0, 3, 1, 2)
+    y = torch.empty((b, h, w, cout), dtype=torch.bfloat16, device=x.device).permute(0, 3, 1, 2)
+    launch("ssdhip_conv3x3_image_pool3_nhwc_bf16", x.device, _ptr(x), _ptr(wt), _ptr(bias), _ptr(y), b, h, w, cin, cout, int(dilation),
            int(bool(relu)))
     return y
 
@@ -1630,6 +1645,43 @@
     return y
 
 
+def conv1_block_f32_supported(images, divide=None):
+    torch = _torch()
+    return (images.is_cuda and images.dtype == torch.float32 and images.dim() == 4 and images.shape[3] == 3 and images.is_contiguous()
+            and divide is None and images.shape[2] % 2 == 0 and images.data_ptr() % 8 == 0)
+
+
+def conv1_block_f32(images, mean, divide, swap, w1, b1, weight, bias, relu=True, pool=False):
+    torch = _torch()
+    require_cuda(images, "images")
+    if images.dtype != torch.float32 or images.dim() != 4:
+        raise SsdHipError("images must be float32 (B, H, W, C)")
+    b, h, w, c = images.shape
+    if tuple(w1.shape) != (64, 3, 3, 3) or weight.shape[1:] != (64, 3, 3) or w1.dtype != torch.bfloat16 or weight.dtype != torch.bfloat16:
+        raise SsdHipError("conv1_block_f32 needs bfloat16 (64, 3, 3, 3) and (Cout, 64, 3, 3) weights")
+    def fa(v):
+        if v is None:
+            return None
+        v = [float(v)] * c if np.isscalar(v) else [float(t) for t in v]
+        if len(v) != c:
+            raise SsdHipError("per-channel constant has %d entries for %d channels" % (len(v), c))
+        return (ctypes.c_float * c)(*v)
+    ia = (ctypes.c_int * c)(*[int(t) for t in swap]) if swap else None
+    cl = lambda t: t if t.permute(0, 2, 3, 1).is_contiguous() else t.permute(0, 2, 3, 1).contiguous().permute(0, 3, 1, 2)
+    w1c, w2c = cl(w1), cl(weight)
+    cout = weight.shape[0]
+    ho, wo = ((h + 1) // 2, (w + 1) // 2) if pool else (h, w)
+    y = torch.empty((b, ho, wo, cout), dtype=torch.bfloat16, device=images.device).permute(0, 3, 1, 2)
+    dev = images.device
+    n_cu = _CU_COUNT.get(dev.index)
+    if n_cu is None:
+        n_cu = torch.cuda.get_device_properties(dev).multi_processor_count
+        _CU_COUNT[dev.index] = n_cu
+    launch("ssdhip_conv1_block_f32_nhwc_bf16", dev, _ptr(images), int(c), fa(mean), fa(divide), ia, _ptr(w1c), _ptr(b1), _ptr(w2c), _ptr(bias),
+           _ptr(y), b, h, w, cout, int(bool(relu)), int(bool(pool)), int(n_cu))
+    return y
+
+
 CONVERSIONS = {"minmax2centroids": 0, "centroids2minmax": 1, "corners2centroids": 2, "centroids2corners": 3,
                "minmax2corners": 4, "corners2minmax": 4}
 
diff --git a/ssd_keras_amd/csrc/ssdhip_bf16.h b/ssd_keras_amd/csrc/ssdhip_bf16.h
--- a/ssd_keras_amd/csrc/ssdhip_bf16.h
+++ b/ssd_keras_amd/csrc/ssdhip_bf16.h
@@ -36,6 +36,20 @@
     return __builtin_bit_cast(u32, __builtin_elementwise_max(__builtin_bit_cast(s16x2, a), __builtin_bit_cast(s16x2, b)));
 }
 
+typedef unsigned short u16x2 __attribute__((ext_vector_type(2)));
+__device__ __forceinline__ u32 ordered2_bf16(u32 v) {
+    const u32 mag = v & 0x7fff7fffu;
+    const u16x2 over = __builtin_elementwise_sub_sat(__builtin_bit_cast(u16x2, mag), __builtin_bit_cast(u16x2, 0x7f807f80u));
+    const u16x2 one = __builtin_elementwise_min(over, __builtin_bit_cast(u16x2, 0x00010001u));
+    v &= ~(__builtin_bit_cast(u32, one) << 15);
+    const u32 neg = __builtin_bit_cast(u32, __builtin_bit_cast(s16x2, v) >> 15);
+    return v ^ (neg & 0x7fff7fffu);
+}
+__device__ __forceinline__ u32 unordered2_bf16(u32 t) {
+    const u32 neg = __builtin_bit_cast(u32, __builtin_bit_cast(s16x2, t) >> 15);
+    return t ^ (neg & 0x7fff7fffu);
+}
+
 __device__ __forceinline__ u32 split2_f16(float a, float b, u32& lo_out) {
     const _Float16 ha = (_Float16)a, hb = (_Float16)b;
     const _Float16 la = (_Float16)(a - (float)ha), lb = (_Float16)(b - (float)hb);
diff --git a/ssd_keras_amd/csrc/ssdhip_conv64.hip b/ssd_keras_amd/csrc/ssdhip_conv64.hip
--- a/ssd_keras_amd/csrc/ssdhip_conv64.hip
+++ b/ssd_keras_amd/csrc/ssdhip_conv64.hip
@@ -60,6 +60,9 @@
     int prio;
     int xcd_pairs;
     bf16_t* y2;
+    const float* x3f;
+    float pre_mean[3];
+    int pre_swap[3];
 };
 
 #if defined(__HIP_DEVICE_COMPILE__)
@@ -82,15 +85,23 @@
     return v;
 }
 
+template <int OFF>
+__device__ __forceinline__ u32x2 c64_load_u64(u32 voff, i32x4 rsrc, u32 soff) {
+    u32x2 v;
+    asm volatile("buffer_load_dwordx2 %0, %1, %2, %3 offen offset:%4" : "=v"(v) : "v"(voff), "s"(rsrc), "s"(soff), "n"(OFF) : "memory");
+    return v;
+}
+
 __device__ __forceinline__ u32 c64_load_u32(u32 voff, i32x4 rsrc, u32 soff) {
     u32 v;
     asm volatile("buffer_load_dword %0, %1, %2, %3 offen" : "=v"(v) : "v"(voff), "s"(rsrc), "s"(soff) : "memory");
     return v;
 }
 
-template <int CS, bool POOL, int NB, bool FRONT, bool WREG, bool KEEP = false>
+template <int CS, bool POOL, int NB, bool FRONT, bool WREG, bool KEEP = false, bool F32IN = false>
 __device__ __forceinline__ void conv64_body(const C64Params& p, unsigned char* lds) {
     static_assert(!KEEP || (POOL && !FRONT), "KEEP is a variant of the pooled, un-fused kernel");
+    static_assert(!F32IN || FRONT, "F32IN is a variant of the fused conv1 block");
     constexpr int CC = 1 << CS, RP = 64 >> CS;
     constexpr int HC = CC + 2, HR = 2 * RP + 2;
     constexpr int HPX = HR * HC;
@@ -181,11 +192,16 @@
             hdst[blk] = (u32)(hpc * 144 + 8 * khalf);
             hcoord[blk] = (u32)((hr << 8) | hc | (hp < HPX ? 0 : 0x10000));
         }
-        const i32x4 r3 = tile_rsrc(p.x3, p.B * p.H * p.W * 6);
+        const i32x4 r3 = F32IN ? tile_rsrc(p.x3f, p.B * p.H * p.W * 12) : tile_rsrc(p.x3, p.B * p.H * p.W * 6);
         auto run = [&](auto widec) {
         constexpr bool WIDE = decltype(widec)::value;
         constexpr int ROWB = PROW * 2, NDW = PATCH / 2, DPR = PROW / 2, NRAWW = (NDW + 63) / 64;
+        constexpr int NPAIR = PATCH / 6, NS = (NPAIR + 63) / 64;
+        static_assert(!F32IN || (WIDE && PC % 2 == 0 && 3 * NS == NRAWW && NS * 64 * 12 <= C64_PATCH1 && NS <= 32),
+                      "pairs tile a patch row; a request stays NRAWW loads; every pair slot stays inside the producer's patch copy");
         constexpr int NR = WIDE ? NRAWW : NRAW;
+        constexpr int NQ = F32IN ? NS : NR;
+        using RawT = std::conditional_t<F32IN, u32x2, u32>;
         static_assert(PROW % 2 == 0 && NRAWW * 64 * 4 <= C64_PATCH1 && (HR + 1) * ROWB + (HC - 1) * 6 + 32 <= C64_PATCH1,
                       "dword patch rows; every raw slot and every fragment read stay inside the producer's patch copy");
         [[maybe_unused]] u32 kofs[2][8];
@@ -217,11 +233,18 @@
                     kofs[st][j] = (u32)(((k / 9) * PROW + (k % 9)) * 2);
                 }
         }
-        u32 rrel[NR], rco[NR];
-#pragma unroll
-        for (int i = 0; i < NR; ++i) {
+        u32 rrel[NQ], rco[NQ];
+        [[maybe_unused]] u32 vbits = 0u;
+#pragma unroll
+        for (int i = 0; i < NQ; ++i) {
             const int n = 64 * i + lane;
-            if constexpr (WIDE) {
+            if constexpr (F32IN) {
+                const int nn = n < NPAIR ? n : 0;
+                const int pr = nn / (PC / 2), cp = nn - pr * (PC / 2);
+                rrel[i] = n < NPAIR ? (u32)((pr * p.W + 2 * cp) * 12) : OOB;
+                rco[i] = (u32)((pr << 16) | ((2 * cp) << 8) | (2 * cp + 1));
+                vbits |= (n < NPAIR ? 1u : 0u) << i;
+            } else if constexpr (WIDE) {
                 const int nn = n < NDW ? n : 0;
                 const int pr = nn / DPR, c4 = nn - pr * DPR;
                 rrel[i] = n < NDW ? (u32)((pr * p.W) * 6 + c4 * 4) : OOB;
@@ -234,11 +257,37 @@
             }
         }
         auto load = [&](u32 voff, u32 soff) { return WIDE ? c64_load_u32(voff, r3, soff) : c64_load_u16(voff, r3, soff); };
-        auto request = [&](int tile, u32 (&raw)[NR]) {
+        auto request = [&](int tile, RawT (&raw)[NR]) -> u32 {
             int b, h0, w0;
             tile_origin(tile, b, h0, w0);
             const int ph = h0 - 2, pw = w0 - 2;
             const bool inside = ph >= 0 && pw >= 0 && ph + PR <= p.H && pw + PC <= p.W;
+            if constexpr (F32IN) {
+                u32 okm = vbits;
+                if (inside) {
+                    const u32 soff = (u32)(((b * p.H + ph) * p.W + pw) * 12);
+#pragma unroll
+                    for (int i = 0; i < NS; ++i) {
+                        raw[3 * i] = c64_load_u64<0>(rrel[i], r3, soff);
+                        raw[3 * i + 1] = c64_load_u64<8>(rrel[i], r3, soff);
+                        raw[3 * i + 2] = c64_load_u64<16>(rrel[i], r3, soff);
+                    }
+                } else {
+                    const int base = ((b * p.H + ph) * p.W + pw) * 12;
+                    okm = 0u;
+#pragma unroll
+                    for (int i = 0; i < NS; ++i) {
+                        const int pr = (int)(rco[i] >> 16), pcs = (int)(rco[i] >> 8) & 0xff;
+                        const bool ok = rrel[i] != OOB && (unsigned)(ph + pr) < (unsigned)p.H && (unsigned)(pw + pcs) < (unsigned)p.W;
+                        const u32 voff = ok ? (u32)(base + (int)rrel[i]) : OOB;
+                        raw[3 * i] = c64_load_u64<0>(voff, r3, 0u);
+                        raw[3 * i + 1] = c64_load_u64<8>(voff, r3, 0u);
+                        raw[3 * i + 2] = c64_load_u64<16>(voff, r3, 0u);
+                        okm |= (ok ? 1u : 0u) << i;
+                    }
+                }
+                return okm;
+            } else
             if (inside) {
                 const u32 soff = (u32)((((b * p.H + ph) * p.W + pw) * 3) * 2);
 #pragma unroll
@@ -253,22 +302,44 @@
                     raw[i] = load(ok ? (u32)(base + (int)rrel[i]) : OOB, 0u);
                 }
             }
+            return 0u;
         };
         C64_PROF_DECL
-        auto landed = [&](u32 (&raw)[NR], bool newer) {
+        auto landed = [&](RawT (&raw)[NR], bool newer) {
             if (newer) asm volatile("s_waitcnt vmcnt(%0)" :: "n"(NR) : "memory");
             else asm volatile("s_waitcnt vmcnt(0)" ::: "memory");
 #pragma unroll
             for (int i = 0; i < NR; ++i) asm volatile("" : "+v"(raw[i]));
         };
-        auto produce = [&](int tile, const u32 (&raw)[NR], int buf) {
+        auto produce = [&](int tile, const RawT (&raw)[NR], [[maybe_unused]] const u32 okm, int buf) {
             int b, h0, w0;
             tile_origin(tile, b, h0, w0);
             unsigned char* hb = lds + H_OFF + buf * HB;
             bf16x8 bfr[MYB][2];
             if constexpr (WIDE) {
+                if constexpr (F32IN) {
+#pragma unroll
+                    for (int i = 0; i < NS; ++i) {
+                        const u32 keep = 0u - ((okm >> i) & 1u);
+                        const u32 vb[6] = {raw[3 * i][0], raw[3 * i][1], raw[3 * i + 1][0], raw[3 * i + 1][1], raw[3 * i + 2][0], raw[3 * i + 2][1]};
+                        u32 o[6];
+#pragma unroll
+                        for (int px = 0; px < 2; ++px)
+#pragma unroll
+                            for (int ch = 0; ch < 3; ++ch) {
+                                const int sc = p.pre_swap[ch];
+                                const float t = __uint_as_float(sc == 0 ? vb[px * 3] : sc == 1 ? vb[px * 3 + 1] : vb[px * 3 + 2]) - p.pre_mean[ch];
+                                o[px * 3 + ch] = bf16_bits(t);
+                            }
+                        u32* dst = reinterpret_cast<u32*>(patch) + 3 * (64 * i + lane);
+                        dst[0] = (o[0] | (o[1] << 16)) & keep;
+                        dst[1] = (o[2] | (o[3] << 16)) & keep;
+                        dst[2] = (o[4] | (o[5] << 16)) & keep;
+                    }
+                } else {
 #pragma unroll
                 for (int i = 0; i < NR; ++i) reinterpret_cast<u32*>(patch)[64 * i + lane] = raw[i];
+                }
 #pragma unroll
                 for (int blk = 0; blk < MYB; ++blk) {
                     const u32* q0 = reinterpret_cast<const u32*>(patch + fadr[blk][0]);
@@ -338,22 +409,22 @@
             else finish(std::true_type{});
             C64_PROF_MARK(3)
         };
-        u32 raw_a[NR], raw_b[NR];
-        request(first, raw_a);
+        RawT raw_a[NR], raw_b[NR];
+        u32 okm_a = request(first, raw_a), okm_b = 0u;
         landed(raw_a, false);
-        produce(first, raw_a, 0);
-        if (first + stride < p.tiles) request(first + stride, raw_a);
+        produce(first, raw_a, okm_a, 0);
+        if (first + stride < p.tiles) okm_a = request(first + stride, raw_a);
         asm volatile("s_waitcnt lgkmcnt(0)" ::: "memory");
         __builtin_amdgcn_s_barrier();
         int buf = 0;
-        auto step = [&](int tile, u32 (&cur)[NR], u32 (&nxt)[NR]) {
+        auto step = [&](int tile, RawT (&cur)[NR], RawT (&nxt)[NR], const u32 okm_cur, u32& okm_nxt) {
             const bool req = !(SSDHIP_C64_ABLATE & 8) && tile + 2 * stride < p.tiles;
-            if (req) request(tile + 2 * stride, nxt);
+            if (req) okm_nxt = request(tile + 2 * stride, nxt);
             C64_PROF_MARK(0)
             if (!(SSDHIP_C64_ABLATE & 8) && tile + stride < p.tiles) {
                 landed(cur, req);
                 C64_PROF_MARK(1)
-                produce(tile + stride, cur, buf ^ 1);
+                produce(tile + stride, cur, okm_cur, buf ^ 1);
             }
             asm volatile("s_waitcnt lgkmcnt(0)" ::: "memory");
             C64_PROF_MARK(4)
@@ -363,13 +434,14 @@
             buf ^= 1;
         };
         for (int tile = first; tile < p.tiles; tile += 2 * stride) {
-            step(tile, raw_a, raw_b);
+            step(tile, raw_a, raw_b, okm_a, okm_b);
             if (tile + stride >= p.tiles) break;
-            step(tile + stride, raw_b, raw_a);
+            step(tile + stride, raw_b, raw_a, okm_b, okm_a);
         }
         if (wave == 4) { C64_PROF_FLUSH(16) }
         };
-        if (!(p.W & 1) && !((uintptr_t)p.x3 & 3)) run(std::true_type{});
+        if constexpr (F32IN) run(std::true_type{});
+        else if (!(p.W & 1) && !((uintptr_t)p.x3 & 3)) run(std::true_type{});
         else run(std::false_type{});
         return;
       }
@@ -609,11 +681,11 @@
 }
 #endif
 
-template <int CS, bool POOL, int NB, bool FRONT = false, bool WREG = false, bool KEEP = false>
+template <int CS, bool POOL, int NB, bool FRONT = false, bool WREG = false, bool KEEP = false, bool F32IN = false>
 __global__ __launch_bounds__(FRONT ? C64_FRONT_THREADS : C64_THREADS, 1) void conv64_kernel(C64Params p) {
 #if defined(__HIP_DEVICE_COMPILE__)
     __shared__ __attribute__((aligned(1024))) unsigned char lds[c64_lds_bytes(CS, NB, FRONT, WREG)];
-    conv64_body<CS, POOL, NB, FRONT, WREG, KEEP>(p, lds);
+    conv64_body<CS, POOL, NB, FRONT, WREG, KEEP, F32IN>(p, lds);
 #endif
 }
 
@@ -679,18 +751,21 @@
     return c64_launch(x, weight, bias, y_pooled, y_full, B, H, W, Cin, Cout, relu, 1, n_workgroups, stream);
 }
 
-extern "C" int ssdhip_conv1_block_nhwc_bf16(const void* x3, const void* w1, const void* b1, const void* weight, const void* bias, void* y,
-                                            int B, int H, int W, int Cout, int relu, int pool, int n_workgroups, void* stream_) {
+static int c64_front_launch(const void* x3, const float* x3f, const float* pre_mean, const int* pre_swap, const void* w1, const void* b1,
+                            const void* weight, const void* bias, void* y, int B, int H, int W, int Cout, int relu, int pool, int n_workgroups,
+                            void* stream_) {
     hipStream_t stream = static_cast<hipStream_t>(stream_);
-    if (!x3 || !w1 || !weight || !y || B <= 0 || H <= 0 || W <= 0 || Cout <= 0 || (Cout % 64)) return SSDHIP_E_BADARG;
+    if ((!x3 && !x3f) || !w1 || !weight || !y || B <= 0 || H <= 0 || W <= 0 || Cout <= 0 || (Cout % 64)) return SSDHIP_E_BADARG;
     if (((uintptr_t)weight | (uintptr_t)y) & 15 || (((uintptr_t)x3 | (uintptr_t)w1 | (uintptr_t)b1 | (uintptr_t)bias) & 1)) return SSDHIP_E_BADARG;
     const long long wb = (long long)Cout * 1152;
-    if ((long long)B * H * W * 6 >= 0x7ffff000LL || wb >= 0x7ffff000LL || (long long)B * H * W * Cout > 0x7fffffff0LL) return SSDHIP_E_BADARG;
+    if ((long long)B * H * W * (x3f ? 12 : 6) >= 0x7ffff000LL || wb >= 0x7ffff000LL || (long long)B * H * W * Cout > 0x7fffffff0LL) return SSDHIP_E_BADARG;
     C64Params p;
     p.x = nullptr; p.w = static_cast<const bf16_t*>(weight); p.bias = static_cast<const bf16_t*>(bias);
     p.y = static_cast<bf16_t*>(y);
     p.x3 = static_cast<const bf16_t*>(x3); p.w1 = static_cast<const bf16_t*>(w1); p.b1 = static_cast<const bf16_t*>(b1);
     p.y2 = nullptr;
+    p.x3f = x3f;
+    for (int c = 0; c < 3; ++c) { p.pre_mean[c] = x3f ? pre_mean[c] : 0.f; p.pre_swap[c] = x3f ? pre_swap[c] : c; }
     { const char* e = getenv("SSDHIP_C64_PRIO"); p.prio = e ? atoi(e) : 3; }
     p.B = B; p.H = H; p.W = W; p.Cout = Cout; p.relu = relu ? 1 : 0;
     p.Ho = (H + 1) / 2; p.Wo = (W + 1) / 2;
@@ -702,6 +777,10 @@
         const long long wt = (W + (1 << cs) - 1) >> cs, ht = (p.Ho + (64 >> cs) - 1) / (64 >> cs);
         if (best < 0 || wt * ht < best) { best = wt * ht; cs_best = cs; p.WT = (int)wt; p.HT = (int)ht; }
     }
+    if (const char* e = getenv("SSDHIP_C64_CS")) {
+        const int cs = atoi(e);
+        if (cs == 3 || cs == 4) { cs_best = cs; p.WT = (W + (1 << cs) - 1) >> cs; p.HT = (p.Ho + (64 >> cs) - 1) / (64 >> cs); }
+    }
     const long long tiles = (long long)B * p.HT * p.WT;
     if (tiles > 0x3fffffffLL) return SSDHIP_E_BADARG;
     p.tiles = (int)tiles;
@@ -711,7 +790,8 @@
     if (G < p.n_slices) G = p.n_slices;
     { const char* e = getenv("SSDHIP_C64_XCD"); p.xcd_pairs = (p.n_slices > 1 && G % (8 * p.n_slices) == 0 && !(e && atoi(e) == 0)) ? 1 : 0; }
     static const bool wreg = []() { const char* e = getenv("SSDHIP_C64_WREG"); return e ? atoi(e) != 0 : true; }();
-#define C64F_LAUNCH(CS_, POOL_) do { if (wreg) hipLaunchKernelGGL((conv64_kernel<CS_, POOL_, 2, true, true>), dim3(G), dim3(C64_FRONT_THREADS), 0, stream, p); \
+#define C64F_LAUNCH(CS_, POOL_) do { if (x3f) hipLaunchKernelGGL((conv64_kernel<CS_, POOL_, 2, true, true, false, true>), dim3(G), dim3(C64_FRONT_THREADS), 0, stream, p); \
+                                     else if (wreg) hipLaunchKernelGGL((conv64_kernel<CS_, POOL_, 2, true, true>), dim3(G), dim3(C64_FRONT_THREADS), 0, stream, p); \
                                      else hipLaunchKernelGGL((conv64_kernel<CS_, POOL_, 2, true>), dim3(G), dim3(C64_FRONT_THREADS), 0, stream, p); } while (0)
     if (pool) {
         if (cs_best == 3) C64F_LAUNCH(3, true); else C64F_LAUNCH(4, true);
@@ -722,6 +802,26 @@
     return hipGetLastError() == hipSuccess ? SSDHIP_OK : SSDHIP_E_LAUNCH;
 }
 
+extern "C" int ssdhip_conv1_block_nhwc_bf16(const void* x3, const void* w1, const void* b1, const void* weight, const void* bias, void* y,
+                                            int B, int H, int W, int Cout, int relu, int pool, int n_workgroups, void* stream) {
+    if (!x3) return SSDHIP_E_BADARG;
+    return c64_front_launch(x3, nullptr, nullptr, nullptr, w1, b1, weight, bias, y, B, H, W, Cout, relu, pool, n_workgroups, stream);
+}
+
+extern "C" int ssdhip_conv1_block_f32_nhwc_bf16(const float* images, int channels, const float* mean_h, const float* divide_h, const int* swap_h,
+                                                const void* w1, const void* b1, const void* weight, const void* bias, void* y, int B, int H,
+                                                int W, int Cout, int relu, int pool, int n_workgroups, void* stream) {
+    if (!images || channels != 3 || divide_h || W <= 0 || (W & 1) || ((uintptr_t)images & 7)) return SSDHIP_E_BADARG;
+    float mean[3];
+    int swap[3];
+    for (int c = 0; c < 3; ++c) {
+        swap[c] = swap_h ? swap_h[c] : c;
+        if (swap[c] < 0 || swap[c] > 2) return SSDHIP_E_BADARG;
+        mean[c] = mean_h ? mean_h[swap[c]] : 0.f;
+    }
+    return c64_front_launch(nullptr, images, mean, swap, w1, b1, weight, bias, y, B, H, W, Cout, relu, pool, n_workgroups, stream);
+}
+
 #ifdef SSDHIP_PROFILE
 extern "C" int ssdhip_profile_read_c64(unsigned long long* host_out, int reset) {
     if (hipMemcpyFromSymbol(host_out, HIP_SYMBOL(g_prof64), sizeof(g_prof64)) != hipSuccess) return -1;
diff --git a/ssd_keras_amd/csrc/ssdhip_convimg.hip b/ssd_keras_amd/csrc/ssdhip_convimg.hip
--- a/ssd_keras_amd/csrc/ssdhip_convimg.hip
+++ b/ssd_keras_amd/csrc/ssdhip_convimg.hip
@@ -50,7 +50,7 @@
 };
 
 
-template <int BM, int KS, int NPB, bool X3 = false>
+template <int BM, int KS, int NPB, bool X3 = false, bool POOL3 = false>
 __global__ __launch_bounds__(CI_THREADS, 1) void conv_image_kernel(ConvImgParams p) {
 #if defined(__HIP_DEVICE_COMPILE__)
     __shared__ __attribute__((aligned(1024))) unsigned char lds[CI_LDS];
@@ -265,6 +265,9 @@
         return;
     }
     const u32 floor16 = p.relu ? 0u : 0x80008000u;
+    constexpr int PITCH = BM * 2 + 16;
+    static_assert(!POOL3 || (KS == 3 && NPB == 3 && !X3 && CI_PX * PITCH <= 2 * CI_SLAB && PITCH % 16 == 0), "the pooled rows fit the two slab buffers");
+    if constexpr (POOL3) __builtin_amdgcn_s_barrier();
     const size_t img = (size_t)HWo * p.Cout * 2;
     const __amdgpu_buffer_rsrc_t ry = __builtin_amdgcn_make_buffer_rsrc(reinterpret_cast<unsigned char*>(p.y) + (size_t)b * img, 0, (int)img, 0x00020000);
 #pragma unroll
@@ -289,8 +292,35 @@
             for (int pr = 0; pr < 2; ++pr) {
                 const auto sl = __builtin_amdgcn_permlane32_swap(lo[2 * pr], lo[2 * pr + 1], false, false);
                 const auto sh = __builtin_amdgcn_permlane32_swap(hi[2 * pr], hi[2 * pr + 1], false, false);
-                __builtin_amdgcn_raw_buffer_store_b128(u32x4{sl[0], sh[0], sl[1], sh[1]}, ry, voff + pr * 32, 0, 0);
+                if constexpr (POOL3) {
+                    if (q < HWo)
+                        *reinterpret_cast<u32x4*>(lds + q * PITCH + (wm * WCH + ci * 32) * 2 + khalf * 16 + pr * 32) =
+                            u32x4{ordered2_bf16(sl[0]), ordered2_bf16(sh[0]), ordered2_bf16(sl[1]), ordered2_bf16(sh[1])};
+                } else {
+                    __builtin_amdgcn_raw_buffer_store_b128(u32x4{sl[0], sh[0], sl[1], sh[1]}, ry, voff + pr * 32, 0, 0);
+                }
             }
+        }
+    }
+    if constexpr (POOL3) {
+        __syncthreads();
+        constexpr int CV = BM / 8;
+        uint4* yimg = reinterpret_cast<uint4*>(p.y + (size_t)b * HWo * p.Cout + co0);
+        const u32 ycv = (u32)p.Cout >> 3;
+        for (int i = tid; i < HWo * CV; i += CI_THREADS) {
+            const int px = i / CV, c = i - px * CV;
+            const int h = px / p.Wo, w = px - h * p.Wo;
+            uint4 best = make_uint4(0x80008000u, 0x80008000u, 0x80008000u, 0x80008000u);
+#pragma unroll
+            for (int dh = -1; dh <= 1; ++dh)
+#pragma unroll
+                for (int dw = -1; dw <= 1; ++dw) {
+                    const int hi = h + dh, wi = w + dw;
+                    const bool in = (hi >= 0) & (hi < p.Ho) & (wi >= 0) & (wi < p.Wo);
+                    const uint4 v = *reinterpret_cast<const uint4*>(lds + (in ? hi * p.Wo + wi : px) * PITCH + c * 16);
+                    best = make_uint4(pkmax_i16(v.x, best.x), pkmax_i16(v.y, best.y), pkmax_i16(v.z, best.z), pkmax_i16(v.w, best.w));
+                }
+            yimg[(size_t)px * ycv + (u32)c] = make_uint4(unordered2_bf16(best.x), unordered2_bf16(best.y), unordered2_bf16(best.z), unordered2_bf16(best.w));
         }
     }
     CI_PROF_MARK(3)
@@ -320,10 +350,11 @@
     }
 }
 
-extern "C" int ssdhip_conv2d_image_nhwc_bf16(const void* x, const void* weight, const void* bias, void* y, int B, int H, int W, int Cin,
-                                             int Cout, int ksize, int stride, int padding, int dilation, int relu, void* stream_) {
+static int ci_conv2d(const void* x, const void* weight, const void* bias, void* y, int B, int H, int W, int Cin, int Cout, int ksize, int stride,
+                     int padding, int dilation, int relu, bool pool3, void* stream_) {
     hipStream_t stream = static_cast<hipStream_t>(stream_);
     if (!x || !weight || !y || B <= 0 || H <= 0 || W <= 0 || Cin <= 0 || Cout <= 0) return SSDHIP_E_BADARG;
+    if (pool3 && (ksize != 3 || stride != 1 || padding != dilation || x == y)) return SSDHIP_E_BADARG;
     if ((ksize != 1 && ksize != 3) || stride < 1 || stride > 4 || dilation < 1 || dilation > 16 || padding < 0 ||
         padding > dilation * (ksize / 2))
         return SSDHIP_E_BADARG;
@@ -347,7 +378,10 @@
     p.xcd_map = (B % 8 == 0) ? 1 : 0;
     const bool small = (Ho * Wo <= 128 && (ksize == 3 || H * W <= 128)) || p.n_pxt > 1;
 #define CI_LAUNCH(BM_, KS_, NPB_) hipLaunchKernelGGL((conv_image_kernel<BM_, KS_, NPB_>), grid, block, 0, stream, p)
-    if (ksize == 3) {
+    if (pool3) {
+        if (bm == 128) hipLaunchKernelGGL((conv_image_kernel<128, 3, 3, false, true>), grid, block, 0, stream, p);
+        else hipLaunchKernelGGL((conv_image_kernel<64, 3, 3, false, true>), grid, block, 0, stream, p);
+    } else if (ksize == 3) {
         if (bm == 128) { if (small) CI_LAUNCH(128, 3, 1); else CI_LAUNCH(128, 3, 3); }
         else { if (small) CI_LAUNCH(64, 3, 1); else CI_LAUNCH(64, 3, 3); }
     } else {
@@ -356,6 +390,16 @@
     }
 #undef CI_LAUNCH
     return hipGetLastError() == hipSuccess ? SSDHIP_OK : SSDHIP_E_LAUNCH;
+}
+
+extern "C" int ssdhip_conv2d_image_nhwc_bf16(const void* x, const void* weight, const void* bias, void* y, int B, int H, int W, int Cin,
+                                             int Cout, int ksize, int stride, int padding, int dilation, int relu, void* stream) {
+    return ci_conv2d(x, weight, bias, y, B, H, W, Cin, Cout, ksize, stride, padding, dilation, relu, false, stream);
+}
+
+extern "C" int ssdhip_conv3x3_image_pool3_nhwc_bf16(const void* x, const void* weight, const void* bias, void* y, int B, int H, int W,
+                                                    int Cin, int Cout, int dilation, int relu, void* stream) {
+    return ci_conv2d(x, weight, bias, y, B, H, W, Cin, Cout, 3, 1, dilation, dilation, relu, true, stream);
 }
 
 extern "C" int ssdhip_conv2d_image_x3_nhwc_f16(const void* x, const void* weight, const float* bias, void* y, int B, int H, int W, int C,
diff --git a/ssd_keras_amd/csrc/ssdhip_layers.hip b/ssd_keras_amd/csrc/ssdhip_layers.hip
--- a/ssd_keras_amd/csrc/ssdhip_layers.hip
+++ b/ssd_keras_amd/csrc/ssdhip_layers.hip
@@ -82,19 +82,6 @@
 }
 
 constexpr int POOL3_THREADS = 1024;
-typedef unsigned short l_u16x2 __attribute__((ext_vector_type(2)));
-__device__ __forceinline__ u32 l_ordered2(u32 v) {
-    const u32 mag = v & 0x7fff7fffu;
-    const l_u16x2 over = __builtin_elementwise_sub_sat(__builtin_bit_cast(l_u16x2, mag), __builtin_bit_cast(l_u16x2, 0x7f807f80u));
-    const l_u16x2 one = __builtin_elementwise_min(over, __builtin_bit_cast(l_u16x2, 0x00010001u));
-    v &= ~(__builtin_bit_cast(u32, one) << 15);
-    const u32 neg = __builtin_bit_cast(u32, __builtin_bit_cast(s16x2, v) >> 15);
-    return v ^ (neg & 0x7fff7fffu);
-}
-__device__ __forceinline__ u32 l_unordered2(u32 t) {
-    const u32 neg = __builtin_bit_cast(u32, __builtin_bit_cast(s16x2, t) >> 15);
-    return t ^ (neg & 0x7fff7fffu);
-}
 __global__ __launch_bounds__(POOL3_THREADS) void pool3x3s1_slab_kernel(const uint4* __restrict__ x, uint4* __restrict__ y, int H, int W,
                                                                        u32 cvec, u32 slabs) {
     extern __shared__ uint4 pool3_tile[];
@@ -103,7 +90,7 @@
     const size_t base = (size_t)b * (size_t)(H * W) * cvec + slab * 8u;
     for (u32 i = threadIdx.x; i < n; i += POOL3_THREADS) {
         const uint4 v = x[base + (size_t)(i >> 3) * cvec + (i & 7u)];
-        pool3_tile[i] = make_uint4(l_ordered2(v.x), l_ordered2(v.y), l_ordered2(v.z), l_ordered2(v.w));
+        pool3_tile[i] = make_uint4(ordered2_bf16(v.x), ordered2_bf16(v.y), ordered2_bf16(v.z), ordered2_bf16(v.w));
     }
     __syncthreads();
     for (u32 i = threadIdx.x; i < n; i += POOL3_THREADS) {
@@ -119,7 +106,7 @@
                 const uint4 v = pool3_tile[(in ? hi * W + wi : px) * 8 + c];
                 best = make_uint4(pkmax_i16(v.x, best.x), pkmax_i16(v.y, best.y), pkmax_i16(v.z, best.z), pkmax_i16(v.w, best.w));
             }
-        y[base + (size_t)px * cvec + (u32)c] = make_uint4(l_unordered2(best.x), l_unordered2(best.y), l_unordered2(best.z), l_unordered2(best.w));
+        y[base + (size_t)px * cvec + (u32)c] = make_uint4(unordered2_bf16(best.x), unordered2_bf16(best.y), unordered2_bf16(best.z), unordered2_bf16(best.w));
     }
 }
 
diff --git a/ssd_keras_amd/models/_common.py b/ssd_keras_amd/models/_common.py
--- a/ssd_keras_amd/models/_common.py
+++ b/ssd_keras_amd/models/_common.py
@@ -70,6 +70,10 @@
     steps = steps if steps is not None else [None] * n_predictor_layers
     offsets = offsets if offsets is not None else [None] * n_predictor_layers
     return list(scales), ars, n_boxes, steps, offsets
+
+
+def deferred_images(x):
+    return getattr(x, "_ssdhip_deferred_images", None)
 
 
 class SSDModel(PredictorHeads, nn.Module):
@@ -258,13 +262,44 @@
                 return _ConvBiasActPoolFn.apply(x, conv.weight, conv.bias, run, conv.stride, conv.padding, conv.dilation, wb, bb, wt, link_in)
         return self.max_pool(self.conv_act(conv, x, relu=True, link_in=link_in), kernel, stride, pad, ceil_mode=ceil_mode)
 
-    def conv1_block_pool(self, c1, c2, x):
+    def conv_act_pool3(self, conv, x):
+        fused = (sel.pool3_candidates(sel.geometry_of(conv, x))
+                 if self._fused(x, conv) and sel.switch("CONV") in ("auto", "auto_miopen") else {})
+        if not fused:
+            return self.conv_act_pool(conv, x, 3, 1, pad=1)
+        cands = {"separate": lambda: self.conv_act_pool(conv, x, 3, 1, pad=1)}
+        for name, fn in fused.items():
+            cands[name] = lambda fn=fn: fn(x, conv.weight, conv.bias)
+        key = ("conv_pool3", tuple(x.shape), conv.out_channels, conv.kernel_size[0], conv.dilation[0])
+        if SSDModel._conv_choice.get(key) is None:
+            cands["separate"]()
+        name = self._pick(key, cands)
+        return cands[name if name in cands else "separate"]()
+
+    def _conv1_block_ok(self, c1, c2, x):
         same3 = lambda c: (c.kernel_size == (3, 3) and c.stride == (1, 1) and c.padding == (1, 1) and c.dilation == (1, 1)
                            and c.groups == 1 and c.bias is not None)
-        if (not sel.on("NO_CONV1_BLOCK") and sel.switch("CONV") in ("auto", "auto_miopen")
+        return (not sel.on("NO_CONV1_BLOCK") and sel.switch("CONV") in ("auto", "auto_miopen")
                 and self._fused(x, c1) and self._fused(x, c2) and same3(c1) and same3(c2)
                 and c1.in_channels == 3 and c1.out_channels == 64
-                and c2.in_channels == 64 and c2.out_channels % 64 == 0):
+                and c2.in_channels == 64 and c2.out_channels % 64 == 0)
+
+    def conv1_block_pool(self, c1, c2, x):
+        raw = deferred_images(x)
+        if raw is not None:
+            lambdas = (self.subtract_mean, None, list(self.swap_channels) if self.swap_channels else None)
+            pre = lambda: nat.preprocess(raw, *lambdas)
+            if not self._conv1_block_ok(c1, c2, x):
+                return self.conv1_block_pool(c1, c2, pre())
+            cands = {"separate": lambda: self.conv_act_pool(c2, self.conv_act(c1, pre()), 2, 2, ceil_mode=True),
+                     "conv1_block": lambda: nat.conv1_block(pre(), c1.weight, c1.bias, c2.weight, c2.bias, relu=True, pool=True),
+                     "conv1_block_f32": lambda: nat.conv1_block_f32(raw, *lambdas, c1.weight, c1.bias, c2.weight, c2.bias, relu=True, pool=True)}
+            key = ("conv1_block_f32", tuple(x.shape), c2.out_channels)
+            if SSDModel._conv_choice.get(key) is None:
+                cands["separate"]()
+            name = self._pick(key, cands)
+            return cands[name if name in cands else "separate"]()
+        if self._conv1_block_ok(c1, c2, x):
             cands = {"separate": lambda: self.conv_act_pool(c2, self.conv_act(c1, x), 2, 2, ceil_mode=True),
                      "conv1_block": lambda: nat.conv1_block(x, c1.weight, c1.bias, c2.weight, c2.bias, relu=True, pool=True)}
             key = ("conv1_block", tuple(x.shape), c2.out_channels)
@@ -273,6 +308,20 @@
             name = self._pick(key, cands)
             return cands[name if name in cands else "separate"]()
         return self.conv_act_pool(c2, self.conv_act(c1, x), 2, 2, ceil_mode=True)
+
+    def model_input(self, images):
+        first = getattr(self, "_first_block", None)
+        x = images
+        if (first is not None and not sel.on("NO_CONV1_F32") and x.dim() == 4 and x.shape[-1] == self.img_channels == 3 and x.shape[1] != 3
+                and self.fused_inference and x.is_cuda and not torch.is_grad_enabled() and self.__dict__.get("_precise") is None
+                and next(self.parameters()).dtype == torch.bfloat16 and nat.conv1_block_f32_supported(x, self.divide_by_stddev)):
+            c1, c2 = (getattr(self, n) for n in first)
+            b, h, w, c = x.shape
+            ph = torch.empty((b, h, w, c), dtype=torch.bfloat16, device=x.device).permute(0, 3, 1, 2)
+            if self._conv1_block_ok(c1, c2, ph):
+                ph._ssdhip_deferred_images = x
+                return ph
+        return self.preprocess(images)
 
     def max_pool(self, x, kernel, stride, pad=0, ceil_mode=False):
         if self._fused(x) and x.shape[1] % 8 == 0:
@@ -347,7 +396,7 @@
             self.__dict__["_in_forward"] = False
 
     def _raw_predictions(self, images, decode):
-        x = self.preprocess(images)
+        x = self.model_input(images)
         dtype = next(self.parameters()).dtype
         xin = x.to(dtype) if not torch.is_autocast_enabled() else x
         split = self._split_heads(xin)
@@ -436,7 +485,7 @@
         if not had:
             self.__dict__["_head_overlap"] = "4"
         try:
-            x = self.preprocess(images)
+            x = self.model_input(images)
             split = self._split_heads(x.to(next(self.parameters()).dtype))
             if split is None:
                 raise RuntimeError("head_outputs: this model / input does not take the fused inference path")
diff --git a/ssd_keras_amd/models/_conv_select.py b/ssd_keras_amd/models/_conv_select.py
--- a/ssd_keras_amd/models/_conv_select.py
+++ b/ssd_keras_amd/models/_conv_select.py
@@ -5,7 +5,7 @@
 
 SWITCHES = {
     "CONV": "auto", "PREFER": None, "GEMM_1X1": "0", "IMAGE2": "1",
-    "NO_HALO": "0", "NO_IMAGE": "0", "NO_SPLITK": "0", "NO_CONV1_BLOCK": "0", "NO_CHAIN": "0", "NO_POOL_NORM": "0",
+    "NO_HALO": "0", "NO_IMAGE": "0", "NO_IMAGE_POOL3": "0", "NO_SPLITK": "0", "NO_CONV1_BLOCK": "0", "NO_CONV1_F32": "0", "NO_CHAIN": "0", "NO_POOL_NORM": "0",
     "NO_HALO_MIXED": "0", "HEAD_OVERLAP": None, "GRAPH_HEAD_OVERLAP": "4", "HEAD_SPLIT": "3", "HEAD_WGS": None, "SIDE_PRIORITY": "0",
     "NO_OWN_DGRAD": "0", "NO_OWN_WGRAD": "0", "NO_TAPS_BWD": "0", "NO_MASKED_DGRAD": "0", "NO_MASKED_SUMS": "0", "NO_C64_DGRAD": "0",
     "NO_CONV1_1_BWD": "0", "NO_POOL_KEEP": "0", "NO_HALO_POOL_KEEP": "0", "NO_FUSED_POOL_BWD": "0", "NO_OWN_POOL": "0",
@@ -94,6 +94,10 @@
             and not on("NO_IMAGE"))
 
 
+def image_pool3(g):
+    return (igemm(g) and g.k == 3 and g.h * g.w <= 384 and 1 <= g.dilation <= 16 and not on("NO_IMAGE") and not on("NO_IMAGE_POOL3"))
+
+
 def image2(g):
     if switch("IMAGE2") == "0" or on("NO_IMAGE") or g.groups != 1:
         return False
@@ -180,5 +184,11 @@
     return cands
 
 
+def pool3_candidates(g):
+    if not image_pool3(g):
+        return {}
+    return {"image_pool3": lambda x, w, b: nat.conv3x3_image_pool3(x, w, b, dilation=g.dilation, relu=True)}
+
+
 def act_key(g, relu):
     return ("act", (g.batch, g.cin, g.h, g.w), g.cout, g.k, g.dilation, relu, g.stride, g.padding)
diff --git a/ssd_keras_amd/models/keras_ssd300.py b/ssd_keras_amd/models/keras_ssd300.py
--- a/ssd_keras_amd/models/keras_ssd300.py
+++ b/ssd_keras_amd/models/keras_ssd300.py
@@ -12,6 +12,8 @@
 
 
 class _VGGBase(SSDModel):
+
+    _first_block = ("conv1_1", "conv1_2")
 
     def _build_vgg(self, in_ch):
         def c(i, o, k=3, **kw):
@@ -34,8 +36,8 @@
         return ca(self.conv4_3, ca(self.conv4_2, ca(self.conv4_1, x, link_out=l41), link_in=l41, link_out=l42), link_in=l42)
 
     def _vgg_from_pool4(self, x):
-        ca, cap = self.conv_act, self.conv_act_pool
-        x = cap(self.conv5_3, ca(self.conv5_2, ca(self.conv5_1, x)), 3, 1, pad=1)
+        ca = self.conv_act
+        x = self.conv_act_pool3(self.conv5_3, ca(self.conv5_2, ca(self.conv5_1, x)))
         return ca(self.fc7, ca(self.fc6, x))
 
     def _vgg_from_conv4_3(self, conv4_3):
```

Result: no change. 16810 images/sec (median of 6 runs) (+0.6%).
